# SonyResearch/micro_diffusion

Hardware: AMD Instinct MI355X
Metric: training images/sec (global batch 2048) MicroDiT-XL/2 256-res mask=0.75 (higher is better)
Workload: dtype bf16; 1 GPU; MicroDiT_XL_2 res_256_pretrain.yaml mask=0.75, full step = 2 microbatches x 1024 fwd+bwd + grad exchange + clip 0.25 + AdamW; global_batch=2048, microbatch=1024, parallelism=dp1, grad_exchange=none (single rank)

## Files before the change

include/microdit_hip.h:

```cpp
#ifndef MICRODIT_HIP_H
#define MICRODIT_HIP_H

#include <stdint.h>

#ifdef __cplusplus
extern "C" {
#endif

#ifndef __HIP_PLATFORM_AMD__
typedef struct ihipStream_t* hipStream_t;
#endif

#define MD_ABI_VERSION 6
int md_abi_version(void);

enum md_act { MD_ACT_NONE = 0, MD_ACT_GELU_TANH = 1, MD_ACT_GELU_ERF = 2, MD_ACT_SILU = 3 };

enum md_epilogue {
    MD_EPI_STORE_BF16 = 0,
    MD_EPI_RESIDUAL = 1,
    MD_EPI_STORE_F32 = 2,
    MD_EPI_ACCUM_F32 = 3,
    MD_EPI_ATOMIC_F32 = 4,
    MD_EPI_DACT = 5,
// ... 7 lines not shown
    int64_t M, N;
    int64_t c_off;
} md_gemm_problem;
#define MD_GEMM_MAX_PROBLEMS 8

typedef struct md_gemm_args {
    const void* A;
    const void* B;
    void* C;
    void* C2;
    const void* bias;
    const void* res;
    const void* gate;
    const void* aux;
    int64_t M, N, K;
    int64_t lda, ldb, ldc, ldc2, ldr, ldg, ldaux;
    int64_t sA, sB, sC, sC2, sBias, sAux;
    int64_t sSplit;
    int64_t rows_per_sample;
    int32_t batch;
    int32_t ksplit;
    int32_t a_kcontig, b_kcontig;
    int32_t mode;
    int32_t act;
    float alpha;
    int32_t variant;
    int32_t raster_group_n;
    void* timeline;
    int32_t* chosen_variant;
    const void* const* A_list;
    const void* const* B_list;
    int32_t list_segments;
    const md_gemm_problem* problems;
    int32_t n_problems;
    int32_t cu_limit;
    void* tail_ws;
    int64_t tail_ws_bytes;
    int32_t tail_mode;
    int32_t* tail_used;
    int32_t dact_cached;
} md_gemm_args;

#define MD_NOT_ELIGIBLE (-2)
enum md_gemm_variant {
    MD_GEMM_AUTO = 0,
    MD_GEMM_REG128 = 1,
    MD_GEMM_DMA128 = 2,
    MD_GEMM_PACED256 = 3,
    MD_GEMM_PP256 = 4,
    MD_GEMM_W4 = 5
};

int md_gemm_bf16(const md_gemm_args* args, hipStream_t stream);
int md_splitk_reduce(const float* ws, float* out, int64_t M, int64_t N, int64_t ldo, int64_t sOut, int32_t ksplit,
                     int32_t batch, int32_t accumulate, hipStream_t stream);

int md_splitk_reduce_flat(const float* ws, float* out, int64_t n, int64_t slice_stride, int32_t ksplit, int32_t accumulate,
                          hipStream_t stream);

typedef struct md_ln_args {
    const void* x;
    const void* w;
    const void* shift;
    const void* scale;
    const void* pos;
    void* out;
    void* mean;
    void* rstd;
    int64_t rows, C, ldx, ldo, ldmod, rows_per_sample, pos_rows;
    float eps;
    int32_t act;
} md_ln_args;

typedef struct md_ln_bwd_args {
    const void* dz;
    void* dx;
    void* dscale;
    void* dshift;
    void* dw;
    int64_t lddz, lddx, ldg;
    int64_t rows_per_block;
    int32_t accumulate;
    int32_t dscale_is_output;
} md_ln_bwd_args;

int md_ln_fwd(const md_ln_args* a, hipStream_t stream);
int md_ln_bwd(const md_ln_args* a, const md_ln_bwd_args* b, hipStream_t stream);

int md_qkln_fwd(void* buf, int64_t rows, int64_t ld, int64_t col0, int64_t width, int32_t nseg, int64_t seg_stride,
                float* rstd_out, float eps, hipStream_t stream);
int md_qkln_bwd(void* d, int64_t ldd, int64_t dcol0, const void* y, int64_t ldy, int64_t ycol0, int64_t rows,
                int64_t width, int32_t nseg, int64_t dseg_stride, int64_t yseg_stride, const float* rstd, hipStream_t stream);

int md_qkln_fwd_hm(const void* buf, int64_t rows, int64_t ld, int64_t col0, int64_t width, int32_t nseg, int64_t seg_stride,
                   void* out, int64_t out_seg_stride, int64_t S, int32_t hd, float* rstd_out, float eps, hipStream_t stream);
int md_qkln_bwd_hm(const void* dy, int64_t dy_seg_stride, const void* y, int64_t y_seg_stride, void* d, int64_t ldd, int64_t dcol0,
                   int64_t dseg_stride, int64_t rows, int64_t width, int32_t nseg, int64_t S, int32_t hd, const float* rstd,
                   hipStream_t stream);

enum md_det_kind { MD_DET_GATE_BWD = 0, MD_DET_LN_BWD = 1, MD_DET_COLSUM = 2 };
int md_det_ws_floats(int32_t kind, int64_t rows, int64_t rows_per_sample, int64_t rows_per_block, int64_t C, int64_t* out_floats);
int md_ln_bwd_det(const md_ln_args* a, const md_ln_bwd_args* b, float* ws, int64_t ws_floats, hipStream_t stream);
int md_gate_bwd_det(const void* dx, const void* br, const void* gate, int64_t ldgate, void* dbr, float* dgate, int64_t lddg,
                    int64_t rows, int64_t C, int64_t rows_per_sample, int64_t rows_per_block, float* ws, int64_t ws_floats,
                    hipStream_t stream);
int md_colsum_det(const void* x, int32_t x_is_f32, int64_t ld, float* out, int64_t rows, int64_t C, float* ws, int64_t ws_floats,
                  hipStream_t stream);

typedef struct md_attn_args {
    const void *q, *k, *v;
    void* o;
    void* lse;
    const void* d_o;
    void *dq, *dk, *dv;
    void* delta;
    int64_t B, H, Sq, Skv;
    int64_t ldq, ldk, ldv, ldo, sq, sk, sv, so;
    int64_t lddq, lddk, lddv, lddo, sdq, sdk, sdv, sdo;
    float scale;
    int32_t hd;
    int32_t bwd_split;
    int64_t hsq, hsk, hsv, hso, hsdq, hsdk, hsdv, hsdo;
} md_attn_args;

int md_attn_fwd(const md_attn_args* a, hipStream_t stream);
int md_attn_bwd(const md_attn_args* a, hipStream_t stream);

int md_swiglu_fwd(const void* h12, int64_t ldh, void* a, int64_t lda, int64_t M, int64_t f, hipStream_t stream);
int md_swiglu_bwd(const void* da, int64_t ldda, const void* h12, int64_t ldh, void* dh12, int64_t lddh, int64_t M, int64_t f,
                  hipStream_t stream);
int md_gate_bwd(const void* dx, const void* br, const void* gate, int64_t ldgate, void* dbr, float* dgate, int64_t lddg,
                int64_t rows, int64_t C, int64_t rows_per_sample, int64_t rows_per_block, hipStream_t stream);
int md_act_fwd(const void* x, void* y, int64_t n, int32_t act, hipStream_t stream);
int md_act_bwd(const float* dy, const void* x, void* dx, int64_t n, int32_t act, hipStream_t stream);
int md_colsum(const void* x, int32_t x_is_f32, int64_t ld, float* out, int64_t rows, int64_t C, hipStream_t stream);
int md_cast_f32_bf16(const float* x, void* y, int64_t n, const float* scale_ptr, hipStream_t stream);
int md_cast_f32_bf16_clear(float* x, void* y, int64_t n, hipStream_t stream);
int md_cast_rows_bf16(const void* x, int32_t x_dtype, void* y, int64_t rows, int64_t C, const float* rowscale,
                      int64_t rows_per_sample, hipStream_t stream);
int md_mean_tokens(const void* y, void* out, int64_t B, int64_t L, int64_t C, hipStream_t stream);
int md_mean_tokens_bwd(const void* dpool, float* dy, int64_t B, int64_t L, int64_t C, hipStream_t stream);
int md_add_bf16(const void* a, const void* b, void* y, int64_t n, hipStream_t stream);
int md_fill_zero(void* p, int64_t bytes, hipStream_t stream);

int md_get_mask(const float* noise, int64_t B, int64_t T, int64_t len_keep, int32_t* keep_rows, int32_t* ids_restore,
                float* mask, hipStream_t stream);
int md_gather_rows(const void* src, int64_t ld_src, const int32_t* idx, void* dst, int64_t ld_dst, int64_t n, int64_t C,
                   hipStream_t stream);
int md_scatter_rows(const void* src, int64_t ld_src, const int32_t* idx, void* dst, int64_t ld_dst, int64_t n, int64_t C,
                    hipStream_t stream);
int md_moe_route(const float* logits, float* probs, int64_t ld, int64_t B, int64_t S, int32_t E, int32_t k, int32_t* rowidx,
                 float* gval, int32_t* slot, hipStream_t stream);
int md_moe_combine(const void* h2, const float* gval, const int32_t* slot, const void* res, const void* gate, int64_t ldgate,
                   void* br, void* out, int64_t B, int64_t S, int32_t E, int32_t k, int64_t C, hipStream_t stream);
int md_moe_combine_bwd(const void* dbr, const void* h2, const int32_t* rowidx, const float* gval, void* dh2, float* dgval,
                       int64_t R, int64_t C, hipStream_t stream);
int md_moe_dispatch_bwd(const void* dxin, const int32_t* slot, void* dx, const float* probs, int64_t ldp, const float* dgval,
                        void* dlogits, int64_t ldo, int64_t B, int64_t S, int32_t E, int32_t k, int64_t C, hipStream_t stream);

int md_edm_prepare(const float* x0, const float* eps, const float* rnd, float* xn, float* sigma, float* cin, float* cnoise,
                   int64_t B, int64_t per_sample, float p_mean, float p_std, float sigma_data, hipStream_t stream);
int md_edm_prepare_f16(const void* x0_f16, const float* eps, const float* rnd, float* xn, float* x0_f32, float* sigma, float* cin,
                       float* cnoise, int64_t B, int64_t per_sample, float p_mean, float p_std, float sigma_data,
                       hipStream_t stream);
int md_patchify(const float* x, const float* scale, void* out, int64_t B, int32_t C, int32_t H, int32_t W, int32_t p,
                hipStream_t stream);
int md_timestep_embed(const float* t, void* out, int64_t B, int32_t dim, hipStream_t stream);
int md_unpatchify(const void* tok, const int32_t* ids_restore, int64_t Tk, const float* mask_token, float* img, int64_t B,
                  int32_t C, int32_t H, int32_t W, int32_t p, hipStream_t stream);
int md_edm_loss(const void* tok, const int32_t* keep_rows, const float* xn, const float* x0, const float* sigma,
                float* loss_per_sample, float* loss_mean, float* dtok, int64_t B, int64_t Tk, int32_t C, int32_t H, int32_t W,
                int32_t p, float sigma_data, hipStream_t stream);
int md_edm_loss_train(const void* tok, const int32_t* keep_rows, const float* xn, const float* x0, const float* sigma,
                      float* loss_per_sample, float* loss_mean, void* dtok_bf16, float grad_scale, float* loss_accum,
                      float accum_weight, int64_t B, int64_t Tk, int32_t C, int32_t H, int32_t W, int32_t p, float sigma_data,
                      hipStream_t stream);

int md_logvar_fwd(const float* cnoise, const float* freq, const float* phase, const float* w, float* u, float* inv, int64_t B,
                  int32_t C, hipStream_t stream);
// ... 103 lines not shown
```

micro_diffusion_amd/csrc/attention.hip:

```cpp
#include <stdlib.h>
#include "md_common.h"
#include "../../include/microdit_hip.h"

namespace {

typedef __attribute__((address_space(3))) s16x4 lds_s16x4;
typedef unsigned int u32x4 __attribute__((ext_vector_type(4)));

__device__ __forceinline__ bf16x4 tr4(const unsigned char* p) {
    s16x4 v = __builtin_amdgcn_ds_read_tr16_b64_v4i16((lds_s16x4*)(p));
    U64 t;
    t.s = v;
    return t.h;
}

__device__ __forceinline__ bf16x8 tr_frag(const unsigned char* tile, int pitch, int k_lo, int k_hi, int col0, int lane) {
    const int li = lane & 15;
    const int col = col0 + ((lane >> 4) & 1) * 16 + (li & 3) * 4;
    const bf16x4 lo = tr4(tile + (k_lo + (li >> 2)) * pitch + col * 2);
    const bf16x4 hi = tr4(tile + (k_hi + (li >> 2)) * pitch + col * 2);
    bf16x8 f;
    f[0] = lo[0]; f[1] = lo[1]; f[2] = lo[2]; f[3] = lo[3];
    f[4] = hi[0]; f[5] = hi[1]; f[6] = hi[2]; f[7] = hi[3];
    return f;
}

__device__ __forceinline__ bf16x8 row_frag(const unsigned char* tile, int pitch, int kbase, int lane) {
    U128 t;
    t.u = *reinterpret_cast<const uint4*>(tile + (lane & 31) * pitch + (kbase + (lane >> 5) * 8) * 2);
    return t.h;
}

template <int HD>
__device__ __forceinline__ void stage_tile(unsigned char* tile, int pitch, const bf16* src, int64_t ld, int64_t row0,
                                           int64_t nrows, int nstage, int tid, int nthreads) {
    constexpr int CPR = HD / 8;
    for (int task = tid; task < nstage * CPR; task += nthreads) {
        const int r = task / CPR, c = task % CPR;
        uint4 v = make_uint4(0, 0, 0, 0);
        if (row0 + r < nrows) v = *reinterpret_cast<const uint4*>(src + (row0 + r) * ld + c * 8);
        *reinterpret_cast<uint4*>(tile + r * pitch + c * 16) = v;
    }
}

constexpr int STG = 32;

template <int HD, int MAXIT>
__device__ __forceinline__ void stage_pair(unsigned char* tileA, unsigned char* tileB, int pitch, const bf16* A, int64_t lda, const bf16* B,
                                           int64_t ldb, int64_t row0, int64_t nrows, int nstage, int tid, int nthreads) {
    constexpr int CPR = HD / 8;
    uint4 ra[MAXIT], rb[MAXIT];
#pragma unroll
    for (int it = 0; it < MAXIT; ++it) {
        const int task = tid + it * nthreads, r = task / CPR, c = task % CPR;
        ra[it] = rb[it] = make_uint4(0, 0, 0, 0);
        if (task < nstage * CPR && row0 + r < nrows) {
            ra[it] = *reinterpret_cast<const uint4*>(A + (row0 + r) * lda + c * 8);
            rb[it] = *reinterpret_cast<const uint4*>(B + (row0 + r) * ldb + c * 8);
        }
    }
#pragma unroll
    for (int it = 0; it < MAXIT; ++it) {
        const int task = tid + it * nthreads, r = task / CPR, c = task % CPR;
        if (task < nstage * CPR) {
            *reinterpret_cast<uint4*>(tileA + r * pitch + c * 16) = ra[it];
            *reinterpret_cast<uint4*>(tileB + r * pitch + c * 16) = rb[it];
        }
    }
}

constexpr float LOG2E = 1.4426950408889634f;
__device__ __forceinline__ int tile_slot(int r, int hh) { return (r & 3) + 8 * (r >> 2) + 4 * hh; }

__device__ __forceinline__ void ds_cols(f32x16& s, const f32x16& dp, float c1, float l2, float dlt, int rem, int hh) {
#pragma unroll
    for (int r = 0; r < 16; ++r) {
        const float pr = tile_slot(r, hh) < rem ? __builtin_amdgcn_exp2f(s[r] * c1 - l2) : 0.f;
        s[r] = pr * (dp[r] - dlt);
    }
}
template <bool WANT_P, bool WANT_DS>
__device__ __forceinline__ void p_ds_rows(f32x16& s, f32x16& dp, float c1, const float* tL2, const float* tDlt, int rem, int hh) {
#pragma unroll
    for (int r = 0; r < 16; ++r) {
        const int ql = tile_slot(r, hh);
        const float pr = ql < rem ? __builtin_amdgcn_exp2f(s[r] * c1 - tL2[ql]) : 0.f;
        if (WANT_DS) dp[r] = pr * (dp[r] - tDlt[ql]);
        if (WANT_P) s[r] = pr;
    }
}
constexpr float LSE_MASKED = 1e30f;
template <bool WANT_P, bool WANT_DS, bool VEC = true>
__device__ __forceinline__ void p_ds_rows_nomask(f32x16& s, f32x16& dp, float c1, const float* tL2, const float* tDlt, int hh) {
    if (!VEC) {
#pragma unroll
        for (int r = 0; r < 16; ++r) {
            const int ql = tile_slot(r, hh);
            const float pr = __builtin_amdgcn_exp2f(s[r] * c1 - tL2[ql]);
            if (WANT_DS) dp[r] = pr * (dp[r] - tDlt[ql]);
            if (WANT_P) s[r] = pr;
        }
        return;
    }
#pragma unroll
    for (int j = 0; j < 4; ++j) {
        const f32x4 l4 = *reinterpret_cast<const f32x4*>(tL2 + 8 * j + 4 * hh);
        f32x4 d4 = {0.f, 0.f, 0.f, 0.f};
        if (WANT_DS) d4 = *reinterpret_cast<const f32x4*>(tDlt + 8 * j + 4 * hh);
#pragma unroll
        for (int e = 0; e < 4; ++e) {
            const int r = 4 * j + e;
            const float pr = __builtin_amdgcn_exp2f(s[r] * c1 - l4[e]);
            if (WANT_DS) dp[r] = pr * (dp[r] - d4[e]);
            if (WANT_P) s[r] = pr;
        }
    }
}

__device__ __forceinline__ bf16x8 pack8(const f32x16& a, int base) {
    bf16x8 o;
#pragma unroll
    for (int e = 0; e < 8; ++e) o[e] = f2bf(a[base + e]);
    return o;
}

__device__ __forceinline__ void bh_of(int64_t lin, int64_t H, int64_t B, int64_t& b, int64_t& h) {
    const int64_t n8 = (B >> 3) * 8 * H;
    if (lin < n8) {
        const int64_t s = lin >> 3, x = lin & 7;
        lin = ((s / H) * 8 + x) * H + s % H;
    }
    b = lin / H;
    h = lin - b * H;
}

template <int HD>
__device__ __forceinline__ void store_rows(bf16* dst_row, const f32x16 (&acc)[HD / 32], float mul, int lane) {
    const int hh = lane >> 5;
#pragma unroll
    for (int di = 0; di < HD / 32; ++di)
#pragma unroll
        for (int g = 0; g < 4; ++g) {
            bf16x4 o;
#pragma unroll
            for (int e = 0; e < 4; ++e) o[e] = f2bf(acc[di][4 * g + e] * mul);
            st_bf16x4(dst_row + di * 32 + 8 * g + 4 * hh, o);
        }
}

template <int HD, int MAXIT>
__global__ __launch_bounds__(256) void attn_fwd_kernel(md_attn_args p) {
    constexpr int PK = (HD + 8) * 2;
    __shared__ __attribute__((aligned(16))) unsigned char smem[2 * STG * PK];
    const int tid = threadIdx.x, lane = tid & 63, wave = tid >> 6, nthreads = blockDim.x, nw = nthreads >> 6;
    const int hh = lane >> 5;
    const float c1 = p.scale * LOG2E;
    int64_t b = blockIdx.z, h = blockIdx.y;
    if (gridDim.x == 1) bh_of(blockIdx.y + (int64_t)gridDim.y * blockIdx.z, gridDim.y, gridDim.z, b, h);
    const int64_t q = ((int64_t)blockIdx.x * nw + wave) * 32 + (lane & 31);
    const bool qvalid = q < p.Sq;
    const bf16* Q = reinterpret_cast<const bf16*>(p.q) + b * p.sq + h * p.hsq;
    const bf16* K = reinterpret_cast<const bf16*>(p.k) + b * p.sk + h * p.hsk;
    const bf16* V = reinterpret_cast<const bf16*>(p.v) + b * p.sv + h * p.hsv;

    bf16x8 qf[HD / 16];
#pragma unroll
    for (int s = 0; s < HD / 16; ++s) {
        if (qvalid)
            qf[s] = ld_bf16x8(Q + q * p.ldq + s * 16 + hh * 8);
        else
#pragma unroll
            for (int e = 0; e < 8; ++e) qf[s][e] = f2bf(0.f);
    }
    f32x16 oacc[HD / 32];
#pragma unroll
    for (int di = 0; di < HD / 32; ++di)
#pragma unroll
        for (int r = 0; r < 16; ++r) oacc[di][r] = 0.f;
    float m = -1e30f, l = 0.f;

    for (int64_t kbase = 0; kbase < p.Skv; kbase += STG) {
        __syncthreads();
        const int nst = (int)((p.Skv - kbase >= STG) ? STG : ((p.Skv - kbase + 31) / 32) * 32);
        stage_pair<HD, MAXIT>(smem, smem + STG * PK, PK, K, p.ldk, V, p.ldv, kbase, p.Skv, nst, tid, nthreads);
        __syncthreads();
      for (int sub = 0; sub < STG / 32 && kbase + sub * 32 < p.Skv; ++sub) {
        const int64_t key0 = kbase + sub * 32;
        const unsigned char* sK = smem + sub * 32 * PK;
        const unsigned char* sV = smem + STG * PK + sub * 32 * PK;
        f32x16 sacc;
#pragma unroll
        for (int r = 0; r < 16; ++r) sacc[r] = 0.f;
#pragma unroll
        for (int s = 0; s < HD / 16; ++s)
            sacc = __builtin_amdgcn_mfma_f32_32x32x16_bf16(row_frag(sK, PK, s * 16, lane), qf[s], sacc, 0, 0, 0);
        const int rem = (int)(p.Skv - key0);
        float tmax = -1e30f;
#pragma unroll
        for (int r = 0; r < 16; ++r) {
            sacc[r] = tile_slot(r, hh) < rem ? sacc[r] * c1 : -1e30f;
            tmax = fmaxf(tmax, sacc[r]);
        }
        tmax = fmaxf(tmax, __shfl_xor(tmax, 32, 64));
        const float m_new = fmaxf(m, tmax);
        const float alpha = __builtin_amdgcn_exp2f(m - m_new);
        float psum = 0.f;
#pragma unroll
        for (int r = 0; r < 16; ++r) {
            const float pr = __builtin_amdgcn_exp2f(sacc[r] - m_new);
            sacc[r] = pr;
            psum += pr;
        }
        psum += __shfl_xor(psum, 32, 64);
        l = l * alpha + psum;
        m = m_new;
#pragma unroll
        for (int di = 0; di < HD / 32; ++di)
#pragma unroll
            for (int r = 0; r < 16; ++r) oacc[di][r] *= alpha;
#pragma unroll
        for (int sp = 0; sp < 2; ++sp) {
            const bf16x8 pf = pack8(sacc, 8 * sp);
#pragma unroll
            for (int di = 0; di < HD / 32; ++di)
                oacc[di] = __builtin_amdgcn_mfma_f32_32x32x16_bf16(
                    tr_frag(sV, PK, 16 * sp + 4 * hh, 16 * sp + 8 + 4 * hh, di * 32, lane), pf, oacc[di], 0, 0, 0);
        }
      }
    }
    if (qvalid) {
        bf16* O = reinterpret_cast<bf16*>(p.o) + b * p.so + h * p.hso + q * p.ldo;
        store_rows<HD>(O, oacc, 1.f / l, lane);
        if (lane < 32 && p.lse) reinterpret_cast<float*>(p.lse)[(b * p.H + h) * p.Sq + q] = (m + __log2f(l)) * 0.6931471805599453f;
    }
}


template <int HD, int MAXIT>
struct ChunkRegs {
    u32x4 a[MAXIT], b[MAXIT];
};
template <int HD, int SCH, int MAXIT>
__device__ __forceinline__ void chunk_load(ChunkRegs<HD, MAXIT>& R, const bf16* A, int64_t lda, const bf16* B, int64_t ldb, int64_t row0,
                                           int64_t nrows, int tid, int nthreads) {
    constexpr int CPR = HD / 8;
    const u32x4 z4 = {0u, 0u, 0u, 0u};
#pragma unroll
    for (int it = 0; it < MAXIT; ++it) {
        const int task = tid + it * nthreads, r = task / CPR, c = task % CPR;
        const bool ok = task < SCH * CPR && row0 + r < nrows;
        R.a[it] = ok ? *reinterpret_cast<const u32x4*>(A + (row0 + r) * lda + c * 8) : z4;
        R.b[it] = ok ? *reinterpret_cast<const u32x4*>(B + (row0 + r) * ldb + c * 8) : z4;
    }
}
template <int HD, int SCH, int MAXIT>
__device__ __forceinline__ void chunk_store(const ChunkRegs<HD, MAXIT>& R, unsigned char* tileA, unsigned char* tileB, int pitch, int tid,
                                            int nthreads) {
    constexpr int CPR = HD / 8;
#pragma unroll
    for (int it = 0; it < MAXIT; ++it) {
        const int task = tid + it * nthreads, r = task / CPR, c = task % CPR;
        if (task < SCH * CPR) {
            *reinterpret_cast<u32x4*>(tileA + r * pitch + c * 16) = R.a[it];
            *reinterpret_cast<u32x4*>(tileB + r * pitch + c * 16) = R.b[it];
        }
    }
}

template <int HD, int SCH, int MAXIT>
__global__ __launch_bounds__(512) void attn_fwd_stream_kernel(md_attn_args p) {
    constexpr int PK = (HD + 8) * 2;
    __shared__ __attribute__((aligned(16))) unsigned char smem[2 * SCH * PK];
    unsigned char* sKc = smem;
    unsigned char* sVc = smem + SCH * PK;
    const int tid = threadIdx.x, lane = tid & 63, wave = tid >> 6, nthreads = blockDim.x, nw = nthreads >> 6;
    const int hh = lane >> 5;
    const float c1 = p.scale * LOG2E;
    const int64_t b = blockIdx.z, h = blockIdx.y;
    const int64_t q = ((int64_t)blockIdx.x * nw + wave) * 32 + (lane & 31);
    const bool qvalid = q < p.Sq;
    const bf16* Q = reinterpret_cast<const bf16*>(p.q) + b * p.sq + h * p.hsq;
    const bf16* K = reinterpret_cast<const bf16*>(p.k) + b * p.sk + h * p.hsk;
    const bf16* V = reinterpret_cast<const bf16*>(p.v) + b * p.sv + h * p.hsv;

    ChunkRegs<HD, MAXIT> R;
    chunk_load<HD, SCH, MAXIT>(R, K, p.ldk, V, p.ldv, 0, p.Skv, tid, nthreads);
    bf16x8 qf[HD / 16];
// ... 224 lines not shown
        if (tid < SCH) {
            sLseAll[tid] = rl;
            sDltAll[tid] = rd;
        }
        __syncthreads();
        if (qbase + SCH < p.Sq) {
            chunk_load<HD, SCH, MAXIT>(R, Q, p.ldq, dO, p.lddo, qbase + SCH, p.Sq, tid, nthreads);
            const int64_t rn = qbase + SCH + tid;
            const bool ok = tid < SCH && rn < p.Sq;
            rl = ok ? LSE[rn] * LOG2E : LSE_MASKED;
            rd = ok ? DLT[rn] : 0.f;
        }
        auto tile = [&](int sub, int rem) {
            const unsigned char* tQ = sQ + sub * 32 * PK;
            const unsigned char* tdO = sdO + sub * 32 * PK;
            const float* tLse = sLseAll + sub * 32;
            const float* tDlt = sDltAll + sub * 32;
            f32x16 sacc, dpacc;
#pragma unroll
            for (int r = 0; r < 16; ++r) {
                sacc[r] = 0.f;
                dpacc[r] = 0.f;
            }
#pragma unroll
            for (int s = 0; s < HD / 16; ++s) {
                sacc = __builtin_amdgcn_mfma_f32_32x32x16_bf16(row_frag(tQ, PK, s * 16, lane), kf[s], sacc, 0, 0, 0);
                dpacc = __builtin_amdgcn_mfma_f32_32x32x16_bf16(row_frag(tdO, PK, s * 16, lane), vf[s], dpacc, 0, 0, 0);
            }
            (void)rem;
            p_ds_rows_nomask<true, true>(sacc, dpacc, c1, tLse, tDlt, hh);
#pragma unroll
            for (int sp = 0; sp < 2; ++sp) {
                const bf16x8 pf = pack8(sacc, 8 * sp);
                const bf16x8 dsf = pack8(dpacc, 8 * sp);
#pragma unroll
                for (int di = 0; di < HD / 32; ++di) {
                    dvacc[di] = __builtin_amdgcn_mfma_f32_32x32x16_bf16(
                        tr_frag(tdO, PK, 16 * sp + 4 * hh, 16 * sp + 8 + 4 * hh, di * 32, lane), pf, dvacc[di], 0, 0, 0);
                    dkacc[di] = __builtin_amdgcn_mfma_f32_32x32x16_bf16(
                        tr_frag(tQ, PK, 16 * sp + 4 * hh, 16 * sp + 8 + 4 * hh, di * 32, lane), dsf, dkacc[di], 0, 0, 0);
                }
            }
        };
        for (int sub = 0; sub < SCH / 32 && qbase + sub * 32 < p.Sq; ++sub) tile(sub, (int)(p.Sq - qbase - sub * 32));
    }
    if (kvalid) {
        bf16* dK = reinterpret_cast<bf16*>(p.dk) + b * p.sdk + h * p.hsdk + key * p.lddk;
        bf16* dV = reinterpret_cast<bf16*>(p.dv) + b * p.sdv + h * p.hsdv + key * p.lddv;
        store_rows<HD>(dK, dkacc, p.scale, lane);
        store_rows<HD>(dV, dvacc, 1.f, lane);
    }
}

template <int HD, int SQP, int SKP>
__global__ __launch_bounds__((SQP > SKP ? SQP : SKP) * 2) void attn_bwd_fused_kernel(md_attn_args p) {
    constexpr int PK = (HD + 8) * 2;
    __shared__ __attribute__((aligned(16))) unsigned char smem[(2 * SQP + 2 * SKP) * PK + 2 * SQP * 4];
    unsigned char* sQ = smem;
    unsigned char* sdO = smem + SQP * PK;
    unsigned char* sK = smem + 2 * SQP * PK;
    unsigned char* sV = sK + SKP * PK;
    float* sLse = reinterpret_cast<float*>(sV + SKP * PK);
    float* sDlt = sLse + SQP;
    const int tid = threadIdx.x, lane = tid & 63, wave = tid >> 6, nthreads = blockDim.x;
    const int hh = lane >> 5;
    const float c1 = p.scale * LOG2E;
    int64_t b, h;
    bh_of(blockIdx.x + (int64_t)gridDim.x * blockIdx.y, gridDim.x, gridDim.y, b, h);
    const bf16* Q = reinterpret_cast<const bf16*>(p.q) + b * p.sq + h * p.hsq;
    const bf16* K = reinterpret_cast<const bf16*>(p.k) + b * p.sk + h * p.hsk;
    const bf16* V = reinterpret_cast<const bf16*>(p.v) + b * p.sv + h * p.hsv;
    const bf16* dO = reinterpret_cast<const bf16*>(p.d_o) + b * p.sdo + h * p.hsdo;
    const bf16* O = reinterpret_cast<const bf16*>(p.o) + b * p.so + h * p.hso;
    const int nq32 = (int)((p.Sq + 31) / 32), nk32 = (int)((p.Skv + 31) / 32);

    {
        constexpr int CPR = HD / 8;
        constexpr int NT = (SQP > SKP ? SQP : SKP) * 2;
        constexpr int ITQ = (SQP * CPR + NT - 1) / NT, ITK = (SKP * CPR + NT - 1) / NT;
        const float* LSE = reinterpret_cast<const float*>(p.lse) + (b * p.H + h) * p.Sq;
        u32x4 rq[ITQ], rdo[ITQ], ro[ITQ], rk[ITK], rv[ITK];
        float rl[ITQ];
        const u32x4 z4 = {0u, 0u, 0u, 0u};
#pragma unroll
        for (int it = 0; it < ITQ; ++it) {
            const int task = tid + it * NT, r = task / CPR, c = task % CPR;
            const bool ok = task < SQP * CPR && r < p.Sq;
            rq[it] = ok ? *reinterpret_cast<const u32x4*>(Q + (int64_t)r * p.ldq + c * 8) : z4;
            rdo[it] = ok ? *reinterpret_cast<const u32x4*>(dO + (int64_t)r * p.lddo + c * 8) : z4;
            ro[it] = ok ? *reinterpret_cast<const u32x4*>(O + (int64_t)r * p.ldo + c * 8) : z4;
            rl[it] = (ok && c == 0) ? LSE[r] : 0.f;
        }
#pragma unroll
        for (int it = 0; it < ITK; ++it) {
            const int task = tid + it * NT, r = task / CPR, c = task % CPR;
            const bool ok = task < SKP * CPR && r < p.Skv;
            rk[it] = ok ? *reinterpret_cast<const u32x4*>(K + (int64_t)r * p.ldk + c * 8) : z4;
            rv[it] = ok ? *reinterpret_cast<const u32x4*>(V + (int64_t)r * p.ldv + c * 8) : z4;
        }
#pragma unroll
        for (int it = 0; it < ITQ; ++it) {
            const int task = tid + it * NT, r = task / CPR, c = task % CPR;
            if (task < SQP * CPR) {
                *reinterpret_cast<u32x4*>(sQ + r * PK + c * 16) = rq[it];
                *reinterpret_cast<u32x4*>(sdO + r * PK + c * 16) = rdo[it];
            }
            const bf16x8 g = __builtin_bit_cast(bf16x8, rdo[it]), o = __builtin_bit_cast(bf16x8, ro[it]);
            float d = 0.f;
#pragma unroll
            for (int e = 0; e < 8; ++e) d += bf2f(o[e]) * bf2f(g[e]);
#pragma unroll
            for (int s2 = CPR / 2; s2 > 0; s2 >>= 1) d += __shfl_xor(d, s2, 64);
            if (c == 0 && task < SQP * CPR) {
                sDlt[r] = d;
                sLse[r] = rl[it] * LOG2E;
            }
        }
#pragma unroll
        for (int it = 0; it < ITK; ++it) {
            const int task = tid + it * NT, r = task / CPR, c = task % CPR;
            if (task < SKP * CPR) {
                *reinterpret_cast<u32x4*>(sK + r * PK + c * 16) = rk[it];
                *reinterpret_cast<u32x4*>(sV + r * PK + c * 16) = rv[it];
            }
        }
    }
    __syncthreads();

    if (wave < nq32) {
        const unsigned char* myQ = sQ + wave * 32 * PK;
        const unsigned char* mydO = sdO + wave * 32 * PK;
        const int64_t q = (int64_t)wave * 32 + (lane & 31);
        bf16x8 qf[HD / 16], dof[HD / 16];
#pragma unroll
        for (int s = 0; s < HD / 16; ++s) {
            qf[s] = row_frag(myQ, PK, s * 16, lane);
            dof[s] = row_frag(mydO, PK, s * 16, lane);
        }
        const float lse = sLse[wave * 32 + (lane & 31)], dlt = sDlt[wave * 32 + (lane & 31)];
        f32x16 dqacc[HD / 32];
#pragma unroll
        for (int di = 0; di < HD / 32; ++di)
#pragma unroll
            for (int r = 0; r < 16; ++r) dqacc[di][r] = 0.f;
        for (int j = 0; j < nk32; ++j) {
            const unsigned char* tK = sK + j * 32 * PK;
            const unsigned char* tV = sV + j * 32 * PK;
            f32x16 sacc, dpacc;
#pragma unroll
            for (int r = 0; r < 16; ++r) {
                sacc[r] = 0.f;
                dpacc[r] = 0.f;
            }
#pragma unroll
            for (int s = 0; s < HD / 16; ++s) {
                sacc = __builtin_amdgcn_mfma_f32_32x32x16_bf16(row_frag(tK, PK, s * 16, lane), qf[s], sacc, 0, 0, 0);
                dpacc = __builtin_amdgcn_mfma_f32_32x32x16_bf16(row_frag(tV, PK, s * 16, lane), dof[s], dpacc, 0, 0, 0);
            }
            ds_cols(sacc, dpacc, c1, lse, dlt, (int)p.Skv - j * 32, hh);
#pragma unroll
            for (int sp = 0; sp < 2; ++sp) {
                const bf16x8 dsf = pack8(sacc, 8 * sp);
#pragma unroll
                for (int di = 0; di < HD / 32; ++di)
                    dqacc[di] = __builtin_amdgcn_mfma_f32_32x32x16_bf16(
                        tr_frag(tK, PK, 16 * sp + 4 * hh, 16 * sp + 8 + 4 * hh, di * 32, lane), dsf, dqacc[di], 0, 0, 0);
            }
        }
        if (q < p.Sq) {
            bf16* dQ = reinterpret_cast<bf16*>(p.dq) + b * p.sdq + h * p.hsdq + q * p.lddq;
            store_rows<HD>(dQ, dqacc, p.scale, lane);
        }
    }
// ... 4 lines not shown
        bf16x8 kf[HD / 16], vf[HD / 16];
#pragma unroll
        for (int s = 0; s < HD / 16; ++s) {
            kf[s] = row_frag(myK, PK, s * 16, lane);
            vf[s] = row_frag(myV, PK, s * 16, lane);
        }
        f32x16 dkacc[HD / 32], dvacc[HD / 32];
#pragma unroll
        for (int di = 0; di < HD / 32; ++di)
#pragma unroll
            for (int r = 0; r < 16; ++r) {
                dkacc[di][r] = 0.f;
                dvacc[di][r] = 0.f;
            }
        for (int i = 0; i < nq32; ++i) {
            const unsigned char* tQ = sQ + i * 32 * PK;
            const unsigned char* tdO = sdO + i * 32 * PK;
            const float* tLse = sLse + i * 32;
            const float* tDlt = sDlt + i * 32;
            f32x16 sacc, dpacc;
#pragma unroll
            for (int r = 0; r < 16; ++r) {
                sacc[r] = 0.f;
                dpacc[r] = 0.f;
            }
#pragma unroll
            for (int s = 0; s < HD / 16; ++s) {
                sacc = __builtin_amdgcn_mfma_f32_32x32x16_bf16(row_frag(tQ, PK, s * 16, lane), kf[s], sacc, 0, 0, 0);
                dpacc = __builtin_amdgcn_mfma_f32_32x32x16_bf16(row_frag(tdO, PK, s * 16, lane), vf[s], dpacc, 0, 0, 0);
            }
            p_ds_rows<true, true>(sacc, dpacc, c1, tLse, tDlt, (int)p.Sq - i * 32, hh);
#pragma unroll
            for (int sp = 0; sp < 2; ++sp) {
                const bf16x8 pf = pack8(sacc, 8 * sp);
                const bf16x8 dsf = pack8(dpacc, 8 * sp);
#pragma unroll
                for (int di = 0; di < HD / 32; ++di) {
                    dvacc[di] = __builtin_amdgcn_mfma_f32_32x32x16_bf16(
                        tr_frag(tdO, PK, 16 * sp + 4 * hh, 16 * sp + 8 + 4 * hh, di * 32, lane), pf, dvacc[di], 0, 0, 0);
                    dkacc[di] = __builtin_amdgcn_mfma_f32_32x32x16_bf16(
                        tr_frag(tQ, PK, 16 * sp + 4 * hh, 16 * sp + 8 + 4 * hh, di * 32, lane), dsf, dkacc[di], 0, 0, 0);
                }
            }
        }
        if (key < p.Skv) {
            bf16* dK = reinterpret_cast<bf16*>(p.dk) + b * p.sdk + h * p.hsdk + key * p.lddk;
            bf16* dV = reinterpret_cast<bf16*>(p.dv) + b * p.sdv + h * p.hsdv + key * p.lddv;
            store_rows<HD>(dK, dkacc, p.scale, lane);
            store_rows<HD>(dV, dvacc, 1.f, lane);
        }
    }
}

template <int HD, int SQP, int SKP, bool SPLIT2>
__global__ __launch_bounds__((SQP > SKP ? SQP : SKP) * 2) __attribute__((amdgpu_waves_per_eu(SPLIT2 ? 4 : 3)))
void attn_bwd_fused2_kernel(md_attn_args p) {
    constexpr int PK = (HD + 8) * 2;
    constexpr int RMAX = SQP > SKP ? SQP : SKP;
    constexpr int NT = RMAX * 2;
    __shared__ __attribute__((aligned(16))) unsigned char smem[2 * RMAX * PK + 2 * SQP * 4];
    unsigned char* sA = smem;
    unsigned char* sB = smem + RMAX * PK;
    float* sLse = reinterpret_cast<float*>(smem + 2 * RMAX * PK);
    float* sDlt = sLse + SQP;
    const int tid = threadIdx.x, lane = tid & 63, wave = tid >> 6;
    const int hh = lane >> 5;
    const float c1 = p.scale * LOG2E;
    int64_t b, h;
    bh_of(blockIdx.x + (int64_t)gridDim.x * blockIdx.y, gridDim.x, gridDim.y, b, h);
    const bf16* Q = reinterpret_cast<const bf16*>(p.q) + b * p.sq + h * p.hsq;
    const bf16* K = reinterpret_cast<const bf16*>(p.k) + b * p.sk + h * p.hsk;
    const bf16* V = reinterpret_cast<const bf16*>(p.v) + b * p.sv + h * p.hsv;
    const bf16* dO = reinterpret_cast<const bf16*>(p.d_o) + b * p.sdo + h * p.hsdo;
    const bf16* O = reinterpret_cast<const bf16*>(p.o) + b * p.so + h * p.hso;
    const int nq32 = (int)((p.Sq + 31) / 32), nk32 = (int)((p.Skv + 31) / 32);

    constexpr int CPR = HD / 8;
    constexpr int ITQ = (SQP * CPR + NT - 1) / NT, ITK = (SKP * CPR + NT - 1) / NT;
    u32x4 rk[ITK], rv[ITK];
    {
        const float* LSE = reinterpret_cast<const float*>(p.lse) + (b * p.H + h) * p.Sq;
        u32x4 rq[ITQ], rdo[ITQ], ro[ITQ];
        float rl[ITQ];
        const u32x4 z4 = {0u, 0u, 0u, 0u};
#pragma unroll
        for (int it = 0; it < ITQ; ++it) {
            const int task = tid + it * NT, r = task / CPR, c = task % CPR;
            const bool ok = task < SQP * CPR && r < p.Sq;
            rq[it] = ok ? *reinterpret_cast<const u32x4*>(Q + (int64_t)r * p.ldq + c * 8) : z4;
            rdo[it] = ok ? *reinterpret_cast<const u32x4*>(dO + (int64_t)r * p.lddo + c * 8) : z4;
            ro[it] = ok ? *reinterpret_cast<const u32x4*>(O + (int64_t)r * p.ldo + c * 8) : z4;
            rl[it] = (ok && c == 0) ? LSE[r] : 0.f;
        }
#pragma unroll
        for (int it = 0; it < ITK; ++it) {
            const int task = tid + it * NT, r = task / CPR, c = task % CPR;
            const bool ok = task < SKP * CPR && r < p.Skv;
            rk[it] = ok ? *reinterpret_cast<const u32x4*>(K + (int64_t)r * p.ldk + c * 8) : z4;
            rv[it] = ok ? *reinterpret_cast<const u32x4*>(V + (int64_t)r * p.ldv + c * 8) : z4;
        }
#pragma unroll
        for (int it = 0; it < ITQ; ++it) {
            const int task = tid + it * NT, r = task / CPR, c = task % CPR;
            if (task < SQP * CPR) {
                *reinterpret_cast<u32x4*>(sA + r * PK + c * 16) = rq[it];
                *reinterpret_cast<u32x4*>(sB + r * PK + c * 16) = rdo[it];
            }
            const bf16x8 g = __builtin_bit_cast(bf16x8, rdo[it]), o = __builtin_bit_cast(bf16x8, ro[it]);
            float d = 0.f;
#pragma unroll
            for (int e = 0; e < 8; ++e) d += bf2f(o[e]) * bf2f(g[e]);
#pragma unroll
            for (int s2 = CPR / 2; s2 > 0; s2 >>= 1) d += __shfl_xor(d, s2, 64);
            if (c == 0 && task < SQP * CPR) {
                sDlt[r] = d;
                sLse[r] = rl[it] * LOG2E;
            }
        }
    }
    __syncthreads();
    const bool qrole = wave < nq32, krole = wave < nk32;
    bf16x8 qf[HD / 16], dof[HD / 16];
    float lse = 0.f, dlt = 0.f;
    if (qrole) {
#pragma unroll
        for (int s = 0; s < HD / 16; ++s) {
            qf[s] = row_frag(sA + wave * 32 * PK, PK, s * 16, lane);
            dof[s] = row_frag(sB + wave * 32 * PK, PK, s * 16, lane);
        }
        lse = sLse[wave * 32 + (lane & 31)];
        dlt = sDlt[wave * 32 + (lane & 31)];
    }
    __syncthreads();
#pragma unroll
    for (int it = 0; it < ITK; ++it) {
        const int task = tid + it * NT, r = task / CPR, c = task % CPR;
        if (task < SKP * CPR) {
            *reinterpret_cast<u32x4*>(sA + r * PK + c * 16) = rk[it];
            *reinterpret_cast<u32x4*>(sB + r * PK + c * 16) = rv[it];
        }
    }
    __syncthreads();
    if (qrole) {
        const int64_t q = (int64_t)wave * 32 + (lane & 31);
        f32x16 dqacc[HD / 32];
#pragma unroll
        for (int di = 0; di < HD / 32; ++di)
#pragma unroll
            for (int r = 0; r < 16; ++r) dqacc[di][r] = 0.f;
        for (int j = 0; j < nk32; ++j) {
            const unsigned char* tK = sA + j * 32 * PK;
            const unsigned char* tV = sB + j * 32 * PK;
            f32x16 sacc, dpacc;
#pragma unroll
            for (int r = 0; r < 16; ++r) {
                sacc[r] = 0.f;
                dpacc[r] = 0.f;
            }
#pragma unroll
            for (int s = 0; s < HD / 16; ++s) {
                sacc = __builtin_amdgcn_mfma_f32_32x32x16_bf16(row_frag(tK, PK, s * 16, lane), qf[s], sacc, 0, 0, 0);
                dpacc = __builtin_amdgcn_mfma_f32_32x32x16_bf16(row_frag(tV, PK, s * 16, lane), dof[s], dpacc, 0, 0, 0);
            }
            ds_cols(sacc, dpacc, c1, lse, dlt, (int)p.Skv - j * 32, hh);
#pragma unroll
            for (int sp = 0; sp < 2; ++sp) {
                const bf16x8 dsf = pack8(sacc, 8 * sp);
#pragma unroll
                for (int di = 0; di < HD / 32; ++di)
// ... 86 lines not shown
                            tr_frag(tQ, PK, 16 * sp + 4 * hh, 16 * sp + 8 + 4 * hh, di * 32, lane), dsf, acc[di], 0, 0, 0);
                }
            }
            if (key < p.Skv) {
                store_rows<HD>(dK, acc, p.scale, lane);
            }
        } else {
            f32x16 dkacc[HD / 32], dvacc[HD / 32];
#pragma unroll
            for (int di = 0; di < HD / 32; ++di)
#pragma unroll
                for (int r = 0; r < 16; ++r) {
                    dkacc[di][r] = 0.f;
                    dvacc[di][r] = 0.f;
                }
            for (int i = 0; i < nq32; ++i) {
                const unsigned char* tQ = sA + i * 32 * PK;
                const unsigned char* tdO = sB + i * 32 * PK;
                const float* tLse = sLse + i * 32;
                const float* tDlt = sDlt + i * 32;
                f32x16 sacc, dpacc;
#pragma unroll
                for (int r = 0; r < 16; ++r) {
                    sacc[r] = 0.f;
                    dpacc[r] = 0.f;
                }
#pragma unroll
                for (int s = 0; s < HD / 16; ++s) {
                    sacc = __builtin_amdgcn_mfma_f32_32x32x16_bf16(row_frag(tQ, PK, s * 16, lane), kf[s], sacc, 0, 0, 0);
                    dpacc = __builtin_amdgcn_mfma_f32_32x32x16_bf16(row_frag(tdO, PK, s * 16, lane), vf[s], dpacc, 0, 0, 0);
                }
                p_ds_rows<true, true>(sacc, dpacc, c1, tLse, tDlt, (int)p.Sq - i * 32, hh);
#pragma unroll
                for (int sp = 0; sp < 2; ++sp) {
                    const bf16x8 pf = pack8(sacc, 8 * sp);
                    const bf16x8 dsf = pack8(dpacc, 8 * sp);
#pragma unroll
                    for (int di = 0; di < HD / 32; ++di) {
                        dvacc[di] = __builtin_amdgcn_mfma_f32_32x32x16_bf16(
                            tr_frag(tdO, PK, 16 * sp + 4 * hh, 16 * sp + 8 + 4 * hh, di * 32, lane), pf, dvacc[di], 0, 0, 0);
                        dkacc[di] = __builtin_amdgcn_mfma_f32_32x32x16_bf16(
                            tr_frag(tQ, PK, 16 * sp + 4 * hh, 16 * sp + 8 + 4 * hh, di * 32, lane), dsf, dkacc[di], 0, 0, 0);
                    }
                }
            }
            if (key < p.Skv) {
                store_rows<HD>(dK, dkacc, p.scale, lane);
                store_rows<HD>(dV, dvacc, 1.f, lane);
            }
        }
    }
}

inline int fused_bucket(int64_t S) { return S <= 64 ? 64 : S <= 96 ? 96 : S <= 256 ? 256 : 0; }

template <int HD>
void launch_bwd_fused_one(const md_attn_args* a, int variant, int bq, int bk, hipStream_t stream) {
    const dim3 grid((unsigned)a->H, (unsigned)a->B);
#define FUSED(SQP, SKP) hipLaunchKernelGGL((attn_bwd_fused_kernel<HD, SQP, SKP>), grid, dim3((SQP > SKP ? SQP : SKP) * 2), 0, stream, *a)
#define FUSED2(SQP, SKP, SPL) \
    hipLaunchKernelGGL((attn_bwd_fused2_kernel<HD, SQP, SKP, SPL>), grid, dim3((SQP > SKP ? SQP : SKP) * 2), 0, stream, *a)
#define SMALL(SQP, SKP)                          \
    do {                                         \
        if (variant == 2 || (variant == 0 && SQP == 64 && SKP == 64)) FUSED(SQP, SKP); \
        else if (variant == 4) FUSED2(SQP, SKP, true); \
        else FUSED2(SQP, SKP, false);            \
    } while (0)
#define BIG(SQP, SKP)                            \
    do {                                         \
        if (variant == 2) FUSED(SQP, SKP);       \
        else FUSED2(SQP, SKP, true);             \
    } while (0)
    if (bq == 64 && bk == 64) SMALL(64, 64);
    else if (bq == 64 && bk == 96) SMALL(64, 96);
    else if (bq == 96 && bk == 64) SMALL(96, 64);
    else if (bq == 96 && bk == 96) SMALL(96, 96);
    else if (bq == 256 && bk == 96) BIG(256, 96);
    else if (bq == 256 && bk == 256) BIG(256, 256);
    else if (bq == 64 && bk == 256) BIG(64, 256);
    else if (bq == 256 && bk == 64) BIG(256, 64);
    else BIG(96, 256);
#undef SMALL
#undef BIG
#undef FUSED
#undef FUSED2
}

template <int HD>
bool launch_bwd_fused(const md_attn_args* a, int variant, hipStream_t stream) {
    const int bq = fused_bucket(a->Sq), bk = fused_bucket(a->Skv);
    if (!bq || !bk) return false;
    launch_bwd_fused_one<HD>(a, variant, bq, bk, stream);
    return true;
}

inline int stream_waves(int64_t S) {
    static const int cap = [] {
        const char* e = getenv("MD_ATTN_STREAM_WAVES");
        const int v = e ? atoi(e) : 8;
        return v < 3 ? 3 : (v > 8 ? 8 : v);
    }();
    int w = (int)((S + 31) / 32 > cap ? cap : (S + 31) / 32);
    if (w == 5) w = 6;
    if (w < 3) w = 3;
    return w;
}
template <int HD>
void launch_bwd_stream(const md_attn_args* a, hipStream_t stream) {
    int nwq = stream_waves(a->Sq), nwk = stream_waves(a->Skv);
    if (a->Skv <= 128 && nwq > 4) nwq = 4;
    if (a->Sq <= 128 && nwk > 4) nwk = 4;
    const dim3 gq((unsigned)((a->Sq + 32 * nwq - 1) / (32 * nwq)), (unsigned)a->H, (unsigned)a->B);
    const dim3 gk((unsigned)((a->Skv + 32 * nwk - 1) / (32 * nwk)), (unsigned)a->H, (unsigned)a->B);
#define STREAM(KERN, GRID, NW)                                                                                       \
    do {                                                                                                             \
        const dim3 blk(64 * NW);                                                                                     \
        if (NW == 8) hipLaunchKernelGGL((KERN<HD, 128, 2>), GRID, blk, 0, stream, *a);                               \
        else if (NW >= 6) hipLaunchKernelGGL((KERN<HD, 128, 3>), GRID, blk, 0, stream, *a);                          \
        else if (NW == 4) hipLaunchKernelGGL((KERN<HD, 64, 2>), GRID, blk, 0, stream, *a);                           \
        else hipLaunchKernelGGL((KERN<HD, 64, 3>), GRID, blk, 0, stream, *a);                                        \
    } while (0)
    STREAM(attn_bwd_dq_stream_kernel, gq, nwq);
    STREAM(attn_bwd_dkv_stream_kernel, gk, nwk);
#undef STREAM
}

inline int waves_for(int64_t S) {
    int64_t w = (S + 31) / 32;
    return (int)(w > 4 ? 4 : (w < 1 ? 1 : w));
}

inline bool attn_ok(const md_attn_args* a) {
    return a && a->q && a->k && a->v && a->o && a->B > 0 && a->H > 0 && a->Sq > 0 && a->Skv > 0 &&
           (a->hd == 32 || a->hd == 64) && a->ldq % 8 == 0 && a->ldk % 8 == 0 && a->ldv % 8 == 0 && a->ldo % 4 == 0 &&
           a->sq % 8 == 0 && a->sk % 8 == 0 && a->sv % 8 == 0 && a->so % 4 == 0 && a->hsq % 8 == 0 && a->hsk % 8 == 0 &&
           a->hsv % 8 == 0 && a->hso % 4 == 0 && a->hsdo % 8 == 0 && a->hsdq % 4 == 0 && a->hsdk % 4 == 0 && a->hsdv % 4 == 0;
}

inline md_attn_args with_head_strides(const md_attn_args* a) {
    md_attn_args c = *a;
    int64_t* hs[8] = {&c.hsq, &c.hsk, &c.hsv, &c.hso, &c.hsdq, &c.hsdk, &c.hsdv, &c.hsdo};
    for (int64_t* p : hs)
        if (*p == 0) *p = c.hd;
    return c;
}

}

extern "C" int md_attn_fwd(const md_attn_args* a_in, hipStream_t stream) {
    if (!attn_ok(a_in)) return MD_BAD_ARG;
    const md_attn_args args = with_head_strides(a_in);
    const md_attn_args* a = &args;
    static const bool fwd_stream = [] { const char* e = getenv("MD_ATTN_FWD_STREAM"); return !e || atoi(e) != 0; }();
    static const int fwd_stream_min = [] { const char* e = getenv("MD_ATTN_FWD_STREAM_MIN_SKV"); return e ? atoi(e) : 257; }();
    if (fwd_stream && a->Skv >= fwd_stream_min && a->Sq >= 192) {
        int nw = stream_waves(a->Sq);
        if (nw < 6) nw = 6;
        const dim3 grid((unsigned)((a->Sq + 32 * nw - 1) / (32 * nw)), (unsigned)a->H, (unsigned)a->B), blk(64 * nw);
        if (a->hd == 64) {
            if (nw == 8) hipLaunchKernelGGL((attn_fwd_stream_kernel<64, 128, 2>), grid, blk, 0, stream, *a);
            else hipLaunchKernelGGL((attn_fwd_stream_kernel<64, 128, 3>), grid, blk, 0, stream, *a);
        } else {
            if (nw == 8) hipLaunchKernelGGL((attn_fwd_stream_kernel<32, 128, 2>), grid, blk, 0, stream, *a);
            else hipLaunchKernelGGL((attn_fwd_stream_kernel<32, 128, 3>), grid, blk, 0, stream, *a);
        }
        MD_LAUNCH_CHECK();
        return 0;
    }
    const int nw = waves_for(a->Sq);
    dim3 grid((unsigned)((a->Sq + 32 * nw - 1) / (32 * nw)), (unsigned)a->H, (unsigned)a->B);
#define FWD(HD_)                                                                                                  \
    do {                                                                                                           \
        const int chunks = (32 * (HD_ / 8) + 64 * nw - 1) / (64 * nw);                                             \
        if (chunks <= 1) hipLaunchKernelGGL((attn_fwd_kernel<HD_, 1>), grid, dim3(64 * nw), 0, stream, *a);        \
        else if (chunks == 2) hipLaunchKernelGGL((attn_fwd_kernel<HD_, 2>), grid, dim3(64 * nw), 0, stream, *a);   \
        else hipLaunchKernelGGL((attn_fwd_kernel<HD_, 4>), grid, dim3(64 * nw), 0, stream, *a);                    \
    } while (0)
    if (a->hd == 64) FWD(64);
    else FWD(32);
#undef FWD
    MD_LAUNCH_CHECK();
    return 0;
}

extern "C" int md_attn_bwd(const md_attn_args* a_in, hipStream_t stream) {
    if (!attn_ok(a_in) || !a_in->d_o || !a_in->dq || !a_in->dk || !a_in->dv || !a_in->lse || !a_in->delta) return MD_BAD_ARG;
    const md_attn_args args = with_head_strides(a_in);
    const md_attn_args* a = &args;
    if (a->lddq % 4 || a->lddk % 4 || a->lddv % 4 || a->lddo % 8 || a->sdo % 8) return MD_BAD_ARG;
    if (a->bwd_split < 0 || a->bwd_split > 5 || a->bwd_split == 1) return MD_BAD_ARG;
    const bool long_seq = a->Sq > 256 || a->Skv > 256;
    if (a->bwd_split == 5 || (a->bwd_split == 0 && long_seq)) {
        if (a->hd == 64) launch_bwd_stream<64>(a, stream);
        else launch_bwd_stream<32>(a, stream);
        MD_LAUNCH_CHECK();
        return 0;
    }
    if (a->hd == 64 ? launch_bwd_fused<64>(a, a->bwd_split, stream) : launch_bwd_fused<32>(a, a->bwd_split, stream)) {
        MD_LAUNCH_CHECK();
        return 0;
    }
    return -1;
}
```

micro_diffusion_amd/csrc/gemm_pp_common.h:

```cpp
#pragma once
#include "md_common.h"
#include "gemm_common.h"

namespace {

constexpr int PT = 256;
constexpr int HT = 16384;
constexpr int B_REGION = 65536;
constexpr int NUM_CU = 256;

template <int KC>
struct Frag;
template <>
struct Frag<1> {
    bf16x8 v;
    __device__ __forceinline__ bf16x8 get() const { return v; }
};
template <>
struct Frag<0> {
    bf16x4 lo, hi;
    __device__ __forceinline__ bf16x8 get() const {
        bf16x8 f;
        f[0] = lo[0]; f[1] = lo[1]; f[2] = lo[2]; f[3] = lo[3];
        f[4] = hi[0]; f[5] = hi[1]; f[6] = hi[2]; f[7] = hi[3];
// ... 43 lines not shown
    else frag_read<KC, SLOT + KS * 4096>(f, ad[I]);
}

template <int KC>
__device__ __forceinline__ void stage_offsets(unsigned (&ofs)[2][2], int r0, int rmax, int ld, int wave, int lane) {
    asm volatile("" : "+v"(lane));
#pragma unroll
    for (int h = 0; h < 2; ++h)
#pragma unroll
        for (int j = 0; j < 2; ++j) {
            if constexpr (KC) {
                const int row = (wave * 2 + j) * 8 + (lane >> 3);
                const int c = (lane & 7) ^ ((row >> 1) & 7);
                int gr = r0 + h * 128 + row;
                gr = (gr < rmax ? gr : rmax - 1) - r0;
                ofs[h][j] = (unsigned)(gr * ld + c * 8) * 2u;
            } else {
                const int kk = (wave * 2 + j) * 4 + (lane >> 4);
                const int c = (lane & 15) ^ ((kk & 3) << 2);
                int gc = r0 + h * 128 + c * 8;
                const int last = (rmax - 1) & ~7;
                gc = (gc < last ? gc : last) - r0;
                ofs[h][j] = (unsigned)(kk * ld + gc) * 2u;
            }
        }
}

__device__ __forceinline__ void stage_half(const char* base, const unsigned (&ofs)[2], unsigned char* slot, int wave) {
#pragma unroll
    for (int j = 0; j < 2; ++j)
        __builtin_amdgcn_global_load_lds((glb_void_t*)(base + ofs[j]), (lds_void_t*)(slot + (wave * 2 + j) * 1024), 16, 0, 0);
}

constexpr int PP_MAX_PROB = MD_GEMM_MAX_PROBLEMS;
struct PPProblem {
    const void* A;
    const void* B;
    int64_t c_off;
    int lda, ldb, M, N;
    int ntm, ntn, tile0, group_n;
};

struct PPPlan {
    int ntm, ntn, ntiles, total;
    int nk;
    int kspan;
    int group_n;
    int M, N, ksplit;
    int lda, ldb;
    int rps_shift;
    int nseg, nk_seg;
    int nprob;
    int tail_first, tail_units, tail_split, tail_nk;
    PPProblem prob[PP_MAX_PROB];
};

__device__ __forceinline__ void work_decode(const PPPlan& w, int item, int& m0, int& n0, int& batch, int& split) {
    const unsigned y = (unsigned)item / (unsigned)w.ntiles;
    const unsigned t = (unsigned)item - y * (unsigned)w.ntiles;
    batch = (int)(y / (unsigned)w.ksplit);
    split = (int)(y - (unsigned)batch * (unsigned)w.ksplit);
    const unsigned per_group = (unsigned)(w.group_n * w.ntm);
    const unsigned g = t / per_group, rem = t - g * per_group;
    const int first_n = (int)g * w.group_n;
    const int gn = (w.ntn - first_n) < w.group_n ? (w.ntn - first_n) : w.group_n;
    const unsigned tm = rem / (unsigned)gn;
    m0 = (int)tm * PT;
    n0 = (first_n + (int)(rem - tm * (unsigned)gn)) * PT;
}

__device__ __forceinline__ void work_decode_grouped(const PPPlan& w, int item, int& q, int& m0, int& n0, int& split) {
    const unsigned y = (unsigned)item / (unsigned)w.ntiles;
    const int t = (int)((unsigned)item - y * (unsigned)w.ntiles);
    split = (int)y;
    q = 0;
#pragma unroll 1
    for (int i = 1; i < w.nprob; ++i)
        if (t >= w.prob[i].tile0) q = i;
    const PPProblem& pr = w.prob[q];
    const unsigned tl = (unsigned)(t - pr.tile0);
    const unsigned per_group = (unsigned)(pr.group_n * pr.ntm);
    const unsigned g = tl / per_group, rem = tl - g * per_group;
    const int first_n = (int)g * pr.group_n;
    const int gn = (pr.ntn - first_n) < pr.group_n ? (pr.ntn - first_n) : pr.group_n;
    const unsigned tm = rem / (unsigned)gn;
    m0 = (int)tm * PT;
    n0 = (first_n + (int)(rem - tm * (unsigned)gn)) * PT;
}

enum {
    PP_E_BF16 = 0,
    PP_E_BF16_GELU = 1,
    PP_E_RES = 2,
    PP_E_DACT_GELU = 3,
    PP_E_F32 = 4,
    PP_E_BF16_GELU_D = 5,
    PP_E_DACT_MUL = 6,
    PP_E_DACT_SWIGLU = 7
};

struct EpiTile {
    int m0, n0, batch, split;
    int q, M, N, ldc;
    bool plain;
    char* cbase;
    char* c2base;
// ... 114 lines not shown
inline int md_gemm_pp_epi_kind(const md_gemm_args* a) {
    switch (a->mode) {
        case MD_EPI_STORE_BF16:
            return a->act == MD_ACT_NONE ? PP_E_BF16 : a->act == MD_ACT_GELU_ERF ? ((a->dact_cached && a->C2) ? PP_E_BF16_GELU_D : PP_E_BF16_GELU) : -1;
        case MD_EPI_RESIDUAL: return PP_E_RES;
        case MD_EPI_DACT: return a->act == MD_ACT_GELU_ERF ? (a->dact_cached ? PP_E_DACT_MUL : PP_E_DACT_GELU) : -1;
        case MD_EPI_STORE_F32: return PP_E_F32;
        case MD_EPI_SWIGLU_BWD: return PP_E_DACT_SWIGLU;
        default: return -1;
    }
}


inline bool md_gemm_pp_plan(const md_gemm_args* a, PPPlan* w) {
    w->nprob = 0;
    w->ntm = (int)((a->M + PT - 1) / PT);
    w->ntn = (int)((a->N + PT - 1) / PT);
    w->ntiles = w->ntm * w->ntn;
    if (a->problems && a->n_problems > 0) {
        w->nprob = a->n_problems;
        int t0 = 0;
        const int64_t kspan_ = a->K / a->ksplit;
        for (int i = 0; i < a->n_problems; ++i) {
            const md_gemm_problem& s = a->problems[i];
            PPProblem& d = w->prob[i];
            d.A = s.A; d.B = s.B; d.c_off = s.c_off;
            d.lda = (int)s.lda; d.ldb = (int)s.ldb; d.M = (int)s.M; d.N = (int)s.N;
            d.ntm = (int)((s.M + PT - 1) / PT);
            d.ntn = (int)((s.N + PT - 1) / PT);
            d.tile0 = t0;
            int64_t g = (2 << 20) / (PT * kspan_ * 2);
            if (g < 4) g = 4;
            if (g > d.ntn) g = d.ntn;
            d.group_n = (int)g;
            t0 += d.ntm * d.ntn;
        }
        w->ntiles = t0;
    }
    const int64_t total = (int64_t)w->ntiles * (w->nprob ? 1 : a->batch) * a->ksplit;
    if (total > (1 << 30)) return false;
    w->total = (int)total;
    w->kspan = (int)(a->K / a->ksplit);
    w->nk = w->kspan / BKT;
    w->nseg = (a->A_list && a->list_segments > 1) ? a->list_segments : 1;
    w->nk_seg = w->nk / w->nseg;
    w->group_n = a->raster_group_n > 0 ? a->raster_group_n : 1;
    w->M = (int)a->M;
    w->N = (int)a->N;
    w->ksplit = a->ksplit;
    w->lda = (int)a->lda;
    w->ldb = (int)a->ldb;
    w->tail_first = w->total;
    w->tail_units = w->tail_split = w->tail_nk = 0;
    w->rps_shift = -1;
    if (a->rows_per_sample > 0 && (a->rows_per_sample & (a->rows_per_sample - 1)) == 0) {
        w->rps_shift = 0;
        while (((int64_t)1 << w->rps_shift) < a->rows_per_sample) ++w->rps_shift;
    }
    return true;
}

}
```

micro_diffusion_amd/csrc/gemm_w4.hip:

```cpp
#include "gemm_pp_common.h"

namespace {

struct W4Addr {
    unsigned adA[8];
    unsigned adB[8];
    unsigned aofs[8], bofs[8];
    unsigned ldsw;
};

#ifndef W4_ACC_INC
#define W4_ACC_INC "gemm_w4_acc.inc"
#endif
#include W4_ACC_INC

constexpr int W4_BUF = 32768;
constexpr int W4_BREG = 65536;
constexpr int W4_SLAB = 8192;

constexpr bool w4_is_dact(int epi) { return epi == PP_E_DACT_GELU || epi == PP_E_DACT_MUL || epi == PP_E_DACT_SWIGLU; }



typedef unsigned w4_u32x2 __attribute__((ext_vector_type(2), may_alias));
typedef unsigned w4_u32x4 __attribute__((ext_vector_type(4), may_alias));

struct W4Tile {
    int m0, n0, batch;
    int mlim, nlim;
    char* cbase;
    char* c2base;
    const char* opbase;
    const char* gbase;
};

struct W4EpiLane {
    unsigned wr[8];
    unsigned rd[4];
    unsigned oc, oc2, oo, og;
    int rg, c8;
};
struct W4Ops {
    uint4 v[4];
    uint4 gq;
    uint4 v2[4];
};

template <int EPI>
__device__ __forceinline__ void w4_epi_lane(const md_gemm_args& p, const W4Tile& et, int wcol, int lane_in, W4EpiLane& L) {
    int lane = lane_in;
    asm volatile("" : "+v"(lane));
    const int r = lane & 15, g = lane >> 4;
#pragma unroll
    for (int j = 0; j < 8; ++j) L.wr[j] = (unsigned)(r * 256 + ((32 * j + 8 * g) ^ (r << 4)));
#pragma unroll
    for (int t = 0; t < 4; ++t) L.rd[t] = (unsigned)((4 * t + g) * 256 + ((16 * r) ^ ((4 * t + g) << 4)));
    L.rg = g;
    L.c8 = r * 8;
    const int cc = wcol + r * 8 < et.nlim ? r * 8 : 0;
    L.oc = (unsigned)(g * (int)p.ldc + r * 8) * 2u;
    L.oc2 = (unsigned)(g * (int)p.ldc2 + r * 8) * 2u;
    L.oo = (unsigned)(g * (int)(EPI == PP_E_RES ? p.ldr : p.ldaux) + cc) * 2u;
    L.og = (unsigned)cc * 2u;
}

struct W4Rows {
    char* c;
    char* c2;
    const char* op;
    int64_t sc, sc2, so;
};

template <int EPI, bool INTERIOR>
__device__ __forceinline__ void w4_epi_req(const md_gemm_args& p, const W4Tile& et, const W4EpiLane& L, const char* oprow, int row0, int wcol, uint4& dst) {
    if (INTERIOR) {
        dst = *reinterpret_cast<const uint4*>(oprow + L.oo);
    } else if constexpr (EPI == PP_E_DACT_SWIGLU) {
        dst = make_uint4(0u, 0u, 0u, 0u);
    } else {
        const int64_t ldo = EPI == PP_E_RES ? p.ldr : p.ldaux;
        const int row = row0 + L.rg < et.mlim - 1 ? row0 + L.rg : et.mlim - 1;
        dst = *reinterpret_cast<const uint4*>(et.opbase + ((int64_t)row * ldo + wcol) * 2 + L.og);
    }
}
template <int EPI, int I>
__device__ __forceinline__ void w4_epi_gate(const md_gemm_args& p, const PPPlan& w, const W4Tile& et, const W4EpiLane& L, int wrow, int wcol, uint4& gq) {
    gq = make_uint4(0x3f803f80u, 0x3f803f80u, 0x3f803f80u, 0x3f803f80u);
    if (et.gbase) {
        int r0 = et.m0 + wrow + 16 * I;
        r0 = r0 < w.M - 1 ? r0 : w.M - 1;
        const unsigned srow = w.rps_shift >= 0 ? (unsigned)r0 >> w.rps_shift : (unsigned)r0 / (unsigned)p.rows_per_sample;
        gq = *reinterpret_cast<const uint4*>(et.gbase + ((int64_t)srow * p.ldg + wcol) * 2 + L.og);
    }
}

template <int I>
__device__ __forceinline__ void w4_epi_write(unsigned char* slab, const W4EpiLane& L) {
    unsigned char* half = slab + (I & 1) * 4096;
#pragma unroll
    for (int jh = 0; jh < 2; ++jh) {
        float a[16];
        if (jh == 0) w4_acc_read16<I, 0>(a);
        else w4_acc_read16<I, 1>(a);
#pragma unroll
        for (int q = 0; q < 4; ++q) {
            const w4_u32x2 v = {cvt_pk_bf16(a[4 * q], a[4 * q + 1]), cvt_pk_bf16(a[4 * q + 2], a[4 * q + 3])};
            *reinterpret_cast<w4_u32x2*>(half + L.wr[4 * jh + q]) = v;
        }
    }
}

template <int EPI, int I, bool INTERIOR>
__device__ __forceinline__ void w4_epi_store(const md_gemm_args& p, const PPPlan& w, const W4Tile& et, const W4EpiLane& L, int wrow, int wcol,
                                             const w4_u32x4 (&Tv)[4], W4Ops& ops, W4Rows& R) {
#pragma unroll
    for (int t = 0; t < 4; ++t) {
        const uint4 T = make_uint4(Tv[t].x, Tv[t].y, Tv[t].z, Tv[t].w);
        const int row0 = wrow + 16 * I + 4 * t;
        const bool ok = INTERIOR || (wcol + L.c8 < et.nlim && row0 + L.rg < et.mlim);
        char* const crow = R.c;
        uint4 out = T;
        if constexpr (EPI == PP_E_BF16 || EPI == PP_E_RES || EPI == PP_E_BF16_GELU) {
            if (et.c2base && ok) *reinterpret_cast<uint4*>(R.c2 + L.oc2) = T;
        }
        if constexpr (EPI == PP_E_BF16_GELU) {
            float v[8];
            unpack8(T, v);
#pragma unroll
            for (int e = 0; e < 8; e += 2) {
                const f32x2 g2 = gelu_erf_2(f32x2{v[e], v[e + 1]});
                v[e] = g2.x;
                v[e + 1] = g2.y;
            }
            out = make_uint4(cvt_pk_bf16(v[0], v[1]), cvt_pk_bf16(v[2], v[3]), cvt_pk_bf16(v[4], v[5]), cvt_pk_bf16(v[6], v[7]));
        } else if constexpr (EPI == PP_E_BF16_GELU_D) {
            float v[8], dv[8];
            unpack8(T, v);
#pragma unroll
            for (int e = 0; e < 8; e += 2) {
                f32x2 g2, d2;
                gelu_dgelu_erf_2(f32x2{v[e], v[e + 1]}, g2, d2);
                v[e] = g2.x;
                v[e + 1] = g2.y;
                dv[e] = d2.x;
                dv[e + 1] = d2.y;
            }
            out = make_uint4(cvt_pk_bf16(v[0], v[1]), cvt_pk_bf16(v[2], v[3]), cvt_pk_bf16(v[4], v[5]), cvt_pk_bf16(v[6], v[7]));
            if (et.c2base && ok)
                *reinterpret_cast<uint4*>(R.c2 + L.oc2) =
                    make_uint4(cvt_pk_bf16(dv[0], dv[1]), cvt_pk_bf16(dv[2], dv[3]), cvt_pk_bf16(dv[4], dv[5]), cvt_pk_bf16(dv[6], dv[7]));
        } else if constexpr (EPI == PP_E_RES) {
            const uint4 gq = ops.gq;
            const unsigned lw[4] = {T.x, T.y, T.z, T.w}, rw[4] = {ops.v[t].x, ops.v[t].y, ops.v[t].z, ops.v[t].w}, gw[4] = {gq.x, gq.y, gq.z, gq.w};
            unsigned ow[4];
#pragma unroll
            for (int h = 0; h < 4; ++h) {
                const float y0 = __uint_as_float(lw[h] << 16), y1 = __uint_as_float(lw[h] & 0xffff0000u);
                const float r0 = __uint_as_float(rw[h] << 16), r1 = __uint_as_float(rw[h] & 0xffff0000u);
                const float g0 = __uint_as_float(gw[h] << 16), g1 = __uint_as_float(gw[h] & 0xffff0000u);
                ow[h] = cvt_pk_bf16(r0 + g0 * y0, r1 + g1 * y1);
            }
            out = make_uint4(ow[0], ow[1], ow[2], ow[3]);
        } else if constexpr (EPI == PP_E_DACT_MUL) {
            float v[8], ax[8];
            unpack8(T, v);
            unpack8(ops.v[t], ax);
#pragma unroll
            for (int e = 0; e < 8; ++e) v[e] *= ax[e];
            out = make_uint4(cvt_pk_bf16(v[0], v[1]), cvt_pk_bf16(v[2], v[3]), cvt_pk_bf16(v[4], v[5]), cvt_pk_bf16(v[6], v[7]));
        } else if constexpr (EPI == PP_E_DACT_SWIGLU) {
            float g[8], x1[8], x2[8], o2[8];
            unpack8(T, g);
            unpack8(ops.v[t], x1);
            unpack8(ops.v2[t], x2);
#pragma unroll
            for (int e = 0; e < 8; ++e) {
                const float sg = __builtin_amdgcn_rcpf(1.f + __builtin_amdgcn_exp2f(x1[e] * -1.4426950408889634f));
                const float sl = x1[e] * sg;
                o2[e] = g[e] * sl;
                g[e] = g[e] * x2[e] * (sg + sl * (1.f - sg));
            }
            out = make_uint4(cvt_pk_bf16(g[0], g[1]), cvt_pk_bf16(g[2], g[3]), cvt_pk_bf16(g[4], g[5]), cvt_pk_bf16(g[6], g[7]));
            if (ok) *reinterpret_cast<uint4*>(crow + L.oc + 2 * (int64_t)p.N) =
                make_uint4(cvt_pk_bf16(o2[0], o2[1]), cvt_pk_bf16(o2[2], o2[3]), cvt_pk_bf16(o2[4], o2[5]), cvt_pk_bf16(o2[6], o2[7]));
        } else if constexpr (EPI == PP_E_DACT_GELU) {
            float v[8], ax[8];
            unpack8(T, v);
            unpack8(ops.v[t], ax);
#pragma unroll
            for (int e = 0; e < 8; e += 2) {
                const f32x2 d = dgelu_erf_2(f32x2{ax[e], ax[e + 1]});
                v[e] *= d.x;
                v[e + 1] *= d.y;
            }
            out = make_uint4(cvt_pk_bf16(v[0], v[1]), cvt_pk_bf16(v[2], v[3]), cvt_pk_bf16(v[4], v[5]), cvt_pk_bf16(v[6], v[7]));
        }
#ifdef W4_X_NOSTORE
        asm volatile("" : : "v"(out.x), "v"(out.y), "v"(out.z), "v"(out.w));
#else
        if (ok) *reinterpret_cast<uint4*>(crow + L.oc) = out;
#endif
        if constexpr ((EPI == PP_E_RES || w4_is_dact(EPI)) && I < 7) {
            w4_epi_req<EPI, INTERIOR>(p, et, L, R.op, row0 + 16, wcol, ops.v[t]);
            if constexpr (EPI == PP_E_DACT_SWIGLU) w4_epi_req<EPI, INTERIOR>(p, et, L, R.op + 2 * (int64_t)p.N, row0 + 16, wcol, ops.v2[t]);
        }
        R.c += R.sc;
        R.c2 += R.sc2;
        R.op += R.so;
    }
    if constexpr (EPI == PP_E_RES && I < 7) w4_epi_gate<EPI, I + 1>(p, w, et, L, wrow, wcol, ops.gq);
}

template <int I>
__device__ __forceinline__ void w4_epi_read(unsigned char* slab, const W4EpiLane& L, w4_u32x4 (&Tv)[4]) {
    unsigned char* half = slab + (I & 1) * 4096;
#pragma unroll
    for (int t = 0; t < 4; ++t) Tv[t] = *reinterpret_cast<const w4_u32x4*>(half + L.rd[t]);
}

template <int EPI, bool INTERIOR>
__device__ __forceinline__ void w4_epilogue(const md_gemm_args& p, const PPPlan& w, const W4Tile& et, unsigned char* slab, int wrow, int wcol, int lane) {
    W4EpiLane L;
    w4_epi_lane<EPI>(p, et, wcol, lane, L);
    W4Ops ops;
    W4Rows R;
    const int64_t ldo = EPI == PP_E_RES ? p.ldr : p.ldaux;
    R.sc = 8 * p.ldc;
    R.sc2 = 8 * p.ldc2;
    R.so = 8 * ldo;
    R.c = et.cbase + ((int64_t)wrow * p.ldc + wcol) * 2;
    R.c2 = et.c2base ? et.c2base + ((int64_t)wrow * p.ldc2 + wcol) * 2 : nullptr;
    R.op = nullptr;
    if constexpr (EPI == PP_E_RES || w4_is_dact(EPI)) {
        R.op = et.opbase + ((int64_t)wrow * ldo + wcol) * 2;
#pragma unroll
        for (int t = 0; t < 4; ++t) {
            w4_epi_req<EPI, INTERIOR>(p, et, L, R.op, wrow + 4 * t, wcol, ops.v[t]);
            if constexpr (EPI == PP_E_DACT_SWIGLU) w4_epi_req<EPI, INTERIOR>(p, et, L, R.op + 2 * (int64_t)p.N, wrow + 4 * t, wcol, ops.v2[t]);
            R.op += R.so;
        }
        if constexpr (EPI == PP_E_RES) w4_epi_gate<EPI, 0>(p, w, et, L, wrow, wcol, ops.gq);
    }
    w4_u32x4 Tv[4];
    w4_epi_write<0>(slab, L);
#define W4_EPI_STEP(I)                                                                                                  \
    w4_epi_read<I>(slab, L, Tv);                                                                                        \
    if constexpr ((I) < 7) w4_epi_write<((I) < 7 ? (I) + 1 : 7)>(slab, L);                                               \
    if constexpr ((I) == 0) asm volatile("s_waitcnt vmcnt(0)" ::: "memory");                                             \
    w4_epi_store<EPI, I, INTERIOR>(p, w, et, L, wrow, wcol, Tv, ops, R);
    W4_EPI_STEP(0) W4_EPI_STEP(1) W4_EPI_STEP(2) W4_EPI_STEP(3) W4_EPI_STEP(4) W4_EPI_STEP(5) W4_EPI_STEP(6) W4_EPI_STEP(7)
#undef W4_EPI_STEP
}

__device__ __forceinline__ void w4_epilogue_f32(float* tile, int64_t ldc, int wrow, int wcol, int lane_in) {
    int lane = lane_in;
    asm volatile("" : "+v"(lane));
    float* const p0 = tile + (int64_t)(wrow + (lane & 15)) * ldc + wcol + 4 * (lane >> 4);
    asm volatile("s_waitcnt vmcnt(0)" ::: "memory");
#define W4_F32_STEP(I, JH)                                                                                               \
    {                                                                                                                    \
        float a[16];                                                                                                     \
        w4_acc_read16<I, JH>(a);                                                                                         \
        float* const pr = p0 + (int64_t)(16 * (I)) * ldc + 64 * (JH);                                                    \
        _Pragma("unroll") for (int q = 0; q < 4; ++q)                                                                    \
            *reinterpret_cast<float4*>(pr + 16 * q) = make_float4(a[4 * q], a[4 * q + 1], a[4 * q + 2], a[4 * q + 3]);   \
    }
    W4_F32_STEP(0, 0) W4_F32_STEP(0, 1) W4_F32_STEP(1, 0) W4_F32_STEP(1, 1) W4_F32_STEP(2, 0) W4_F32_STEP(2, 1) W4_F32_STEP(3, 0) W4_F32_STEP(3, 1)
    W4_F32_STEP(4, 0) W4_F32_STEP(4, 1) W4_F32_STEP(5, 0) W4_F32_STEP(5, 1) W4_F32_STEP(6, 0) W4_F32_STEP(6, 1) W4_F32_STEP(7, 0) W4_F32_STEP(7, 1)
#undef W4_F32_STEP
}

template <int AKC, int BKC, int EPI>
__global__ __launch_bounds__(256) __attribute__((amdgpu_num_vgpr(144))) void gemm_bf16_w4_kernel(md_gemm_args p, PPPlan w) {
    __shared__ __attribute__((aligned(1024))) unsigned char smem[2 * W4_BREG + 4 * W4_SLAB];
    const int tid = threadIdx.x, lane = tid & 63;
    const int wave = __builtin_amdgcn_readfirstlane(tid >> 6);
    const int wr = wave >> 1, wc = wave & 1;

    int w_first, w_stride, w_count;
    {
        const int G = gridDim.x, x = blockIdx.x & 7, j = blockIdx.x >> 3;
        const int q = w.total >> 3, r = w.total & 7;
        const int lo = x < r ? x * (q + 1) : r * (q + 1) + (x - r) * q;
        const int cnt = q + (x < r ? 1 : 0);
        w_stride = (G - x + 7) >> 3;
        w_first = lo + j;
        w_count = j < cnt ? (int)((unsigned)(cnt - j + w_stride - 1) / (unsigned)w_stride) : 0;
    }
    if (w_count == 0) return;
    const int pairs = w_count * (w.nk >> 1);

    const unsigned lds0 = (unsigned)(uintptr_t)(lds_void_t*)smem;
    W4Addr ad;
    {
        const int ra = wr * 128 + (lane & 15), rb = wc * 128 + (lane & 15);
#pragma unroll
        for (int ks = 0; ks < 2; ++ks) {
            if (AKC) ad.adA[ks] = lds0 + (unsigned)(ra * 128 + ((((4 * ks + (lane >> 4)) ^ (ra >> 1)) & 7) << 4));
            if (BKC) ad.adB[ks] = lds0 + (unsigned)(W4_BREG + rb * 128 + ((((4 * ks + (lane >> 4)) ^ (rb >> 1)) & 7) << 4));
        }
        if (AKC) {
#pragma unroll
            for (int i = 2; i < 8; ++i) ad.adA[i] = 0;
        } else {
            const int li = lane & 15, g = lane >> 4;
            const int kk = 8 * g + (li >> 2);
            const int swz = ((kk & 3) << 1) | (((kk >> 3) & 1) << 3);
#pragma unroll
            for (int i = 0; i < 8; ++i) {
                const int col = wr * 128 + 16 * i + 4 * (li & 3);
                ad.adA[i] = lds0 + (unsigned)(kk * 512 + ((((col >> 3) ^ swz) & 31) << 4) + ((col >> 2) & 1) * 8);
            }
        }
        if (!BKC) {
            const int li = lane & 15, g = lane >> 4;
            const int kk = 8 * g + (li >> 2);
            const int swz = ((kk & 3) << 1) | (((kk >> 3) & 1) << 3);
#pragma unroll
            for (int j = 0; j < 8; ++j) {
                const int col = wc * 128 + 16 * j + 4 * (li & 3);
                ad.adB[j] = lds0 + (unsigned)(W4_BREG + kk * 512 + ((((col >> 3) ^ swz) & 31) << 4) + ((col >> 2) & 1) * 8);
            }
        } else {
#pragma unroll
            for (int j = 2; j < 8; ++j) ad.adB[j] = 0;
// ... 84 lines not shown
    int c_n = 0, c_kt = 0;
#define W4_KTILE(BUF, FRESH)                                                                                            \
    do {                                                                                                                \
        w4_h0<AKC, BKC, BUF, FRESH>(ad, rA, rB, s_koffA, s_koffB);                                                      \
        w4_h1<AKC, BKC, BUF, FRESH>(ad, rA, rB, s_koffA, s_koffB);                                                      \
        w4_h2<AKC, BKC, BUF, FRESH>(ad, rA, rB, s_koffA, s_koffB);                                                      \
        s_koffA += kstepA;                                                                                              \
        s_koffB += kstepB;                                                                                              \
        w4_h3<AKC, BKC, BUF>(ad);                                                                                       \
    } while (0)

    for (int it = 0; it < pairs; ++it) {
        if (c_kt == 0) W4_KTILE(0, true);
        else W4_KTILE(0, false);
        W4_KTILE(1, false);
        stager_pair_done();
        c_kt += 2;
        if (c_kt == w.nk) {
            if constexpr (EPI == PP_E_F32) {
                int m0, n0, batch = 0, split;
                float* tile;
                int64_t ldc;
                if (GROUPABLE && w.nprob) {
                    int q;
                    work_decode_grouped(w, w_first + c_n * w_stride, q, m0, n0, split);
                    const PPProblem& pr = w.prob[q];
                    ldc = pr.N;
                    tile = reinterpret_cast<float*>(p.C) + (int64_t)split * p.sSplit + pr.c_off + (int64_t)m0 * ldc + n0;
                } else {
                    work_decode(w, w_first + c_n * w_stride, m0, n0, batch, split);
                    ldc = p.ldc;
                    tile = reinterpret_cast<float*>(p.C) + (int64_t)batch * p.sC + (int64_t)split * p.sSplit + (int64_t)m0 * ldc + n0;
                }
                asm volatile("s_nop 15\n\ts_nop 15");
                w4_epilogue_f32(tile, ldc, wr * 128, wc * 128, lane);
                c_kt = 0;
                ++c_n;
                continue;
            }
            W4Tile et;
            int split;
            work_decode(w, w_first + c_n * w_stride, et.m0, et.n0, et.batch, split);
            et.mlim = w.M - et.m0;
            et.nlim = w.N - et.n0;
            et.cbase = reinterpret_cast<char*>(p.C) + ((int64_t)et.batch * p.sC + (int64_t)et.m0 * p.ldc + et.n0) * 2;
            et.c2base = (!w4_is_dact(EPI) && p.C2) ? reinterpret_cast<char*>(p.C2) + ((int64_t)et.batch * p.sC2 + (int64_t)et.m0 * p.ldc2 + et.n0) * 2 : nullptr;
            et.opbase = EPI == PP_E_RES   ? reinterpret_cast<const char*>(p.res) + ((int64_t)et.m0 * p.ldr + et.n0) * 2
                        : w4_is_dact(EPI) ? reinterpret_cast<const char*>(p.aux) + ((int64_t)et.batch * p.sAux + (int64_t)et.m0 * p.ldaux + et.n0) * 2
                                          : nullptr;
            et.gbase = (EPI == PP_E_RES && p.gate) ? reinterpret_cast<const char*>(p.gate) + (size_t)et.n0 * 2 : nullptr;
            asm volatile("s_nop 15\n\ts_nop 15");
#ifndef W4_X_NOEPI
            unsigned char* const slab = smem + 2 * W4_BREG + wave * W4_SLAB;
            if (et.mlim >= PT && et.nlim >= PT) w4_epilogue<EPI, true>(p, w, et, slab, wr * 128, wc * 128, lane);
            else w4_epilogue<EPI, false>(p, w, et, slab, wr * 128, wc * 128, lane);
#else
            asm volatile("s_waitcnt vmcnt(0)" ::: "memory");
#endif
            c_kt = 0;
            ++c_n;
        }
    }
    asm volatile("s_waitcnt vmcnt(0)" ::: "memory");
}

}

static bool w4_instantiated(int akc, int bkc, int epi) {
    if (!akc) return !bkc && epi == PP_E_F32;
    if (bkc) return epi == PP_E_BF16 || epi == PP_E_RES || epi == PP_E_DACT_GELU || epi == PP_E_DACT_MUL;
    return epi == PP_E_BF16 || epi == PP_E_BF16_GELU || epi == PP_E_BF16_GELU_D || epi == PP_E_RES || epi == PP_E_DACT_SWIGLU;
}

bool md_gemm_w4_eligible(const md_gemm_args* a) {
    const int epi = md_gemm_pp_epi_kind(a);
    if (epi < 0 || !w4_instantiated(a->a_kcontig, a->b_kcontig, epi)) return false;
    if (!md_gemm_pp_shape_ok(a, epi)) return false;
    if (epi == PP_E_DACT_SWIGLU && (!a->aux || a->batch != 1 || a->ldaux < 2 * a->N || a->ldc < 2 * a->N)) return false;
    if (a->A_list || a->B_list || a->timeline) return false;
    if (a->bias || a->alpha != 1.f) return false;
    const int64_t kspan = a->K / a->ksplit;
    if (epi == PP_E_F32) {
        if (a->ksplit > 1 && a->sSplit <= 0) return false;
        if (a->problems) {
            for (int i = 0; i < a->n_problems; ++i) {
                const md_gemm_problem& s = a->problems[i];
                if (s.M % PT || s.N % PT || kspan * (s.lda > s.ldb ? s.lda : s.ldb) >= ((int64_t)1 << 30)) return false;
            }
            return true;
        }
        if (a->M % PT || a->N % PT || a->ldc % 4) return false;
        return kspan * (a->lda > a->ldb ? a->lda : a->ldb) < ((int64_t)1 << 30);
    }
    if (a->ksplit != 1 || a->problems) return false;
    if (!a->b_kcontig && (a->K * a->ldb >= (int64_t)1 << 30)) return false;
    return true;
}

int md_gemm_w4_launch(const md_gemm_args* a, hipStream_t stream) {
    PPPlan w;
    if (!md_gemm_pp_plan(a, &w)) return MD_BAD_ARG;
    const int cus = (a->cu_limit > 0 && a->cu_limit < NUM_CU) ? a->cu_limit : NUM_CU;
    const unsigned G = (unsigned)(w.total < cus ? w.total : cus);
    if (a->tail_used) *a->tail_used = 0;
    const int epi = md_gemm_pp_epi_kind(a);
    const dim3 grid(G, 1, 1), block(256);
#define W4_LAUNCH(AK, BK, E) hipLaunchKernelGGL((gemm_bf16_w4_kernel<AK, BK, E>), grid, block, 0, stream, *a, w)
    if (!a->a_kcontig) {
        W4_LAUNCH(0, 0, PP_E_F32);
    } else if (a->b_kcontig) {
        if (epi == PP_E_BF16) W4_LAUNCH(1, 1, PP_E_BF16);
        else if (epi == PP_E_RES) W4_LAUNCH(1, 1, PP_E_RES);
        else if (epi == PP_E_DACT_MUL) W4_LAUNCH(1, 1, PP_E_DACT_MUL);
        else W4_LAUNCH(1, 1, PP_E_DACT_GELU);
    } else {
        if (epi == PP_E_BF16) W4_LAUNCH(1, 0, PP_E_BF16);
        else if (epi == PP_E_BF16_GELU) W4_LAUNCH(1, 0, PP_E_BF16_GELU);
        else if (epi == PP_E_BF16_GELU_D) W4_LAUNCH(1, 0, PP_E_BF16_GELU_D);
        else if (epi == PP_E_DACT_SWIGLU) W4_LAUNCH(1, 0, PP_E_DACT_SWIGLU);
        else W4_LAUNCH(1, 0, PP_E_RES);
    }
#undef W4_LAUNCH
    MD_LAUNCH_CHECK();
    return 0;
}
```

micro_diffusion_amd/csrc/norm.hip:

```cpp
#include "md_common.h"
#include "../../include/microdit_hip.h"

namespace {

constexpr int MAXCH = 4;

__device__ __forceinline__ float act_fwd(float v, int act) {
    if (act == MD_ACT_GELU_TANH) return gelu_tanh_f(v);
    if (act == MD_ACT_GELU_ERF) return gelu_erf_f(v);
    if (act == MD_ACT_SILU) return silu_f(v);
    return v;
}
__device__ __forceinline__ float act_bwd(float v, int act) {
    if (act == MD_ACT_GELU_TANH) return dgelu_tanh_f(v);
    if (act == MD_ACT_GELU_ERF) return dgelu_erf_f(v);
    if (act == MD_ACT_SILU) return dsilu_f(v);
    return 1.f;
}

template <int NCH, bool GENERIC, bool KEEP_RAW>
__device__ __forceinline__ void load_row(const md_ln_args& p, int64_t row, int lane, float (&v)[NCH][8],
                                         float (&raw)[KEEP_RAW ? NCH : 1][8]) {
    const bf16* xr = reinterpret_cast<const bf16*>(p.x) + row * p.ldx;
    const float* pr = (GENERIC && p.pos) ? reinterpret_cast<const float*>(p.pos) + (row % p.pos_rows) * p.C : nullptr;
// ... 301 lines not shown
__global__ __launch_bounds__(256) void ln_det_sum_kernel(const float* ws, int64_t nslices, float* out, int64_t ldo, int64_t C) {
    det_slice_sum(ws, nslices, out, ldo, C);
}

template <int NCH>
__global__ __launch_bounds__(256) void qkln_fwd_kernel(bf16* buf, int64_t rows, int64_t ld, int64_t col0, int C, int nseg,
                                                       int64_t seg_stride, float* rstd_out, float eps) {
    const int lane = threadIdx.x & 63;
    const int64_t wave = (int64_t)blockIdx.x * 4 + (threadIdx.x >> 6);
    const int64_t nwaves = (int64_t)gridDim.x * 4;
    const int64_t items = rows * nseg;
    const float invC = 1.f / (float)C;
    auto at = [&](int64_t vr) { return buf + (vr / nseg) * ld + col0 + (vr % nseg) * seg_stride; };
    bf16x8 nxt[NCH];
    if (wave < items) issue_row<NCH>(at(wave), C, lane, nxt);
    for (int64_t vr = wave; vr < items; vr += nwaves) {
        bf16* r = at(vr);
        float v[NCH][8];
        unpack_row<NCH>(nxt, v);
        if (vr + nwaves < items) issue_row<NCH>(at(vr + nwaves), C, lane, nxt);
        float s = 0.f;
#pragma unroll
        for (int j = 0; j < NCH; ++j)
#pragma unroll
            for (int e = 0; e < 8; ++e) s += v[j][e];
        const float mean = wave_sum(s) * invC;
        float q = 0.f;
#pragma unroll
        for (int j = 0; j < NCH; ++j) {
            const int c = lane * 8 + j * 512;
            if (c < C) {
#pragma unroll
                for (int e = 0; e < 8; ++e) {
                    const float d = v[j][e] - mean;
                    q += d * d;
                }
            }
        }
        const float rstd = rsqrtf(wave_sum(q) * invC + eps);
        if (lane == 0) rstd_out[(vr % nseg) * rows + vr / nseg] = rstd;
#pragma unroll
        for (int j = 0; j < NCH; ++j) {
            const int c = lane * 8 + j * 512;
            if (c < C) {
                bf16x8 o;
#pragma unroll
                for (int e = 0; e < 8; ++e) o[e] = f2bf((v[j][e] - mean) * rstd);
                st_bf16x8(r + c, o);
            }
        }
    }
}

template <int NCH>
__global__ __launch_bounds__(256) void qkln_bwd_kernel(bf16* d, int64_t ldd, int64_t dcol0, const bf16* y, int64_t ldy,
                                                       int64_t ycol0, int64_t rows, int C, int nseg, int64_t dseg_stride,
                                                       int64_t yseg_stride, const float* rstd_in) {
    const int lane = threadIdx.x & 63;
    const int64_t wave = (int64_t)blockIdx.x * 4 + (threadIdx.x >> 6);
    const int64_t nwaves = (int64_t)gridDim.x * 4;
    const int64_t items = rows * nseg;
    const float invC = 1.f / (float)C;
    auto dat = [&](int64_t vr) { return d + (vr / nseg) * ldd + dcol0 + (vr % nseg) * dseg_stride; };
    auto yat = [&](int64_t vr) { return y + (vr / nseg) * ldy + ycol0 + (vr % nseg) * yseg_stride; };
    bf16x8 ng[NCH], ny[NCH];
    float nrstd = 0.f;
    if (wave < items) {
        issue_row<NCH>(dat(wave), C, lane, ng);
        issue_row<NCH>(yat(wave), C, lane, ny);
        nrstd = rstd_in[(wave % nseg) * rows + wave / nseg];
    }
    for (int64_t vr = wave; vr < items; vr += nwaves) {
        bf16* dr = dat(vr);
        float g[NCH][8], xh[NCH][8];
        unpack_row<NCH>(ng, g);
        unpack_row<NCH>(ny, xh);
        const float rstd = nrstd;
        float s1 = 0.f, s2 = 0.f;
#pragma unroll
        for (int j = 0; j < NCH; ++j)
#pragma unroll
            for (int e = 0; e < 8; ++e) {
                s1 += g[j][e];
                s2 += g[j][e] * xh[j][e];
            }
        if (vr + nwaves < items) {
            const int64_t nx = vr + nwaves;
            issue_row<NCH>(dat(nx), C, lane, ng);
            issue_row<NCH>(yat(nx), C, lane, ny);
            nrstd = rstd_in[(nx % nseg) * rows + nx / nseg];
        }
        s1 = wave_sum(s1) * invC;
        s2 = wave_sum(s2) * invC;
#pragma unroll
        for (int j = 0; j < NCH; ++j) {
            const int c = lane * 8 + j * 512;
            if (c < C) {
                bf16x8 o;
#pragma unroll
                for (int e = 0; e < 8; ++e) o[e] = f2bf(rstd * (g[j][e] - s1 - xh[j][e] * s2));
                st_bf16x8(dr + c, o);
            }
        }
    }
}

struct HmMap {
    int64_t S, H;
    int hd_shift;
    __device__ __forceinline__ int64_t row_base(int64_t row) const {
        const int64_t b = row / S, s = row - b * S;
        return (b * H * S + s) << hd_shift;
    }
    __device__ __forceinline__ int64_t col_off(int c) const {
        return ((int64_t)(c >> hd_shift) * S << hd_shift) + (c & ((1 << hd_shift) - 1));
    }
};
template <int NCH>
__device__ __forceinline__ void issue_row_hm(const bf16* base, const HmMap& m, int C, int lane, bf16x8 (&h)[NCH]) {
#pragma unroll
    for (int j = 0; j < NCH; ++j) {
        const int c = lane * 8 + j * 512;
        if (c < C) h[j] = ld_bf16x8(base + m.col_off(c));
        else
#pragma unroll
            for (int e = 0; e < 8; ++e) h[j][e] = (bf16)0.f;
    }
}

template <int NCH>
__global__ __launch_bounds__(256) void qkln_fwd_hm_kernel(const bf16* buf, int64_t rows, int64_t ld, int64_t col0, int C, int nseg,
                                                          int64_t seg_stride, bf16* out, int64_t out_seg_stride, HmMap m,
                                                          float* rstd_out, float eps) {
    const int lane = threadIdx.x & 63;
    const int64_t wave = (int64_t)blockIdx.x * 4 + (threadIdx.x >> 6);
    const int64_t nwaves = (int64_t)gridDim.x * 4;
    const int64_t items = rows * nseg;
    const float invC = 1.f / (float)C;
    auto at = [&](int64_t vr) { return buf + (vr / nseg) * ld + col0 + (vr % nseg) * seg_stride; };
    bf16x8 nxt[NCH];
    if (wave < items) issue_row<NCH>(at(wave), C, lane, nxt);
    for (int64_t vr = wave; vr < items; vr += nwaves) {
        float v[NCH][8];
// ... 160 lines not shown
    md_ln_bwd_args k = *b;
    if (region > 0) {
        k.dscale = wsS;
        k.dshift = wsH;
    }
    dim3 grid((unsigned)chunks, (unsigned)nsmp, 1);
    const bool generic = a->act != MD_ACT_NONE || a->pos != nullptr;
#define LNB(N, G) hipLaunchKernelGGL((ln_bwd_kernel<N, G, true>), grid, dim3(256), 0, stream, *a, k)
    if (generic) {
        if (a->C <= 512) LNB(1, true); else if (a->C <= 1024) LNB(2, true); else LNB(4, true);
    } else {
        if (a->C <= 512) LNB(1, false); else if (a->C <= 1024) LNB(2, false); else LNB(4, false);
    }
#undef LNB
    if ((want_cols && region > 0) || (b->dscale && (b->dw || b->dscale_is_output)))
        hipLaunchKernelGGL(ln_det_finish_kernel, dim3((unsigned)((a->C + 255) / 256), (unsigned)groups), dim3(256), 0, stream, wsS, wsH,
                           chunks, reinterpret_cast<float*>(b->dscale), reinterpret_cast<float*>(b->dshift), b->ldg,
                           reinterpret_cast<const float*>(a->w), reinterpret_cast<const bf16*>(a->scale), a->ldmod,
                           reinterpret_cast<float*>(b->dw), wsW, nsmp, a->C, b->dscale_is_output);
    if (wsW)
        hipLaunchKernelGGL(ln_det_sum_kernel, dim3((unsigned)((a->C + 63) / 64), 1), dim3(256), 0, stream, wsW, groups,
                           reinterpret_cast<float*>(b->dw), (int64_t)0, a->C);
    MD_LAUNCH_CHECK();
    return 0;
}

extern "C" int md_qkln_fwd(void* buf, int64_t rows, int64_t ld, int64_t col0, int64_t width, int32_t nseg, int64_t seg_stride,
                           float* rstd_out, float eps, hipStream_t stream) {
    if (!buf || !rstd_out || rows <= 0 || width <= 0 || width % 8 || width > 64 * 8 * MAXCH || ld % 8 || col0 % 8 || nseg < 1 ||
        nseg > 4 || seg_stride % 8 || (nseg > 1 && seg_stride < width))
        return MD_BAD_ARG;
#define QKF(N) hipLaunchKernelGGL(qkln_fwd_kernel<N>, dim3(ln_grid(rows * nseg)), dim3(256), 0, stream, (bf16*)buf, rows, ld, \
                                  col0, (int)width, (int)nseg, seg_stride, rstd_out, eps)
    if (width <= 512) QKF(1); else if (width <= 1024) QKF(2); else QKF(4);
#undef QKF
    MD_LAUNCH_CHECK();
    return 0;
}

extern "C" int md_qkln_bwd(void* d, int64_t ldd, int64_t dcol0, const void* y, int64_t ldy, int64_t ycol0, int64_t rows,
                           int64_t width, int32_t nseg, int64_t dseg_stride, int64_t yseg_stride, const float* rstd,
                           hipStream_t stream) {
    if (!d || !y || !rstd || rows <= 0 || width <= 0 || width % 8 || width > 64 * 8 * MAXCH || ldd % 8 || ldy % 8 ||
        dcol0 % 8 || ycol0 % 8 || nseg < 1 || nseg > 4 || dseg_stride % 8 || yseg_stride % 8)
        return MD_BAD_ARG;
#define QKB(N) hipLaunchKernelGGL(qkln_bwd_kernel<N>, dim3(ln_grid(rows * nseg)), dim3(256), 0, stream, (bf16*)d, ldd, dcol0, \
                                  (const bf16*)y, ldy, ycol0, rows, (int)width, (int)nseg, dseg_stride, yseg_stride, rstd)
    if (width <= 512) QKB(1); else if (width <= 1024) QKB(2); else QKB(4);
#undef QKB
    MD_LAUNCH_CHECK();
    return 0;
}

namespace {
inline bool hm_ok(int64_t rows, int64_t width, int64_t S, int32_t hd) {
    return S > 0 && rows % S == 0 && (hd == 32 || hd == 64) && width % hd == 0;
}
}

extern "C" int md_qkln_fwd_hm(const void* buf, int64_t rows, int64_t ld, int64_t col0, int64_t width, int32_t nseg, int64_t seg_stride,
                              void* out, int64_t out_seg_stride, int64_t S, int32_t hd, float* rstd_out, float eps, hipStream_t stream) {
    if (!buf || !out || !rstd_out || rows <= 0 || width <= 0 || width % 8 || width > 64 * 8 * MAXCH || ld % 8 || col0 % 8 || nseg < 1 ||
        nseg > 4 || seg_stride % 8 || (nseg > 1 && (seg_stride < width || out_seg_stride < rows * width)) || out_seg_stride % 8 ||
        !hm_ok(rows, width, S, hd))
        return MD_BAD_ARG;
    const HmMap m{S, width / hd, hd == 64 ? 6 : 5};
#define QKF(N) hipLaunchKernelGGL(qkln_fwd_hm_kernel<N>, dim3(ln_grid(rows * nseg)), dim3(256), 0, stream, (const bf16*)buf, rows, ld, \
                                  col0, (int)width, (int)nseg, seg_stride, (bf16*)out, out_seg_stride, m, rstd_out, eps)
    if (width <= 512) QKF(1); else if (width <= 1024) QKF(2); else QKF(4);
#undef QKF
    MD_LAUNCH_CHECK();
    return 0;
}

extern "C" int md_qkln_bwd_hm(const void* dy, int64_t dy_seg_stride, const void* y, int64_t y_seg_stride, void* d, int64_t ldd,
                              int64_t dcol0, int64_t dseg_stride, int64_t rows, int64_t width, int32_t nseg, int64_t S, int32_t hd,
                              const float* rstd, hipStream_t stream) {
    if (!dy || !y || !d || !rstd || rows <= 0 || width <= 0 || width % 8 || width > 64 * 8 * MAXCH || ldd % 8 || dcol0 % 8 ||
        nseg < 1 || nseg > 4 || dseg_stride % 8 || dy_seg_stride % 8 || y_seg_stride % 8 || !hm_ok(rows, width, S, hd))
        return MD_BAD_ARG;
    const HmMap m{S, width / hd, hd == 64 ? 6 : 5};
#define QKB(N) hipLaunchKernelGGL(qkln_bwd_hm_kernel<N>, dim3(ln_grid(rows * nseg)), dim3(256), 0, stream, (const bf16*)dy, dy_seg_stride, \
                                  (const bf16*)y, y_seg_stride, (bf16*)d, ldd, dcol0, dseg_stride, rows, (int)width, (int)nseg, m, rstd)
    if (width <= 512) QKB(1); else if (width <= 1024) QKB(2); else QKB(4);
#undef QKB
    MD_LAUNCH_CHECK();
    return 0;
}
```

micro_diffusion_amd/engine.py:

```python
from __future__ import annotations

import ctypes
import math
import os
from ctypes import byref
from typing import Dict, List, Optional

import torch

from . import hip
from .arch import BlockPlan, DiTConfig, caption_ffn_hidden, plan_blocks

BF16, F32, I32 = torch.bfloat16, torch.float32, torch.int32
TAIL_WS_BYTES = 256 * 256 * 256 * 4


class Tape:
    pass


class _Arena:
    ALIGN = 256

    def __init__(self, dev):
# ... 54 lines not shown
            return self
        kv = {name: (k[:B * self.Lc], None if khm is None else khm[:B * self.Lc]) for name, (k, khm) in self.kv.items()}
        return Conditioning(B, self.Lc, self.head_major, self.version, self.pooled[:B], kv)


def _p(t):
    return None if t is None else t.data_ptr()


class DiTEngine:
    def __init__(self, cfg: DiTConfig, params: Dict[str, torch.Tensor], shadows: Dict[str, torch.Tensor],
                 grads: Dict[str, torch.Tensor], buffers: Dict[str, torch.Tensor]):
        self.cfg = cfg
        self.P, self.S, self.G, self.buf = params, shadows, grads, buffers
        self.mixer, self.backbone = plan_blocks(cfg)
        self.dev = next(iter(params.values())).device
        self.L = hip.lib()
        self.wgrad_target_blocks = 768
        self.gemm_profile = None
        self.kernel_profile = None
        self.gemm_prefer = hip.GEMM_AUTO
        self.attn_bwd_prefer = hip.ATTN_BWD_AUTO
        self.qk_head_major = os.environ.get("MD_QK_HEAD_MAJOR", "0") == "1"
        self.deterministic = os.environ.get("MD_DETERMINISTIC", "0") == "1"
        self._det_ws_floats = {}
        self.gemm_log = None
        self.before_segment = None
        self.keep_last_tape = False
        self.last_tape = None
        self.route_override = None
        self.route_stats = None
        self.ws = torch.empty(128 << 20, device=self.dev, dtype=F32)
        self.use_arena = False
        self._tape_arena, self._scratch_arena = _Arena(self.dev), _Arena(self.dev)
        self._arena = None
        self._record = False
        self._chosen = ctypes.c_int32(-1)
        self._ptr_cache = {}
        self.ksplit_min_items = 192
        self.splitk_force_pp = False
        self.short_k_accum = True
        self.group_wgrad = True
        self._wgroup = None
        self.single_slice_ws = True
        self.group_dycond = True
        self.group_adaln = True
        self._posb = None
        self.moe_cache_dact = True
        self.batch_adaln = True
        self._adaln = self._adaln_region()
        self.gemm_tail_mode = int(os.environ.get("MD_GEMM_TAIL", "0"))
        self.wgrad_bf16 = None
        self.fuse_swiglu_bwd = os.environ.get("MD_FUSE_SWIGLU_BWD", "1") != "0"
        self.weights_version = 0
        self.cu_limit_fn = None

    def _adaln_region(self):
        names = [bp.name for bp in self.mixer] + [bp.name for bp in self.backbone]
        col, n, w0, b0 = {}, 0, None, None
        for nm in names:
            w, b = self.S.get(nm + ".adaLN_modulation.1.weight"), self.P.get(nm + ".adaLN_modulation.1.bias")
            if w is None or b is None or w.dim() != 2 or w.shape[1] != self.cfg.dim:
                return None
            if w0 is None:
                w0, b0 = w, b
            elif w.data_ptr() != w0.data_ptr() + 2 * n * self.cfg.dim or b.data_ptr() != b0.data_ptr() + 4 * n:
                return None
            col[nm] = n
            n += w.shape[0]
        if w0 is None or n % 8:
            return None
        return {"N": n, "w": w0.data_ptr(), "b": b0.data_ptr(), "col": col}

    def _adaln_all(self, gc, B):
        r = self._adaln
        out = self.empty(B, r["N"])
        D = self.cfg.dim
        self._gemm(A=gc.data_ptr(), B=r["w"], C=out.data_ptr(), bias=r["b"], M=B, N=r["N"], K=D, lda=D, ldb=D, ldc=r["N"], batch=1, ksplit=1,
                   a_kcontig=1, b_kcontig=1, mode=hip.EPI_STORE_BF16, act=0, alpha=1.0)
        return out

    def _st(self):
        return torch.cuda.current_stream().cuda_stream

    def empty(self, *shape, dtype=BF16):
        if self._arena is not None:
            return self._arena.alloc(shape, dtype)
        return torch.empty(*shape, device=self.dev, dtype=dtype)

    def zeros(self, *shape, dtype=F32):
        t = self.empty(*shape, dtype=dtype)
        hip.check(self.L.md_fill_zero(t.data_ptr(), t.numel() * t.element_size(), self._st()), "md_fill_zero")
        return t

    def _prof(self, name, nbytes, launch):
        kp = self.kernel_profile
        if kp is None:
            return launch()
        e0, e1 = torch.cuda.Event(enable_timing=True), torch.cuda.Event(enable_timing=True)
        e0.record()
        launch()
        e1.record()
        kp.setdefault(name, []).append((e0, e1, float(nbytes)))

    def _det_ws(self, kind, rows, rps, rpb, C):
        key = (kind, rows, rps, rpb, C)
        n = self._det_ws_floats.get(key)
        if n is None:
            out = ctypes.c_int64(0)
            hip.check(self.L.md_det_ws_floats(kind, rows, rps, rpb, C, byref(out)), "md_det_ws_floats")
            n = self._det_ws_floats[key] = int(out.value)
        if n == 0:
            return None, 0
        return self.empty(n, dtype=F32).data_ptr(), n

    def _colsum(self, src_ptr, is_f32, ld, out_ptr, rows, C):
        nbytes = (4.0 if is_f32 else 2.0) * rows * C
        if not self.deterministic:
            return self._prof("colsum", nbytes, lambda: hip.check(self.L.md_colsum(src_ptr, is_f32, ld, out_ptr, rows, C, self._st()), "colsum"))
        ws, n = self._det_ws(hip.DET_COLSUM, rows, 0, 0, C)
        self._prof("colsum", nbytes,
                   lambda: hip.check(self.L.md_colsum_det(src_ptr, is_f32, ld, out_ptr, rows, C, ws, n, self._st()), "colsum_det"))

    def _gate_bwd(self, dx, br, gate_ptr, ldgate, dbr, dgate_ptr, lddg, M, d, S, rpb):
        if not self.deterministic:
            return self._prof("gate_bwd", 6.0 * M * d, lambda: hip.check(self.L.md_gate_bwd(
                dx.data_ptr(), br.data_ptr(), gate_ptr, ldgate, dbr.data_ptr(), dgate_ptr, lddg, M, d, S, rpb, self._st()), "gate_bwd"))
        ws, n = self._det_ws(hip.DET_GATE_BWD, M, S, rpb, d)
        self._prof("gate_bwd", 6.0 * M * d, lambda: hip.check(self.L.md_gate_bwd_det(
            dx.data_ptr(), br.data_ptr(), gate_ptr, ldgate, dbr.data_ptr(), dgate_ptr, lddg, M, d, S, rpb, ws, n, self._st()), "gate_bwd_det"))

    def _qkln_fwd(self, ptr, rows, ld, off, width, rstd_ptr, nseg=1):
        self._prof("qk_layernorm", 4.0 * rows * width * nseg, lambda: hip.check(
            self.L.md_qkln_fwd(ptr, rows, ld, off, width, nseg, width, rstd_ptr, self.cfg.norm_eps, self._st()), "md_qkln_fwd"))

    def _qkln_bwd(self, dptr, ldd, doff, yptr, ldy, yoff, rows, width, rstd_ptr, nseg=1):
        self._prof("qk_layernorm", 6.0 * rows * width * nseg, lambda: hip.check(
            self.L.md_qkln_bwd(dptr, ldd, doff, yptr, ldy, yoff, rows, width, nseg, width, width, rstd_ptr, self._st()), "md_qkln_bwd"))

    def _qkln_fwd_hm(self, ptr, rows, ld, off, width, out, S, rstd_ptr, nseg=1):
        self._prof("qk_layernorm", 4.0 * rows * width * nseg, lambda: hip.check(
            self.L.md_qkln_fwd_hm(ptr, rows, ld, off, width, nseg, width, out.data_ptr(), rows * width, S, self.cfg.head_dim, rstd_ptr,
                                  self.cfg.norm_eps, self._st()), "md_qkln_fwd_hm"))

    def _qkln_bwd_hm(self, dy, y, dptr, ldd, doff, rows, width, S, rstd_ptr, nseg=1):
        self._prof("qk_layernorm", 6.0 * rows * width * nseg, lambda: hip.check(
            self.L.md_qkln_bwd_hm(dy.data_ptr(), rows * width, y.data_ptr(), rows * width, dptr, ldd, doff, width, rows, width, nseg, S,
                                  self.cfg.head_dim, rstd_ptr, self._st()), "md_qkln_bwd_hm"))

    def _attn_fwd(self, a):
        nb = 2.0 * a.hd * (2 * a.Sq + 2 * a.Skv) * a.B * a.H
        self._prof("attention", nb, lambda: hip.check(self.L.md_attn_fwd(byref(a), self._st()), "md_attn_fwd"))

    def _gemm(self, **kw):
        a = hip.GemmArgs()
        problems = kw.pop("_problems", None)
        may_refuse = kw.pop("_try", False)
        for k, v in kw.items():
            setattr(a, k, v)
        if self.deterministic and a.mode == hip.EPI_ATOMIC_F32 and a.ksplit > 1:
            raise RuntimeError("deterministic mode: a split-K GEMM with the fp32-atomic epilogue sums in an order that changes from run "
                               "to run; use the workspace slices + md_splitk_reduce (gemm_f32_acc)")
        prof = self.gemm_profile
        if prof is not None:
            e0, e1 = torch.cuda.Event(enable_timing=True), torch.cuda.Event(enable_timing=True)
            e0.record()
        chosen = self._chosen
        a.chosen_variant = ctypes.addressof(chosen)
        if self.cu_limit_fn is not None:
            a.cu_limit = self.cu_limit_fn()
        if self.gemm_tail_mode != 1 and a.mode in (hip.EPI_STORE_BF16, hip.EPI_RESIDUAL, hip.EPI_DACT):
            a.tail_ws, a.tail_ws_bytes, a.tail_mode = self.ws.data_ptr(), TAIL_WS_BYTES, self.gemm_tail_mode
        rc = hip.NOT_ELIGIBLE
        want = self.gemm_prefer if self.gemm_prefer != hip.GEMM_AUTO else a.variant
        if want != hip.GEMM_AUTO:
            a.variant = want
            rc = self.L.md_gemm_bf16(byref(a), self._st())
            if rc == hip.NOT_ELIGIBLE:
                a.variant = hip.GEMM_AUTO
        if rc == hip.NOT_ELIGIBLE:
            rc = self.L.md_gemm_bf16(byref(a), self._st())
        if rc == hip.NOT_ELIGIBLE and may_refuse:
            return False
        hip.check(rc, "md_gemm_bf16")
        if self.gemm_log is not None:
            self.gemm_log.append((chosen.value, a.M, a.N, a.K, a.batch))
        if prof is not None:
            e1.record()
            out_b = 4 if a.mode in (hip.EPI_STORE_F32, hip.EPI_ACCUM_F32, hip.EPI_ATOMIC_F32) else 2
            mn = a.M * a.N * a.batch
            byt = 2.0 * (a.M * a.K + a.N * a.K) * a.batch + mn * out_b * a.ksplit
            byt += mn * 2 * ((1 if a.C2 else 0) + (1 if a.res else 0) + (1 if a.aux else 0)) + (mn * 4 if a.mode == hip.EPI_ACCUM_F32 else 0)
            if a.mode == hip.EPI_SWIGLU_BWD:
                byt += mn * 2 * 2
            fl = 2.0 * a.M * a.N * a.K * a.batch
            key = (a.M, a.N, a.K, a.batch, a.a_kcontig, a.b_kcontig, a.ksplit)
            if problems:
                mn = sum(g["M"] * g["N"] for g in problems)
                fl = 2.0 * mn * a.K
                byt = 2.0 * a.K * sum(g["M"] + g["N"] for g in problems) + mn * 4 * a.ksplit
                key = (-len(problems), mn // 1024, a.K, 1, 0, 0, a.ksplit)
            prof.append((e0, e1, fl, key, byt))
        return True

    def lin_fwd(self, x, wname, out, M, N, K, *, ldx=None, ldc=None, mode=hip.EPI_STORE_BF16, act=0, res=None,
                gate=None, ldg=0, rps=0, C2=None, ldc2=0, xoff=0, ooff=0, bias=True):
        b = self.P.get(wname + ".bias") if bias else None
        self._gemm(A=x.data_ptr() + 2 * xoff, B=self.S[wname + ".weight"].data_ptr(),
                   C=out.data_ptr() + (4 if mode in (hip.EPI_STORE_F32, hip.EPI_ACCUM_F32) else 2) * ooff,
                   C2=_p(C2), bias=_p(b), res=_p(res), gate=gate, M=M, N=N, K=K, lda=ldx or K, ldb=K, ldc=ldc or N,
                   ldc2=ldc2 or N, ldr=N, ldg=ldg, rows_per_sample=rps, batch=1, ksplit=1, a_kcontig=1, b_kcontig=1,
                   mode=mode, act=act, alpha=1.0)

    def lin_dgrad(self, dy, wname, dx, M, N, K, *, lddy=None, mode=hip.EPI_STORE_BF16, act=0, aux=None, res=None,
                  dyoff=0):
        self._gemm(A=dy.data_ptr() + 2 * dyoff, B=self.S[wname + ".weight"].data_ptr(), C=dx.data_ptr(), aux=_p(aux),
                   res=_p(res), M=M, N=K, K=N, lda=lddy or N, ldb=K, ldc=K, ldaux=K, ldr=K, batch=1, ksplit=1,
                   a_kcontig=1, b_kcontig=0, mode=mode, act=act, alpha=1.0)

    def _fused12(self, pre):
        w1, w2 = self.S.get(pre + ".w1.weight"), self.S.get(pre + ".w2.weight")
        if w1 is None or w2 is None or (pre + ".w1.bias") in self.P:
            return False
        return (w2.data_ptr() == w1.data_ptr() + w1.numel() * 2 and
                self.G[pre + ".w2.weight"].data_ptr() == self.G[pre + ".w1.weight"].data_ptr() + w1.numel() * 4)

    def _ksplit(self, out_rows, out_cols, contraction, batch=1):
        ws_cap = max(1, self.ws.numel() // (out_rows * out_cols * batch))
        t256 = ((out_rows + 255) // 256) * ((out_cols + 255) // 256) * batch
        if getattr(self, "short_k_accum", True) and contraction <= 512 and t256 >= 64:
            return 1
        if contraction % 128 == 0 and out_cols % 8 == 0:
            units = contraction // 128
# ... 127 lines not shown
                dst = t["gbf"] + (lo - t["g_lo"]) // 2
                self._prof("splitk_reduce", n * (4.0 * ks + 2), lambda lo=lo, n=n, dst=dst: hip.check(
                    self.L.md_splitk_reduce_flat(self.ws.data_ptr() + (lo - base), dst, n, span_el, ks, 2, self._st()), "md_splitk_reduce_flat"))
                continue
            self._prof("splitk_reduce", 4.0 * n * (ks + 2), lambda lo=lo, n=n: hip.check(
                self.L.md_splitk_reduce_flat(self.ws.data_ptr() + (lo - base), lo, n, span_el, ks, 1, self._st()), "md_splitk_reduce_flat"))

    def ln_args(self, x, wname, out, rows, C, *, shift=None, scale=None, ldmod=0, rps=0, mean=None, rstd=None, act=0,
                pos=None, pos_rows=0):
        return hip.LnArgs(x.data_ptr(), _p(self.P[wname + ".weight"]) if wname else None, shift, scale, _p(pos), _p(out),
                          _p(mean), _p(rstd), rows, C, C, C, ldmod, rps, pos_rows, self.cfg.norm_eps, act)

    def ln_fwd(self, a):
        self._prof("layernorm", 4.0 * a.rows * a.C, lambda: hip.check(self.L.md_ln_fwd(byref(a), self._st()), "md_ln_fwd"))

    @staticmethod
    def _rows_per_block(rows, rps, min_blocks=2048):
        rpb = 64
        while rpb > 4 and (rows + rpb - 1) // rpb < min_blocks:
            rpb //= 2
        return int(max(1, min(rpb, rps)))

    def ln_bwd(self, a, dz, dx, *, accumulate, wname=None, dscale=None, dshift=None, ldg=0):
        rps = a.rows_per_sample if a.rows_per_sample > 0 else a.rows
        rpb = self._rows_per_block(a.rows, rps, 1024)
        is_out = 1 if dscale is not None else 0
        if dscale is None and wname is not None:
            scratch = self.zeros(a.rows // rps, a.C)
            dscale, ldg = scratch.data_ptr(), a.C
        b = hip.LnBwdArgs(dz.data_ptr(), _p(dx), dscale, dshift, _p(self.G[wname + ".weight"]) if wname else None,
                          a.C, a.C, ldg, rpb, 1 if accumulate else 0, is_out)
        if self.deterministic:
            ws, n = self._det_ws(hip.DET_LN_BWD, a.rows, rps, rpb, a.C)
            self._prof("layernorm", (8.0 if accumulate else 6.0) * a.rows * a.C,
                       lambda: hip.check(self.L.md_ln_bwd_det(byref(a), byref(b), ws, n, self._st()), "md_ln_bwd_det"))
            return
        self._prof("layernorm", (8.0 if accumulate else 6.0) * a.rows * a.C,
                   lambda: hip.check(self.L.md_ln_bwd(byref(a), byref(b), self._st()), "md_ln_bwd"))

    def attn_args(self, q, k, v, o, lse, B, H, Sq, Skv, ldq, ldk, ldv, hid, *, do=None, dq=None, dk=None, dv=None,
                  delta=None, lddq=0, lddk=0, lddv=0, hm_qk=False):
        hd = self.cfg.head_dim
        a = hip.AttnArgs(q, k, v, _p(o), _p(lse), _p(do), dq, dk, dv, _p(delta), B, H, Sq, Skv, ldq, ldk, ldv, hid,
                         Sq * ldq, Skv * ldk, Skv * ldv, Sq * hid, lddq, lddk, lddv, hid, Sq * lddq, Skv * lddk,
                         Skv * lddv, Sq * hid, 1.0 / math.sqrt(hd), hd, 0)
        if hm_qk:
            a.ldq = a.ldk = a.lddq = a.lddk = hd
            a.sq = a.sdq = H * Sq * hd
            a.sk = a.sdk = H * Skv * hd
            a.hsq = a.hsdq = Sq * hd
            a.hsk = a.hsdk = Skv * hd
        return a

    def _attn_bwd(self, a):
        self._prof("attention", 2.0 * a.hd * (4 * a.Sq + 4 * a.Skv) * a.B * a.H, lambda: self._attn_bwd_launch(a))

    def _attn_bwd_launch(self, a):
        rc = -1
        if self.attn_bwd_prefer != hip.ATTN_BWD_AUTO:
            a.bwd_split = self.attn_bwd_prefer
            rc = self.L.md_attn_bwd(byref(a), self._st())
            a.bwd_split = hip.ATTN_BWD_AUTO
        if rc == -1:
            rc = self.L.md_attn_bwd(byref(a), self._st())
        hip.check(rc, "md_attn_bwd")

    def _self_attn_fwd(self, pre, xin, B, S, dim, hid, heads, t):
        M, L, st = B * S, self.L, self._st()
        qkv = self.empty(M, 3 * hid)
        self.lin_fwd(xin, pre + ".qkv", qkv, M, 3 * hid, dim)
        rq = self.empty(2, M, dtype=F32)
        o = self.empty(M, hid)
        lse = self.empty(B, heads, S, dtype=F32)
        if self.qk_head_major:
            t.qk = self.empty(2, M, hid)
            self._qkln_fwd_hm(qkv.data_ptr(), M, 3 * hid, 0, hid, t.qk, S, rq.data_ptr(), nseg=2)
            a = self.attn_args(t.qk.data_ptr(), t.qk.data_ptr() + 2 * M * hid, qkv.data_ptr() + 4 * hid, o, lse, B, heads, S, S,
                               0, 0, 3 * hid, hid, hm_qk=True)
        else:
            t.qk = None
            self._qkln_fwd(qkv.data_ptr(), M, 3 * hid, 0, hid, rq.data_ptr(), nseg=2)
            a = self.attn_args(qkv.data_ptr(), qkv.data_ptr() + 2 * hid, qkv.data_ptr() + 4 * hid, o, lse, B, heads, S, S,
                               3 * hid, 3 * hid, 3 * hid, hid)
        self._attn_fwd(a)
        t.qkv, t.rq, t.o, t.lse = qkv, rq, o, lse
        return o

    def _self_attn_bwd(self, pre, xin, do, B, S, dim, hid, heads, t, defer=False):
        M, L, st = B * S, self.L, self._st()
        dqkv = self.empty(M, 3 * hid)
        delta = self.empty(B, heads, S, dtype=F32)
        qkv = t.qkv
        if t.qk is not None:
            dqk = self.empty(2, M, hid)
            a = self.attn_args(t.qk.data_ptr(), t.qk.data_ptr() + 2 * M * hid, qkv.data_ptr() + 4 * hid, t.o, t.lse, B, heads, S, S,
                               0, 0, 3 * hid, hid, do=do, dq=dqk.data_ptr(), dk=dqk.data_ptr() + 2 * M * hid,
                               dv=dqkv.data_ptr() + 4 * hid, delta=delta, lddv=3 * hid, hm_qk=True)
            self._attn_bwd(a)
            self._qkln_bwd_hm(dqk, t.qk, dqkv.data_ptr(), 3 * hid, 0, M, hid, S, t.rq.data_ptr(), nseg=2)
        else:
            a = self.attn_args(qkv.data_ptr(), qkv.data_ptr() + 2 * hid, qkv.data_ptr() + 4 * hid, t.o, t.lse, B, heads, S, S,
                               3 * hid, 3 * hid, 3 * hid, hid, do=do, dq=dqkv.data_ptr(), dk=dqkv.data_ptr() + 2 * hid,
                               dv=dqkv.data_ptr() + 4 * hid, delta=delta, lddq=3 * hid, lddk=3 * hid, lddv=3 * hid)
            self._attn_bwd(a)
            self._qkln_bwd(dqkv.data_ptr(), 3 * hid, 0, qkv.data_ptr(), 3 * hid, 0, M, hid, t.rq.data_ptr(), nseg=2)
        self.lin_wgrad(dqkv, xin, pre + ".qkv", M, 3 * hid, dim, defer=defer)
        dxin = self.empty(M, dim)
        self.lin_dgrad(dqkv, pre + ".qkv", dxin, M, 3 * hid, dim)
        return dxin

    def _kv_linear_fwd(self, n, ycond, Mc, hx, d):
        kv = self.empty(Mc, 2 * hx)
        self.lin_fwd(ycond, n + ".cross_attn.kv_linear", kv, Mc, 2 * hx, d)
        return kv

    def _k_norm_fwd(self, kv, Mc, hx, Lc):
        rk = self.empty(Mc, dtype=F32)
        if self.qk_head_major:
            kn = self.empty(Mc, hx)
            self._qkln_fwd_hm(kv.data_ptr(), Mc, 2 * hx, 0, hx, kn, Lc, rk.data_ptr())
            return rk, kn
        self._qkln_fwd(kv.data_ptr(), Mc, 2 * hx, 0, hx, rk.data_ptr())
        return rk, None

    def _block_fwd(self, bp: BlockPlan, x, ycond, B, S, Lc, gc, mod_all=None, kv=None):
        L, st, cfg = self.L, self._st(), self.cfg
        d, h, hx, f = bp.dim, bp.attn_hidden, bp.xattn_hidden, bp.ffn_hidden
        M, Mc, D = B * S, B * Lc, cfg.dim
        n = bp.name
        t = Tape()
        t.x = x
        if mod_all is not None:
            mod, ldm = mod_all, mod_all.shape[1]
            mp = mod_all.data_ptr() + 2 * self._adaln["col"][n]
        else:
            mod, ldm = self.empty(B, 6 * d), 6 * d
            self.lin_fwd(gc, n + ".adaLN_modulation.1", mod, B, 6 * d, D)
            mp = mod.data_ptr()
        t.mod, t.mp, t.ldm = mod, mp, ldm
        t.xm1 = self.empty(M, d)
        t.st1 = self.empty(2, M, dtype=F32)
        a1 = self.ln_args(x, n + ".norm1", t.xm1, M, d, shift=mp, scale=mp + 2 * d, ldmod=ldm, rps=S, mean=t.st1[0], rstd=t.st1[1])
        self.ln_fwd(a1)
        t.sa = Tape()
        o = self._self_attn_fwd(n + ".attn", t.xm1, B, S, d, h, bp.heads, t.sa)
        t.br1 = self.empty(M, d)
        x1 = self.empty(M, d)
        self.lin_fwd(o, n + ".attn.proj", x1, M, d, h, mode=hip.EPI_RESIDUAL, res=x, gate=mp + 2 * 2 * d, ldg=ldm, rps=S,
                     C2=t.br1)
        t.x1 = x1
        t.xn2 = self.empty(M, d)
        t.st2 = self.empty(2, M, dtype=F32)
        self.ln_fwd(self.ln_args(x1, n + ".norm2", t.xn2, M, d, mean=t.st2[0], rstd=t.st2[1]))
        t.o2 = self.empty(M, hx)
        t.q2 = t.o2 if self.qk_head_major else self.empty(M, hx)
        self.lin_fwd(t.xn2, n + ".cross_attn.q_linear", t.q2, M, hx, d)
        if kv is None:
            t.kv = self._kv_linear_fwd(n, ycond, Mc, hx, d)
        else:
            t.kv, t.k2n = kv
            t.rk2 = None
        t.rq2 = self.empty(M, dtype=F32)
        t.lse2 = self.empty(B, bp.xheads, S, dtype=F32)
        if self.qk_head_major:
            t.q2n = self.empty(M, hx)
            self._qkln_fwd_hm(t.q2.data_ptr(), M, hx, 0, hx, t.q2n, S, t.rq2.data_ptr())
            if kv is None:
                t.rk2, t.k2n = self._k_norm_fwd(t.kv, Mc, hx, Lc)
            ax = self.attn_args(t.q2n.data_ptr(), t.k2n.data_ptr(), t.kv.data_ptr() + 2 * hx, t.o2, t.lse2, B, bp.xheads, S, Lc,
                                0, 0, 2 * hx, hx, hm_qk=True)
        else:
            t.q2n = None
            self._qkln_fwd(t.q2.data_ptr(), M, hx, 0, hx, t.rq2.data_ptr())
            if kv is None:
                t.rk2, t.k2n = self._k_norm_fwd(t.kv, Mc, hx, Lc)
            ax = self.attn_args(t.q2.data_ptr(), t.kv.data_ptr(), t.kv.data_ptr() + 2 * hx, t.o2, t.lse2, B, bp.xheads, S, Lc,
                                hx, 2 * hx, 2 * hx, hx)
        self._attn_fwd(ax)
        x2 = self.empty(M, d)
        self.lin_fwd(t.o2, n + ".cross_attn.proj", x2, M, d, hx, mode=hip.EPI_RESIDUAL, res=x1)
        t.x2 = x2
        t.xm3 = self.empty(M, d)
        t.st3 = self.empty(2, M, dtype=F32)
        self.ln_fwd(self.ln_args(x2, n + ".norm3", t.xm3, M, d, shift=mp + 2 * 3 * d, scale=mp + 2 * 4 * d, ldmod=ldm,
                                 rps=S, mean=t.st3[0], rstd=t.st3[1]))
        x3 = self.empty(M, d)
        t.br3 = self.empty(M, d)
        gate_mlp = mp + 2 * 5 * d
        if not bp.moe:
            t.h12 = self.empty(M, 2 * f)
            if self._fused12(n + ".mlp"):
                self.lin_fwd(t.xm3, n + ".mlp.w1", t.h12, M, 2 * f, d)
            else:
                self.lin_fwd(t.xm3, n + ".mlp.w1", t.h12, M, f, d, ldc=2 * f)
                self.lin_fwd(t.xm3, n + ".mlp.w2", t.h12, M, f, d, ldc=2 * f, ooff=f)
            t.a = self.empty(M, f)
            self._prof("swiglu", 6.0 * M * f, lambda: hip.check(L.md_swiglu_fwd(t.h12.data_ptr(), 2 * f, t.a.data_ptr(), f, M, f, st), "swiglu"))
            self.lin_fwd(t.a, n + ".mlp.w3", x3, M, d, f, mode=hip.EPI_RESIDUAL, res=x2, gate=gate_mlp, ldg=ldm, rps=S,
                         C2=t.br3)
        else:
            E = cfg.num_experts
            k = int(cfg.expert_capacity * S / E)
            ldl = 8 if E <= 8 else 16
            Bk = B * k
            t.k, t.ldl = k, ldl
            logits = self.empty(M, ldl, dtype=F32)
            self.lin_fwd(t.xm3, n + ".mlp.gate", logits, M, E, d, ldc=ldl, mode=hip.EPI_STORE_F32)
            t.probs = self.empty(M, ldl, dtype=F32)
            t.rowidx = self.empty(E, Bk, dtype=I32)
            t.gval = self.empty(E, Bk, dtype=F32)
            t.slot = self.empty(M, E, dtype=I32)
            hip.check(L.md_moe_route(logits.data_ptr(), t.probs.data_ptr(), ldl, B, S, E, k, t.rowidx.data_ptr(),
                                     t.gval.data_ptr(), t.slot.data_ptr(), st), "moe_route")
            if self.route_override is not None and n in self.route_override:
                self._override_routing(t, self.route_override[n], B, S, E, k)
            if self.route_stats is not None:
                self.route_stats.record(n, t.slot, t.probs, ldl, t.gval, B, S, k)
            t.xin = self.empty(E, Bk, d)
            hip.check(L.md_gather_rows(t.xm3.data_ptr(), d, t.rowidx.data_ptr(), t.xin.data_ptr(), d, E * Bk, d, st), "gather")
            t.hpre = self.empty(E, Bk, f)
            t.hact = self.empty(E, Bk, f)
            t.hpre_is_dact = 1 if self.moe_cache_dact else 0
            w1, w2 = self.S[n + ".mlp.w1"], self.S[n + ".mlp.w2"]
            self._gemm(A=t.xin.data_ptr(), B=w1.data_ptr(), C=t.hact.data_ptr(), C2=t.hpre.data_ptr(), M=Bk, N=f, K=d, lda=d,
                       ldb=f, ldc=f, ldc2=f, sA=Bk * d, sB=d * f, sC=Bk * f, sC2=Bk * f, batch=E, ksplit=1, a_kcontig=1,
                       b_kcontig=0, mode=hip.EPI_STORE_BF16, act=hip.ACT_GELU_ERF, alpha=1.0, dact_cached=t.hpre_is_dact)
            t.h2 = self.empty(E, Bk, d)
            self._gemm(A=t.hact.data_ptr(), B=w2.data_ptr(), C=t.h2.data_ptr(), M=Bk, N=d, K=f, lda=f, ldb=d, ldc=d,
                       sA=Bk * f, sB=f * d, sC=Bk * d, batch=E, ksplit=1, a_kcontig=1, b_kcontig=0, mode=hip.EPI_STORE_BF16,
                       act=0, alpha=1.0)
            hip.check(L.md_moe_combine(t.h2.data_ptr(), t.gval.data_ptr(), t.slot.data_ptr(), x2.data_ptr(), gate_mlp, ldm,
# ... 37 lines not shown
            if self._fused12(n + ".mlp"):
                self.lin_wgrad(dh12, t.xm3, n + ".mlp.w1", M, 2 * f, d, defer=True)
                self.lin_dgrad(dh12, n + ".mlp.w1", dxm3, M, 2 * f, d)
            else:
                self.lin_wgrad(dh12, t.xm3, n + ".mlp.w1", M, f, d, lddy=2 * f, defer=True)
                self.lin_wgrad(dh12, t.xm3, n + ".mlp.w2", M, f, d, lddy=2 * f, dyoff=f, defer=True)
                self.lin_dgrad(dh12, n + ".mlp.w1", dxm3, M, f, d, lddy=2 * f)
                self.lin_dgrad(dh12, n + ".mlp.w2", dxm3, M, f, d, lddy=2 * f, dyoff=f, mode=hip.EPI_RESIDUAL, res=dxm3)
        else:
            E, k, ldl = cfg.num_experts, t.k, t.ldl
            Bk = B * k
            w1, w2 = self.S[n + ".mlp.w1"], self.S[n + ".mlp.w2"]
            g1, g2 = self.G[n + ".mlp.w1"], self.G[n + ".mlp.w2"]
            dh2 = self.empty(E, Bk, d)
            dgval = self.empty(E, Bk, dtype=F32)
            hip.check(L.md_moe_combine_bwd(dbr3.data_ptr(), t.h2.data_ptr(), t.rowidx.data_ptr(), t.gval.data_ptr(),
                                           dh2.data_ptr(), dgval.data_ptr(), E * Bk, d, st), "combine_bwd")
            self.gemm_f32_acc(out_ptr=g2.data_ptr(), M=f, N=d, K=Bk, ldo=d, batch=E, sOut=f * d, A=t.hact.data_ptr(),
                              B=dh2.data_ptr(), lda=f, ldb=d, sA=Bk * f, sB=Bk * d, a_kcontig=0, b_kcontig=0)
            dhpre = self.empty(E, Bk, f)
            self._gemm(A=dh2.data_ptr(), B=w2.data_ptr(), C=dhpre.data_ptr(), aux=t.hpre.data_ptr(), M=Bk, N=f, K=d, lda=d,
                       ldb=d, ldc=f, ldaux=f, sA=Bk * d, sB=f * d, sC=Bk * f, sAux=Bk * f, batch=E, ksplit=1, a_kcontig=1,
                       b_kcontig=1, mode=hip.EPI_DACT, act=hip.ACT_GELU_ERF, alpha=1.0, dact_cached=t.hpre_is_dact)
            self.gemm_f32_acc(out_ptr=g1.data_ptr(), M=d, N=f, K=Bk, ldo=f, batch=E, sOut=d * f, A=t.xin.data_ptr(),
                              B=dhpre.data_ptr(), lda=d, ldb=f, sA=Bk * d, sB=Bk * f, a_kcontig=0, b_kcontig=0)
            dxin = self.empty(E, Bk, d)
            self._gemm(A=dhpre.data_ptr(), B=w1.data_ptr(), C=dxin.data_ptr(), M=Bk, N=d, K=f, lda=f, ldb=f, ldc=d, sA=Bk * f,
                       sB=d * f, sC=Bk * d, batch=E, ksplit=1, a_kcontig=1, b_kcontig=1, mode=hip.EPI_STORE_BF16, act=0, alpha=1.0)
            dlog = self.empty(M, ldl)
            hip.check(L.md_moe_dispatch_bwd(dxin.data_ptr(), t.slot.data_ptr(), dxm3.data_ptr(), t.probs.data_ptr(), ldl,
                                            dgval.data_ptr(), dlog.data_ptr(), ldl, B, S, E, k, d, st), "dispatch_bwd")
            self.lin_wgrad(dlog, t.xm3, n + ".mlp.gate", M, E, d, lddy=ldl)
            self.lin_dgrad(dlog, n + ".mlp.gate", dxm3, M, E, d, lddy=ldl, mode=hip.EPI_RESIDUAL, res=dxm3)
        a3 = self.ln_args(t.x2, n + ".norm3", None, M, d, scale=mp + 2 * 4 * d, ldmod=ldm, rps=S, mean=t.st3[0], rstd=t.st3[1])
        self.ln_bwd(a3, dxm3, dx, accumulate=True, wname=n + ".norm3", dscale=dmp + 4 * 4 * d, dshift=dmp + 4 * 3 * d, ldg=6 * d)
        self.lin_wgrad(dx, t.o2, n + ".cross_attn.proj", M, d, hx, defer=True)
        do2 = self.empty(M, hx)
        self.lin_dgrad(dx, n + ".cross_attn.proj", do2, M, d, hx)
        dq2 = self.empty(M, hx)
        dkv = self.empty(Mc, 2 * hx) if kvgroup is None else kvgroup["buf"][len(kvgroup["w"])]
        delta = self.empty(B, bp.xheads, S, dtype=F32)
        if t.q2n is not None:
            dq2n, dk2n = self.empty(M, hx), self.empty(Mc, hx)
            ax = self.attn_args(t.q2n.data_ptr(), t.k2n.data_ptr(), t.kv.data_ptr() + 2 * hx, t.o2, t.lse2, B, bp.xheads, S, Lc, 0,
                                0, 2 * hx, hx, do=do2, dq=dq2n.data_ptr(), dk=dk2n.data_ptr(), dv=dkv.data_ptr() + 2 * hx,
                                delta=delta, lddv=2 * hx, hm_qk=True)
            self._attn_bwd(ax)
            self._qkln_bwd_hm(dq2n, t.q2n, dq2.data_ptr(), hx, 0, M, hx, S, t.rq2.data_ptr())
            self._qkln_bwd_hm(dk2n, t.k2n, dkv.data_ptr(), 2 * hx, 0, Mc, hx, Lc, t.rk2.data_ptr())
        else:
            ax = self.attn_args(t.q2.data_ptr(), t.kv.data_ptr(), t.kv.data_ptr() + 2 * hx, t.o2, t.lse2, B, bp.xheads, S, Lc, hx,
                                2 * hx, 2 * hx, hx, do=do2, dq=dq2.data_ptr(), dk=dkv.data_ptr(), dv=dkv.data_ptr() + 2 * hx,
                                delta=delta, lddq=hx, lddk=2 * hx, lddv=2 * hx)
            self._attn_bwd(ax)
            self._qkln_bwd(dq2.data_ptr(), hx, 0, t.q2.data_ptr(), hx, 0, M, hx, t.rq2.data_ptr())
            self._qkln_bwd(dkv.data_ptr(), 2 * hx, 0, t.kv.data_ptr(), 2 * hx, 0, Mc, hx, t.rk2.data_ptr())
        self.lin_wgrad(dq2, t.xn2, n + ".cross_attn.q_linear", M, hx, d, defer=True)
        self.lin_wgrad(dkv, ycond, n + ".cross_attn.kv_linear", Mc, 2 * hx, d)
        if kvgroup is None:
            self.gemm_f32_acc(out_ptr=dycond_f32.data_ptr(), M=Mc, N=d, K=2 * hx, ldo=d, A=dkv.data_ptr(),
                              B=self.S[n + ".cross_attn.kv_linear.weight"].data_ptr(), lda=2 * hx, ldb=d, a_kcontig=1, b_kcontig=0)
        else:
            kvgroup["w"].append(self.S[n + ".cross_attn.kv_linear.weight"].data_ptr())
        dxn2 = self.empty(M, d)
        self.lin_dgrad(dq2, n + ".cross_attn.q_linear", dxn2, M, hx, d)
        self._wgrad_flush()
        a2 = self.ln_args(t.x1, n + ".norm2", None, M, d, mean=t.st2[0], rstd=t.st2[1], rps=S)
        self.ln_bwd(a2, dxn2, dx, accumulate=True, wname=n + ".norm2")
        dbr1 = self.empty(M, d)
        self._gate_bwd(dx, t.br1, mp + 2 * 2 * d, ldm, dbr1, dmp + 4 * 2 * d, 6 * d, M, d, S, rpb)
        self.lin_wgrad(dbr1, t.sa.o, n + ".attn.proj", M, d, h, defer=True)
        do = self.empty(M, h)
        self.lin_dgrad(dbr1, n + ".attn.proj", do, M, d, h)
        dxm1 = self._self_attn_bwd(n + ".attn", t.xm1, do, B, S, d, h, bp.heads, t.sa, defer=True)
        self._wgrad_flush()
        a1 = self.ln_args(t.x, n + ".norm1", None, M, d, scale=mp + 2 * d, ldmod=ldm, rps=S, mean=t.st1[0], rstd=t.st1[1])
        self.ln_bwd(a1, dxm1, dx, accumulate=True, wname=n + ".norm1", dscale=dmp + 4 * d, dshift=dmp, ldg=6 * d)
        self._wgroup = None
        self._adaln_bwd(n + ".adaLN_modulation.1", dmod, B, 6 * d, gc, dgc_f32, group)

    def _adaln_bwd(self, wname, dmod_f32, B, N, gc, dgc_f32, group=None):
        D = self.cfg.dim
        if group is not None:
            i = len(group["w"])
            dmod = group["buf"][i]
        else:
            dmod = self.empty(B, N)
        hip.check(self.L.md_cast_f32_bf16(dmod_f32.data_ptr(), dmod.data_ptr(), B * N, None, self._st()), "cast")
        self.lin_wgrad(dmod, gc, wname, B, N, D, bias_from=dmod_f32)
        if group is not None:
            group["w"].append(self.S[wname + ".weight"].data_ptr())
            return
        self.gemm_f32_acc(out_ptr=dgc_f32.data_ptr(), M=B, N=D, K=N, ldo=D, A=dmod.data_ptr(),
                          B=self.S[wname + ".weight"].data_ptr(), lda=N, ldb=D, a_kcontig=1, b_kcontig=0)

    def _dycond_grouped(self, group, Mc, d, K, out_f32):
        G = len(group["w"])
        if G == 0:
            return
        t256 = ((Mc + 255) // 256) * ((d + 255) // 256)
        if K % 128 or d % 8 or Mc * d > self.ws.numel():
            for i in range(G):
                self.gemm_f32_acc(out_ptr=out_f32.data_ptr(), M=Mc, N=d, K=K, ldo=d, A=group["buf"][i].data_ptr(), B=group["w"][i],
                                  lda=K, ldb=d, a_kcontig=1, b_kcontig=0)
            return
        out_us = Mc * d * 4 / 4e6
        best, best_cost = 1, None
        for ks in range(1, G + 1):
            if G % ks or ks * Mc * d > self.ws.numel():
# ... 465 lines not shown
```

micro_diffusion_amd/hip.py:

```python
from __future__ import annotations

import ctypes
import os
from ctypes import c_float, c_int, c_int32, c_int64, c_void_p, POINTER, Structure, byref

from . import native

_CSRC = native.CSRC
_HEADER = os.path.join(native.INCLUDE, "microdit_hip.h")
LIB_PATH = os.path.join(os.path.dirname(_CSRC), "libmicrodit_hip.so")

HIPCC_FLAGS = ["--offload-arch=gfx950", "-O3", "-std=c++17", "-fPIC", "-munsafe-fp-atomics",
               "-Wno-unused-result", "-Wno-inline-asm"]

ACT_NONE, ACT_GELU_TANH, ACT_GELU_ERF, ACT_SILU = 0, 1, 2, 3
EPI_STORE_BF16, EPI_RESIDUAL, EPI_STORE_F32, EPI_ACCUM_F32, EPI_ATOMIC_F32, EPI_DACT, EPI_SWIGLU_BWD = 0, 1, 2, 3, 4, 5, 6
DET_GATE_BWD, DET_LN_BWD, DET_COLSUM = 0, 1, 2
GEMM_AUTO, GEMM_REG128, GEMM_DMA128, GEMM_PACED256, GEMM_PP256, GEMM_W4 = 0, 1, 2, 3, 4, 5
GEMM_VARIANT_NAMES = {"auto": 0, "reg128": 1, "dma128": 2, "paced256": 3, "pp256": 4, "w4": 5}
ATTN_BWD_AUTO, ATTN_BWD_FUSED_1PHASE, ATTN_BWD_FUSED_2PHASE, ATTN_BWD_FUSED_2PHASE_SPLIT, ATTN_BWD_STREAM_PAIR = 0, 2, 3, 4, 5


def _hashed_files():
    return [os.path.join(_CSRC, f) for f in sorted(os.listdir(_CSRC)) if os.path.isfile(os.path.join(_CSRC, f))] + [_HEADER]
# ... 65 lines not shown
                raise RuntimeError(
                    f"{LIB_PATH} is missing: the MicroDiT HIP extension has not been built. "
                    "Run `python -c 'import __graft_entry__ as g; g.build()'` (needs hipcc). "
                    "There is no CPU / PyTorch fallback for the training path.")
            path = LIB_PATH
        _lib = native.load(path, _SIGS, "md_abi_version", ABI_VERSION)
    return _lib


NOT_ELIGIBLE = -2


def check(code: int, what: str) -> None:
    if code != 0:
        why = {-1: "bad argument", NOT_ELIGIBLE: "forced kernel variant not eligible for this problem"}.get(code, "hipError_t")
        raise RuntimeError(f"{what} failed with code {code} ({why})")


_SIGS = {"md_abi_version": (c_int, [])}


def _sig(name, *argtypes):
    _SIGS[name] = (c_int, list(argtypes))


P, I64, I32, F32 = c_void_p, c_int64, c_int32, c_float

class LnArgs(Structure):
    _fields_ = [("x", c_void_p), ("w", c_void_p), ("shift", c_void_p), ("scale", c_void_p), ("pos", c_void_p),
                ("out", c_void_p), ("mean", c_void_p), ("rstd", c_void_p),
                ("rows", c_int64), ("C", c_int64), ("ldx", c_int64), ("ldo", c_int64), ("ldmod", c_int64),
                ("rows_per_sample", c_int64), ("pos_rows", c_int64), ("eps", c_float), ("act", c_int32)]


class LnBwdArgs(Structure):
    _fields_ = [("dz", c_void_p), ("dx", c_void_p), ("dscale", c_void_p), ("dshift", c_void_p), ("dw", c_void_p),
                ("lddz", c_int64), ("lddx", c_int64), ("ldg", c_int64), ("rows_per_block", c_int64),
                ("accumulate", c_int32), ("dscale_is_output", c_int32)]


class AttnArgs(Structure):
    _fields_ = [("q", c_void_p), ("k", c_void_p), ("v", c_void_p), ("o", c_void_p), ("lse", c_void_p),
                ("d_o", c_void_p), ("dq", c_void_p), ("dk", c_void_p), ("dv", c_void_p), ("delta", c_void_p),
                ("B", c_int64), ("H", c_int64), ("Sq", c_int64), ("Skv", c_int64),
                ("ldq", c_int64), ("ldk", c_int64), ("ldv", c_int64), ("ldo", c_int64),
                ("sq", c_int64), ("sk", c_int64), ("sv", c_int64), ("so", c_int64),
                ("lddq", c_int64), ("lddk", c_int64), ("lddv", c_int64), ("lddo", c_int64),
                ("sdq", c_int64), ("sdk", c_int64), ("sdv", c_int64), ("sdo", c_int64),
                ("scale", c_float), ("hd", c_int32), ("bwd_split", c_int32),
                ("hsq", c_int64), ("hsk", c_int64), ("hsv", c_int64), ("hso", c_int64),
                ("hsdq", c_int64), ("hsdk", c_int64), ("hsdv", c_int64), ("hsdo", c_int64)]


class AdamWArgs(Structure):
    _fields_ = [("p", c_void_p), ("g", c_void_p), ("m", c_void_p), ("v", c_void_p), ("shadow", c_void_p),
                ("sumsq", c_void_p), ("g_bf16", c_void_p), ("ema", c_void_p), ("n", c_int64),
                ("lr", c_float), ("beta1", c_float), ("beta2", c_float), ("eps", c_float), ("weight_decay", c_float),
                ("bias_corr1", c_float), ("bias_corr2", c_float), ("max_norm", c_float), ("grad_scale", c_float),
                ("ema_smoothing", c_float), ("zero_grad", c_int32), ("ema_mode", c_int32)]


SUMSQ_PARTIALS = 1024
STATS_ITEM_MAX = 65536


class StatsItem(Structure):
    _fields_ = [("src_off", c_int64), ("count", c_int32), ("tensor", c_int32)]


class LoraItem(Structure):
    _fields_ = [("w_off", c_int64), ("a_off", c_int64), ("b_off", c_int64), ("ws_off", c_int64), ("rows", c_int32), ("cols", c_int32)]


_sig("md_gemm_bf16", POINTER(GemmArgs), P)
_sig("md_splitk_reduce_flat", P, P, I64, I64, I32, I32, P)
_sig("md_splitk_reduce", P, P, I64, I64, I64, I64, I32, I32, I32, P)
_sig("md_ln_fwd", POINTER(LnArgs), P)
_sig("md_ln_bwd", POINTER(LnArgs), POINTER(LnBwdArgs), P)
_sig("md_qkln_fwd", P, I64, I64, I64, I64, I32, I64, P, F32, P)
_sig("md_qkln_bwd", P, I64, I64, P, I64, I64, I64, I64, I32, I64, I64, P, P)
_sig("md_qkln_fwd_hm", P, I64, I64, I64, I64, I32, I64, P, I64, I64, I32, P, F32, P)
_sig("md_qkln_bwd_hm", P, I64, P, I64, P, I64, I64, I64, I64, I64, I32, I64, I32, P, P)
_sig("md_attn_fwd", POINTER(AttnArgs), P)
_sig("md_attn_bwd", POINTER(AttnArgs), P)
_sig("md_swiglu_fwd", P, I64, P, I64, I64, I64, P)
_sig("md_swiglu_bwd", P, I64, P, I64, P, I64, I64, I64, P)
_sig("md_gate_bwd", P, P, P, I64, P, P, I64, I64, I64, I64, I64, P)
_sig("md_act_fwd", P, P, I64, I32, P)
_sig("md_act_bwd", P, P, P, I64, I32, P)
_sig("md_colsum", P, I32, I64, P, I64, I64, P)
_sig("md_cast_f32_bf16", P, P, I64, P, P)
_sig("md_cast_f32_bf16_clear", P, P, I64, P)
_sig("md_cast_rows_bf16", P, I32, P, I64, I64, P, I64, P)
_sig("md_mean_tokens", P, P, I64, I64, I64, P)
_sig("md_mean_tokens_bwd", P, P, I64, I64, I64, P)
_sig("md_add_bf16", P, P, P, I64, P)
_sig("md_fill_zero", P, I64, P)
_sig("md_get_mask", P, I64, I64, I64, P, P, P, P)
_sig("md_gather_rows", P, I64, P, P, I64, I64, I64, P)
_sig("md_scatter_rows", P, I64, P, P, I64, I64, I64, P)
_sig("md_moe_route", P, P, I64, I64, I64, I32, I32, P, P, P, P)
_sig("md_moe_combine", P, P, P, P, P, I64, P, P, I64, I64, I32, I32, I64, P)
_sig("md_moe_combine_bwd", P, P, P, P, P, P, I64, I64, P)
_sig("md_moe_dispatch_bwd", P, P, P, P, I64, P, P, I64, I64, I64, I32, I32, I64, P)
_sig("md_edm_prepare", P, P, P, P, P, P, P, I64, I64, F32, F32, F32, P)
_sig("md_edm_prepare_f16", P, P, P, P, P, P, P, P, I64, I64, F32, F32, F32, P)
_sig("md_patchify", P, P, P, I64, I32, I32, I32, I32, P)
_sig("md_timestep_embed", P, P, I64, I32, P)
_sig("md_unpatchify", P, P, I64, P, P, I64, I32, I32, I32, I32, P)
_sig("md_edm_loss", P, P, P, P, P, P, P, P, I64, I64, I32, I32, I32, I32, F32, P)
_sig("md_edm_loss_train", P, P, P, P, P, P, P, P, F32, P, F32, I64, I64, I32, I32, I32, I32, F32, P)
_sig("md_logvar_fwd", P, P, P, P, P, P, I64, I32, P)
_sig("md_edm_loss_train_weighted", P, P, P, P, P, P, P, P, F32, P, F32, I64, I64, I32, I32, I32, I32, F32, P, P)
_sig("md_logvar_bwd", P, P, P, P, P, F32, P, P, P, F32, I64, I32, P)
_sig("md_edm_sampler_input", P, P, I64, F32, F32, I32, P)
_sig("md_edm_heun_update", P, P, P, P, P, I64, F32, I32, ctypes.c_double, ctypes.c_double, ctypes.c_double, F32, I32, P)
_sig("md_edm_sampler_patchify", P, P, I64, I32, I32, I32, I32, F32, F32, I32, P)
_sig("md_edm_heun_update_tok", P, P, P, P, P, I64, I32, I32, I32, I32, F32, I32, ctypes.c_double, ctypes.c_double, ctypes.c_double, F32, I32, P)
_sig("md_edm_solver_update", P, P, P, P, I64, F32, I32, ctypes.c_double, F32, ctypes.c_double, ctypes.c_double, ctypes.c_double, ctypes.c_double, P)
_sig("md_edm_solver_update_tok", P, P, P, P, I64, I32, I32, I32, I32, F32, I32, ctypes.c_double, F32, ctypes.c_double, ctypes.c_double,
     ctypes.c_double, ctypes.c_double, P)
_sig("md_edm_churn", P, P, P, I64, ctypes.c_double, P)
_sig("md_edm_blend_known", P, P, P, P, I64, I32, I64, I32, ctypes.c_double, P)
_sig("md_edm_heun_update_guide", P, P, P, P, P, P, I64, F32, ctypes.c_double, ctypes.c_double, ctypes.c_double, F32, I32, P)
_sig("md_edm_solver_update_guide", P, P, P, P, P, I64, F32, ctypes.c_double, F32, ctypes.c_double, ctypes.c_double, ctypes.c_double,
     ctypes.c_double, P)
_sig("md_edm_heun_update_guide_tok", P, P, P, P, P, P, I64, I32, I32, I32, I32, F32, ctypes.c_double, ctypes.c_double, ctypes.c_double, F32,
     I32, P)
_sig("md_edm_solver_update_guide_tok", P, P, P, P, P, I64, I32, I32, I32, I32, F32, ctypes.c_double, F32, ctypes.c_double, ctypes.c_double,
     ctypes.c_double, ctypes.c_double, P)
_sig("md_sumsq", P, I32, I64, P, P)
_sig("md_sumsq_finish", P, I64, P, P)
_sig("md_checksum_u16", P, I64, P, P)
_sig("md_adamw_step", POINTER(AdamWArgs), P)
_sig("md_adamw_step_ranges", POINTER(AdamWArgs), P, P, I32, P)
_sig("md_tensor_stats_partial", P, I32, P, I64, P, P, P, P)
_sig("md_tensor_stats_finish", P, P, P, P, I32, P, P, P, P)
# ... 75 lines not shown
```

Baseline: 2812 images/sec.

## Fuse QK-LayerNorm stats into QKV GEMM epilogue and normalize inside attention

```diff
diff --git a/include/microdit_hip.h b/include/microdit_hip.h
--- a/include/microdit_hip.h
+++ b/include/microdit_hip.h
@@ -83,6 +83,16 @@
 };
 
 int md_gemm_bf16(const md_gemm_args* args, hipStream_t stream);
+
+typedef struct md_gemm_rowstats {
+    float* stats;
+    int64_t col0[2];
+    int64_t width[2];
+    int32_t nseg;
+} md_gemm_rowstats;
+int md_gemm_bf16_rowstats(const md_gemm_args* args, const md_gemm_rowstats* rs, hipStream_t stream);
+int md_qk_stats_finish(const float* partial, int64_t rows, int64_t nslab, int64_t col0, int64_t width, int32_t nseg, int64_t seg_stride,
+                       float* out, float eps, hipStream_t stream);
 int md_splitk_reduce(const float* ws, float* out, int64_t M, int64_t N, int64_t ldo, int64_t sOut, int32_t ksplit,
                      int32_t batch, int32_t accumulate, hipStream_t stream);
 
@@ -122,6 +132,8 @@
                 float* rstd_out, float eps, hipStream_t stream);
 int md_qkln_bwd(void* d, int64_t ldd, int64_t dcol0, const void* y, int64_t ldy, int64_t ycol0, int64_t rows,
                 int64_t width, int32_t nseg, int64_t dseg_stride, int64_t yseg_stride, const float* rstd, hipStream_t stream);
+int md_qkln_bwd_raw(void* d, int64_t ldd, int64_t dcol0, const void* y, int64_t ldy, int64_t ycol0, int64_t rows,
+                    int64_t width, int32_t nseg, int64_t dseg_stride, int64_t yseg_stride, const float* stats, hipStream_t stream);
 
 int md_qkln_fwd_hm(const void* buf, int64_t rows, int64_t ld, int64_t col0, int64_t width, int32_t nseg, int64_t seg_stride,
                    void* out, int64_t out_seg_stride, int64_t S, int32_t hd, float* rstd_out, float eps, hipStream_t stream);
@@ -156,6 +168,13 @@
 
 int md_attn_fwd(const md_attn_args* a, hipStream_t stream);
 int md_attn_bwd(const md_attn_args* a, hipStream_t stream);
+typedef struct md_attn_ln {
+    const float* q_stats;
+    const float* k_stats;
+    int64_t q_stride, k_stride;
+} md_attn_ln;
+int md_attn_fwd_ln(const md_attn_args* a, const md_attn_ln* n, hipStream_t stream);
+int md_attn_bwd_ln(const md_attn_args* a, const md_attn_ln* n, hipStream_t stream);
 
 int md_swiglu_fwd(const void* h12, int64_t ldh, void* a, int64_t lda, int64_t M, int64_t f, hipStream_t stream);
 int md_swiglu_bwd(const void* da, int64_t ldda, const void* h12, int64_t ldh, void* dh12, int64_t lddh, int64_t M, int64_t f,
diff --git a/micro_diffusion_amd/csrc/attention.hip b/micro_diffusion_amd/csrc/attention.hip
--- a/micro_diffusion_amd/csrc/attention.hip
+++ b/micro_diffusion_amd/csrc/attention.hip
@@ -43,26 +43,45 @@
     }
 }
 
+__device__ __forceinline__ u32x4 ln8(u32x4 raw, float2 ms) {
+    const bf16x8 x = __builtin_bit_cast(bf16x8, raw);
+    bf16x8 o;
+#pragma unroll
+    for (int e = 0; e < 8; ++e) o[e] = f2bf((bf2f(x[e]) - ms.x) * ms.y);
+    return __builtin_bit_cast(u32x4, o);
+}
+__device__ __forceinline__ float2 ln_stat(const float* stats, int64_t stride, int64_t row, bool ok) {
+    return (stats && ok) ? *reinterpret_cast<const float2*>(stats + row * stride) : make_float2(0.f, 1.f);
+}
+
 constexpr int STG = 32;
 
-template <int HD, int MAXIT>
+template <int HD, int MAXIT, bool NORM = false>
 __device__ __forceinline__ void stage_pair(unsigned char* tileA, unsigned char* tileB, int pitch, const bf16* A, int64_t lda, const bf16* B,
-                                           int64_t ldb, int64_t row0, int64_t nrows, int nstage, int tid, int nthreads) {
+                                           int64_t ldb, int64_t row0, int64_t nrows, int nstage, int tid, int nthreads,
+                                           const float* statsA = nullptr, int64_t strideA = 0) {
     constexpr int CPR = HD / 8;
     uint4 ra[MAXIT], rb[MAXIT];
+    float2 sa[MAXIT];
 #pragma unroll
     for (int it = 0; it < MAXIT; ++it) {
         const int task = tid + it * nthreads, r = task / CPR, c = task % CPR;
         ra[it] = rb[it] = make_uint4(0, 0, 0, 0);
-        if (task < nstage * CPR && row0 + r < nrows) {
+        const bool ok = task < nstage * CPR && row0 + r < nrows;
+        if (ok) {
             ra[it] = *reinterpret_cast<const uint4*>(A + (row0 + r) * lda + c * 8);
             rb[it] = *reinterpret_cast<const uint4*>(B + (row0 + r) * ldb + c * 8);
         }
+        if (NORM) sa[it] = ln_stat(statsA, strideA, row0 + r, ok);
     }
 #pragma unroll
     for (int it = 0; it < MAXIT; ++it) {
         const int task = tid + it * nthreads, r = task / CPR, c = task % CPR;
         if (task < nstage * CPR) {
+            if (NORM) {
+                const u32x4 nv = ln8(u32x4{ra[it].x, ra[it].y, ra[it].z, ra[it].w}, sa[it]);
+                ra[it] = make_uint4(nv.x, nv.y, nv.z, nv.w);
+            }
             *reinterpret_cast<uint4*>(tileA + r * pitch + c * 16) = ra[it];
             *reinterpret_cast<uint4*>(tileB + r * pitch + c * 16) = rb[it];
         }
@@ -148,8 +167,8 @@
         }
 }
 
-template <int HD, int MAXIT>
-__global__ __launch_bounds__(256) void attn_fwd_kernel(md_attn_args p) {
+template <int HD, int MAXIT, bool NORM>
+__device__ __forceinline__ void attn_fwd_body(const md_attn_args p, const md_attn_ln nl) {
     constexpr int PK = (HD + 8) * 2;
     __shared__ __attribute__((aligned(16))) unsigned char smem[2 * STG * PK];
     const int tid = threadIdx.x, lane = tid & 63, wave = tid >> 6, nthreads = blockDim.x, nw = nthreads >> 6;
@@ -162,8 +181,11 @@
     const bf16* Q = reinterpret_cast<const bf16*>(p.q) + b * p.sq + h * p.hsq;
     const bf16* K = reinterpret_cast<const bf16*>(p.k) + b * p.sk + h * p.hsk;
     const bf16* V = reinterpret_cast<const bf16*>(p.v) + b * p.sv + h * p.hsv;
+    const float* KS = (NORM && nl.k_stats) ? nl.k_stats + b * p.Skv * nl.k_stride : nullptr;
 
     bf16x8 qf[HD / 16];
+    float2 qms = make_float2(0.f, 1.f);
+    if (NORM) qms = ln_stat(nl.q_stats, nl.q_stride, b * p.Sq + q, qvalid);
 #pragma unroll
     for (int s = 0; s < HD / 16; ++s) {
         if (qvalid)
@@ -171,6 +193,7 @@
         else
 #pragma unroll
             for (int e = 0; e < 8; ++e) qf[s][e] = f2bf(0.f);
+        if (NORM) qf[s] = __builtin_bit_cast(bf16x8, ln8(__builtin_bit_cast(u32x4, qf[s]), qms));
     }
     f32x16 oacc[HD / 32];
 #pragma unroll
@@ -182,7 +205,7 @@
     for (int64_t kbase = 0; kbase < p.Skv; kbase += STG) {
         __syncthreads();
         const int nst = (int)((p.Skv - kbase >= STG) ? STG : ((p.Skv - kbase + 31) / 32) * 32);
-        stage_pair<HD, MAXIT>(smem, smem + STG * PK, PK, K, p.ldk, V, p.ldv, kbase, p.Skv, nst, tid, nthreads);
+        stage_pair<HD, MAXIT, NORM>(smem, smem + STG * PK, PK, K, p.ldk, V, p.ldv, kbase, p.Skv, nst, tid, nthreads, KS, nl.k_stride);
         __syncthreads();
       for (int sub = 0; sub < STG / 32 && kbase + sub * 32 < p.Skv; ++sub) {
         const int64_t key0 = kbase + sub * 32;
@@ -233,6 +256,15 @@
         store_rows<HD>(O, oacc, 1.f / l, lane);
         if (lane < 32 && p.lse) reinterpret_cast<float*>(p.lse)[(b * p.H + h) * p.Sq + q] = (m + __log2f(l)) * 0.6931471805599453f;
     }
+}
+
+template <int HD, int MAXIT>
+__global__ __launch_bounds__(256) void attn_fwd_kernel(md_attn_args p) {
+    attn_fwd_body<HD, MAXIT, false>(p, md_attn_ln{nullptr, nullptr, 0, 0});
+}
+template <int HD, int MAXIT>
+__global__ __launch_bounds__(256) void attn_fwd_ln_kernel(md_attn_args p, md_attn_ln nl) {
+    attn_fwd_body<HD, MAXIT, true>(p, nl);
 }
 
 
@@ -563,8 +595,8 @@
     }
 }
 
-template <int HD, int SQP, int SKP>
-__global__ __launch_bounds__((SQP > SKP ? SQP : SKP) * 2) void attn_bwd_fused_kernel(md_attn_args p) {
+template <int HD, int SQP, int SKP, bool NORM>
+__device__ __forceinline__ void attn_bwd_fused_body(const md_attn_args p, const md_attn_ln nl) {
     constexpr int PK = (HD + 8) * 2;
     __shared__ __attribute__((aligned(16))) unsigned char smem[(2 * SQP + 2 * SKP) * PK + 2 * SQP * 4];
     unsigned char* sQ = smem;
@@ -592,6 +624,7 @@
         const float* LSE = reinterpret_cast<const float*>(p.lse) + (b * p.H + h) * p.Sq;
         u32x4 rq[ITQ], rdo[ITQ], ro[ITQ], rk[ITK], rv[ITK];
         float rl[ITQ];
+        float2 mq[ITQ], mk[ITK];
         const u32x4 z4 = {0u, 0u, 0u, 0u};
 #pragma unroll
         for (int it = 0; it < ITQ; ++it) {
@@ -601,6 +634,7 @@
             rdo[it] = ok ? *reinterpret_cast<const u32x4*>(dO + (int64_t)r * p.lddo + c * 8) : z4;
             ro[it] = ok ? *reinterpret_cast<const u32x4*>(O + (int64_t)r * p.ldo + c * 8) : z4;
             rl[it] = (ok && c == 0) ? LSE[r] : 0.f;
+            if (NORM) mq[it] = ln_stat(nl.q_stats, nl.q_stride, b * p.Sq + r, ok);
         }
 #pragma unroll
         for (int it = 0; it < ITK; ++it) {
@@ -608,10 +642,12 @@
             const bool ok = task < SKP * CPR && r < p.Skv;
             rk[it] = ok ? *reinterpret_cast<const u32x4*>(K + (int64_t)r * p.ldk + c * 8) : z4;
             rv[it] = ok ? *reinterpret_cast<const u32x4*>(V + (int64_t)r * p.ldv + c * 8) : z4;
+            if (NORM) mk[it] = ln_stat(nl.k_stats, nl.k_stride, b * p.Skv + r, ok);
         }
 #pragma unroll
         for (int it = 0; it < ITQ; ++it) {
             const int task = tid + it * NT, r = task / CPR, c = task % CPR;
+            if (NORM) rq[it] = ln8(rq[it], mq[it]);
             if (task < SQP * CPR) {
                 *reinterpret_cast<u32x4*>(sQ + r * PK + c * 16) = rq[it];
                 *reinterpret_cast<u32x4*>(sdO + r * PK + c * 16) = rdo[it];
@@ -630,6 +666,7 @@
 #pragma unroll
         for (int it = 0; it < ITK; ++it) {
             const int task = tid + it * NT, r = task / CPR, c = task % CPR;
+            if (NORM) rk[it] = ln8(rk[it], mk[it]);
             if (task < SKP * CPR) {
                 *reinterpret_cast<u32x4*>(sK + r * PK + c * 16) = rk[it];
                 *reinterpret_cast<u32x4*>(sV + r * PK + c * 16) = rv[it];
@@ -740,9 +777,17 @@
     }
 }
 
-template <int HD, int SQP, int SKP, bool SPLIT2>
-__global__ __launch_bounds__((SQP > SKP ? SQP : SKP) * 2) __attribute__((amdgpu_waves_per_eu(SPLIT2 ? 4 : 3)))
-void attn_bwd_fused2_kernel(md_attn_args p) {
+template <int HD, int SQP, int SKP>
+__global__ __launch_bounds__((SQP > SKP ? SQP : SKP) * 2) void attn_bwd_fused_kernel(md_attn_args p) {
+    attn_bwd_fused_body<HD, SQP, SKP, false>(p, md_attn_ln{nullptr, nullptr, 0, 0});
+}
+template <int HD, int SQP, int SKP>
+__global__ __launch_bounds__((SQP > SKP ? SQP : SKP) * 2) void attn_bwd_fused_ln_kernel(md_attn_args p, md_attn_ln nl) {
+    attn_bwd_fused_body<HD, SQP, SKP, true>(p, nl);
+}
+
+template <int HD, int SQP, int SKP, bool SPLIT2, bool NORM>
+__device__ __forceinline__ void attn_bwd_fused2_body(const md_attn_args p, const md_attn_ln nl) {
     constexpr int PK = (HD + 8) * 2;
     constexpr int RMAX = SQP > SKP ? SQP : SKP;
     constexpr int NT = RMAX * 2;
@@ -770,6 +815,7 @@
         const float* LSE = reinterpret_cast<const float*>(p.lse) + (b * p.H + h) * p.Sq;
         u32x4 rq[ITQ], rdo[ITQ], ro[ITQ];
         float rl[ITQ];
+        float2 mq[ITQ], mk[ITK];
         const u32x4 z4 = {0u, 0u, 0u, 0u};
 #pragma unroll
         for (int it = 0; it < ITQ; ++it) {
@@ -779,6 +825,7 @@
             rdo[it] = ok ? *reinterpret_cast<const u32x4*>(dO + (int64_t)r * p.lddo + c * 8) : z4;
             ro[it] = ok ? *reinterpret_cast<const u32x4*>(O + (int64_t)r * p.ldo + c * 8) : z4;
             rl[it] = (ok && c == 0) ? LSE[r] : 0.f;
+            if (NORM) mq[it] = ln_stat(nl.q_stats, nl.q_stride, b * p.Sq + r, ok);
         }
 #pragma unroll
         for (int it = 0; it < ITK; ++it) {
@@ -786,10 +833,12 @@
             const bool ok = task < SKP * CPR && r < p.Skv;
             rk[it] = ok ? *reinterpret_cast<const u32x4*>(K + (int64_t)r * p.ldk + c * 8) : z4;
             rv[it] = ok ? *reinterpret_cast<const u32x4*>(V + (int64_t)r * p.ldv + c * 8) : z4;
+            if (NORM) mk[it] = ln_stat(nl.k_stats, nl.k_stride, b * p.Skv + r, ok);
         }
 #pragma unroll
         for (int it = 0; it < ITQ; ++it) {
             const int task = tid + it * NT, r = task / CPR, c = task % CPR;
+            if (NORM) rq[it] = ln8(rq[it], mq[it]);
             if (task < SQP * CPR) {
                 *reinterpret_cast<u32x4*>(sA + r * PK + c * 16) = rq[it];
                 *reinterpret_cast<u32x4*>(sB + r * PK + c * 16) = rdo[it];
@@ -803,6 +852,13 @@
             if (c == 0 && task < SQP * CPR) {
                 sDlt[r] = d;
                 sLse[r] = rl[it] * LOG2E;
+            }
+        }
+        if (NORM) {
+#pragma unroll
+            for (int it = 0; it < ITK; ++it) {
+                rk[it] = ln8(rk[it], mk[it]);
+                asm volatile("" : "+v"(rk[it]));
             }
         }
     }
@@ -995,14 +1051,35 @@
     }
 }
 
+template <int HD, int SQP, int SKP, bool SPLIT2>
+__global__ __launch_bounds__((SQP > SKP ? SQP : SKP) * 2) __attribute__((amdgpu_waves_per_eu(SPLIT2 ? 4 : 3)))
+void attn_bwd_fused2_kernel(md_attn_args p) {
+    attn_bwd_fused2_body<HD, SQP, SKP, SPLIT2, false>(p, md_attn_ln{nullptr, nullptr, 0, 0});
+}
+template <int HD, int SQP, int SKP, bool SPLIT2>
+__global__ __launch_bounds__((SQP > SKP ? SQP : SKP) * 2) __attribute__((amdgpu_waves_per_eu(SPLIT2 ? 4 : 3)))
+void attn_bwd_fused2_ln_kernel(md_attn_args p, md_attn_ln nl) {
+    attn_bwd_fused2_body<HD, SQP, SKP, SPLIT2, true>(p, nl);
+}
+
 inline int fused_bucket(int64_t S) { return S <= 64 ? 64 : S <= 96 ? 96 : S <= 256 ? 256 : 0; }
 
-template <int HD>
-void launch_bwd_fused_one(const md_attn_args* a, int variant, int bq, int bk, hipStream_t stream) {
+template <int HD, bool NORM>
+void launch_bwd_fused_one(const md_attn_args* a, const md_attn_ln& nl, int variant, int bq, int bk, hipStream_t stream) {
     const dim3 grid((unsigned)a->H, (unsigned)a->B);
-#define FUSED(SQP, SKP) hipLaunchKernelGGL((attn_bwd_fused_kernel<HD, SQP, SKP>), grid, dim3((SQP > SKP ? SQP : SKP) * 2), 0, stream, *a)
-#define FUSED2(SQP, SKP, SPL) \
-    hipLaunchKernelGGL((attn_bwd_fused2_kernel<HD, SQP, SKP, SPL>), grid, dim3((SQP > SKP ? SQP : SKP) * 2), 0, stream, *a)
+#define FUSED(SQP, SKP)                                                                                                              \
+    do {                                                                                                                             \
+        const dim3 blk((SQP > SKP ? SQP : SKP) * 2);                                                                                 \
+        if constexpr (NORM) hipLaunchKernelGGL((attn_bwd_fused_ln_kernel<HD, SQP, SKP>), grid, blk, 0, stream, *a, nl);              \
+        else hipLaunchKernelGGL((attn_bwd_fused_kernel<HD, SQP, SKP>), grid, blk, 0, stream, *a);                                    \
+    } while (0)
+#define FUSED2(SQP, SKP, SPL)                                                                                                        \
+    do {                                                                                                                             \
+        const dim3 blk((SQP > SKP ? SQP : SKP) * 2);                                                                                 \
+        if constexpr (!NORM) hipLaunchKernelGGL((attn_bwd_fused2_kernel<HD, SQP, SKP, SPL>), grid, blk, 0, stream, *a);              \
+        else if constexpr (HD == 64 && !(SPL)) hipLaunchKernelGGL((attn_bwd_fused_ln_kernel<HD, SQP, SKP>), grid, blk, 0, stream, *a, nl); \
+        else hipLaunchKernelGGL((attn_bwd_fused2_ln_kernel<HD, SQP, SKP, SPL>), grid, blk, 0, stream, *a, nl);                       \
+    } while (0)
 #define SMALL(SQP, SKP)                          \
     do {                                         \
         if (variant == 2 || (variant == 0 && SQP == 64 && SKP == 64)) FUSED(SQP, SKP); \
@@ -1030,10 +1107,11 @@
 }
 
 template <int HD>
-bool launch_bwd_fused(const md_attn_args* a, int variant, hipStream_t stream) {
+bool launch_bwd_fused(const md_attn_args* a, const md_attn_ln* nl, int variant, hipStream_t stream) {
     const int bq = fused_bucket(a->Sq), bk = fused_bucket(a->Skv);
     if (!bq || !bk) return false;
-    launch_bwd_fused_one<HD>(a, variant, bq, bk, stream);
+    if (nl) launch_bwd_fused_one<HD, true>(a, *nl, variant, bq, bk, stream);
+    else launch_bwd_fused_one<HD, false>(a, md_attn_ln{nullptr, nullptr, 0, 0}, variant, bq, bk, stream);
     return true;
 }
 
@@ -1088,15 +1166,18 @@
     return c;
 }
 
-}
-
-extern "C" int md_attn_fwd(const md_attn_args* a_in, hipStream_t stream) {
+inline bool ln_ok(const md_attn_ln* n) {
+    return n && (n->q_stats || n->k_stats) && (!n->q_stats || (n->q_stride >= 2 && n->q_stride % 2 == 0 && (uintptr_t)n->q_stats % 8 == 0)) &&
+           (!n->k_stats || (n->k_stride >= 2 && n->k_stride % 2 == 0 && (uintptr_t)n->k_stats % 8 == 0));
+}
+
+int attn_fwd_impl(const md_attn_args* a_in, const md_attn_ln* nl, hipStream_t stream) {
     if (!attn_ok(a_in)) return MD_BAD_ARG;
     const md_attn_args args = with_head_strides(a_in);
     const md_attn_args* a = &args;
     static const bool fwd_stream = [] { const char* e = getenv("MD_ATTN_FWD_STREAM"); return !e || atoi(e) != 0; }();
     static const int fwd_stream_min = [] { const char* e = getenv("MD_ATTN_FWD_STREAM_MIN_SKV"); return e ? atoi(e) : 257; }();
-    if (fwd_stream && a->Skv >= fwd_stream_min && a->Sq >= 192) {
+    if (!nl && fwd_stream && a->Skv >= fwd_stream_min && a->Sq >= 192) {
         int nw = stream_waves(a->Sq);
         if (nw < 6) nw = 6;
         const dim3 grid((unsigned)((a->Sq + 32 * nw - 1) / (32 * nw)), (unsigned)a->H, (unsigned)a->B), blk(64 * nw);
@@ -1119,14 +1200,48 @@
         else if (chunks == 2) hipLaunchKernelGGL((attn_fwd_kernel<HD_, 2>), grid, dim3(64 * nw), 0, stream, *a);   \
         else hipLaunchKernelGGL((attn_fwd_kernel<HD_, 4>), grid, dim3(64 * nw), 0, stream, *a);                    \
     } while (0)
-    if (a->hd == 64) FWD(64);
-    else FWD(32);
+#define FWD_LN(HD_)                                                                                                        \
+    do {                                                                                                                    \
+        const int chunks = (32 * (HD_ / 8) + 64 * nw - 1) / (64 * nw);                                                      \
+        if (chunks <= 1) hipLaunchKernelGGL((attn_fwd_ln_kernel<HD_, 1>), grid, dim3(64 * nw), 0, stream, *a, *nl);         \
+        else if (chunks == 2) hipLaunchKernelGGL((attn_fwd_ln_kernel<HD_, 2>), grid, dim3(64 * nw), 0, stream, *a, *nl);    \
+        else hipLaunchKernelGGL((attn_fwd_ln_kernel<HD_, 4>), grid, dim3(64 * nw), 0, stream, *a, *nl);                     \
+    } while (0)
+    if (nl) {
+        if (a->hd == 64) FWD_LN(64);
+        else FWD_LN(32);
+    } else {
+        if (a->hd == 64) FWD(64);
+        else FWD(32);
+    }
 #undef FWD
+#undef FWD_LN
     MD_LAUNCH_CHECK();
     return 0;
 }
 
-extern "C" int md_attn_bwd(const md_attn_args* a_in, hipStream_t stream) {
+int attn_bwd_impl(const md_attn_args* a_in, const md_attn_ln* nl, hipStream_t stream);
+
+}
+
+extern "C" int md_attn_fwd(const md_attn_args* a_in, hipStream_t stream) { return attn_fwd_impl(a_in, nullptr, stream); }
+
+extern "C" int md_attn_fwd_ln(const md_attn_args* a_in, const md_attn_ln* nl, hipStream_t stream) {
+    if (!attn_ok(a_in) || !ln_ok(nl)) return MD_BAD_ARG;
+    if (a_in->Sq > 256 || a_in->Skv > 256) return MD_NOT_ELIGIBLE;
+    return attn_fwd_impl(a_in, nl, stream);
+}
+
+extern "C" int md_attn_bwd(const md_attn_args* a_in, hipStream_t stream) { return attn_bwd_impl(a_in, nullptr, stream); }
+
+extern "C" int md_attn_bwd_ln(const md_attn_args* a_in, const md_attn_ln* nl, hipStream_t stream) {
+    if (!attn_ok(a_in) || !ln_ok(nl)) return MD_BAD_ARG;
+    if (a_in->Sq > 256 || a_in->Skv > 256 || a_in->bwd_split == 5) return MD_NOT_ELIGIBLE;
+    return attn_bwd_impl(a_in, nl, stream);
+}
+
+namespace {
+int attn_bwd_impl(const md_attn_args* a_in, const md_attn_ln* nl, hipStream_t stream) {
     if (!attn_ok(a_in) || !a_in->d_o || !a_in->dq || !a_in->dk || !a_in->dv || !a_in->lse || !a_in->delta) return MD_BAD_ARG;
     const md_attn_args args = with_head_strides(a_in);
     const md_attn_args* a = &args;
@@ -1139,9 +1254,10 @@
         MD_LAUNCH_CHECK();
         return 0;
     }
-    if (a->hd == 64 ? launch_bwd_fused<64>(a, a->bwd_split, stream) : launch_bwd_fused<32>(a, a->bwd_split, stream)) {
+    if (a->hd == 64 ? launch_bwd_fused<64>(a, nl, a->bwd_split, stream) : launch_bwd_fused<32>(a, nl, a->bwd_split, stream)) {
         MD_LAUNCH_CHECK();
         return 0;
     }
     return -1;
 }
+}
diff --git a/micro_diffusion_amd/csrc/gemm_pp_common.h b/micro_diffusion_amd/csrc/gemm_pp_common.h
--- a/micro_diffusion_amd/csrc/gemm_pp_common.h
+++ b/micro_diffusion_amd/csrc/gemm_pp_common.h
@@ -119,6 +119,8 @@
     int nseg, nk_seg;
     int nprob;
     int tail_first, tail_units, tail_split, tail_nk;
+    float* rs_stats;
+    int rs_lo[2], rs_hi[2];
     PPProblem prob[PP_MAX_PROB];
 };
 
@@ -339,6 +341,8 @@
     w->ldb = (int)a->ldb;
     w->tail_first = w->total;
     w->tail_units = w->tail_split = w->tail_nk = 0;
+    w->rs_stats = nullptr;
+    w->rs_lo[0] = w->rs_lo[1] = w->rs_hi[0] = w->rs_hi[1] = 0;
     w->rps_shift = -1;
     if (a->rows_per_sample > 0 && (a->rows_per_sample & (a->rows_per_sample - 1)) == 0) {
         w->rps_shift = 0;
diff --git a/micro_diffusion_amd/csrc/gemm_w4.hip b/micro_diffusion_amd/csrc/gemm_w4.hip
--- a/micro_diffusion_amd/csrc/gemm_w4.hip
+++ b/micro_diffusion_amd/csrc/gemm_w4.hip
@@ -69,6 +69,10 @@
     char* c2;
     const char* op;
     int64_t sc, sc2, so;
+    char* st;
+    int64_t sst;
+    unsigned sl;
+    bool son;
 };
 
 template <int EPI, bool INTERIOR>
@@ -110,7 +114,7 @@
     }
 }
 
-template <int EPI, int I, bool INTERIOR>
+template <int EPI, int I, bool INTERIOR, bool RS = false>
 __device__ __forceinline__ void w4_epi_store(const md_gemm_args& p, const PPPlan& w, const W4Tile& et, const W4EpiLane& L, int wrow, int wcol,
                                              const w4_u32x4 (&Tv)[4], W4Ops& ops, W4Rows& R) {
 #pragma unroll
@@ -120,6 +124,24 @@
         const bool ok = INTERIOR || (wcol + L.c8 < et.nlim && row0 + L.rg < et.mlim);
         char* const crow = R.c;
         uint4 out = T;
+        if constexpr (RS) {
+            float xv[8];
+            unpack8(T, xv);
+            float s1 = ((xv[0] + xv[1]) + (xv[2] + xv[3])) + ((xv[4] + xv[5]) + (xv[6] + xv[7]));
+            float s2 = xv[0] * xv[0];
+#pragma unroll
+            for (int e = 1; e < 8; ++e) s2 = fmaf(xv[e], xv[e], s2);
+            s1 += dpp_f<0x111, 0xf>(s1);
+            s2 += dpp_f<0x111, 0xf>(s2);
+            s1 += dpp_f<0x112, 0xf>(s1);
+            s2 += dpp_f<0x112, 0xf>(s2);
+            s1 += dpp_f<0x114, 0xf>(s1);
+            s2 += dpp_f<0x114, 0xf>(s2);
+            s1 += dpp_f<0x118, 0xf>(s1);
+            s2 += dpp_f<0x118, 0xf>(s2);
+            if (R.son && L.c8 == 120 && (INTERIOR || row0 + L.rg < et.mlim)) *reinterpret_cast<float2*>(R.st + R.sl) = make_float2(s1, s2);
+            R.st += R.sst;
+        }
         if constexpr (EPI == PP_E_BF16 || EPI == PP_E_RES || EPI == PP_E_BF16_GELU) {
             if (et.c2base && ok) *reinterpret_cast<uint4*>(R.c2 + L.oc2) = T;
         }
@@ -218,7 +240,7 @@
     for (int t = 0; t < 4; ++t) Tv[t] = *reinterpret_cast<const w4_u32x4*>(half + L.rd[t]);
 }
 
-template <int EPI, bool INTERIOR>
+template <int EPI, bool INTERIOR, bool RS = false>
 __device__ __forceinline__ void w4_epilogue(const md_gemm_args& p, const PPPlan& w, const W4Tile& et, unsigned char* slab, int wrow, int wcol, int lane) {
     W4EpiLane L;
     w4_epi_lane<EPI>(p, et, wcol, lane, L);
@@ -231,6 +253,13 @@
     R.c = et.cbase + ((int64_t)wrow * p.ldc + wcol) * 2;
     R.c2 = et.c2base ? et.c2base + ((int64_t)wrow * p.ldc2 + wcol) * 2 : nullptr;
     R.op = nullptr;
+    if constexpr (RS) {
+        const int col = et.n0 + wcol, nslab = w.N >> 7;
+        R.son = w.rs_stats && ((col >= w.rs_lo[0] && col < w.rs_hi[0]) || (col >= w.rs_lo[1] && col < w.rs_hi[1]));
+        R.st = reinterpret_cast<char*>(w.rs_stats) + ((int64_t)(et.m0 + wrow) * nslab + (col >> 7)) * 8;
+        R.sst = (int64_t)32 * nslab;
+        R.sl = (unsigned)(L.rg * nslab) * 8u;
+    }
     if constexpr (EPI == PP_E_RES || w4_is_dact(EPI)) {
         R.op = et.opbase + ((int64_t)wrow * ldo + wcol) * 2;
 #pragma unroll
@@ -247,7 +276,7 @@
     w4_epi_read<I>(slab, L, Tv);                                                                                        \
     if constexpr ((I) < 7) w4_epi_write<((I) < 7 ? (I) + 1 : 7)>(slab, L);                                               \
     if constexpr ((I) == 0) asm volatile("s_waitcnt vmcnt(0)" ::: "memory");                                             \
-    w4_epi_store<EPI, I, INTERIOR>(p, w, et, L, wrow, wcol, Tv, ops, R);
+    w4_epi_store<EPI, I, INTERIOR, RS>(p, w, et, L, wrow, wcol, Tv, ops, R);
     W4_EPI_STEP(0) W4_EPI_STEP(1) W4_EPI_STEP(2) W4_EPI_STEP(3) W4_EPI_STEP(4) W4_EPI_STEP(5) W4_EPI_STEP(6) W4_EPI_STEP(7)
 #undef W4_EPI_STEP
 }
@@ -270,7 +299,7 @@
 #undef W4_F32_STEP
 }
 
-template <int AKC, int BKC, int EPI>
+template <int AKC, int BKC, int EPI, bool RS = false>
 __global__ __launch_bounds__(256) __attribute__((amdgpu_num_vgpr(144))) void gemm_bf16_w4_kernel(md_gemm_args p, PPPlan w) {
     __shared__ __attribute__((aligned(1024))) unsigned char smem[2 * W4_BREG + 4 * W4_SLAB];
     const int tid = threadIdx.x, lane = tid & 63;
@@ -461,8 +490,8 @@
             asm volatile("s_nop 15\n\ts_nop 15");
 #ifndef W4_X_NOEPI
             unsigned char* const slab = smem + 2 * W4_BREG + wave * W4_SLAB;
-            if (et.mlim >= PT && et.nlim >= PT) w4_epilogue<EPI, true>(p, w, et, slab, wr * 128, wc * 128, lane);
-            else w4_epilogue<EPI, false>(p, w, et, slab, wr * 128, wc * 128, lane);
+            if (et.mlim >= PT && et.nlim >= PT) w4_epilogue<EPI, true, RS>(p, w, et, slab, wr * 128, wc * 128, lane);
+            else w4_epilogue<EPI, false, RS>(p, w, et, slab, wr * 128, wc * 128, lane);
 #else
             asm volatile("s_waitcnt vmcnt(0)" ::: "memory");
 #endif
@@ -475,6 +504,7 @@
 
 }
 
+#ifndef W4_ROWSTATS_TU
 static bool w4_instantiated(int akc, int bkc, int epi) {
     if (!akc) return !bkc && epi == PP_E_F32;
     if (bkc) return epi == PP_E_BF16 || epi == PP_E_RES || epi == PP_E_DACT_GELU || epi == PP_E_DACT_MUL;
@@ -533,3 +563,4 @@
     MD_LAUNCH_CHECK();
     return 0;
 }
+#endif
diff --git a/micro_diffusion_amd/csrc/gemm_w4_rowstats.hip b/micro_diffusion_amd/csrc/gemm_w4_rowstats.hip
--- /dev/null
+++ b/micro_diffusion_amd/csrc/gemm_w4_rowstats.hip
@@ -0,0 +1,45 @@
+#define W4_ROWSTATS_TU
+#include "gemm_w4.hip"
+
+#include <stdlib.h>
+
+extern "C" int md_gemm_bf16_rowstats(const md_gemm_args* a_in, const md_gemm_rowstats* rs, hipStream_t stream) {
+    if (!a_in || !rs || !rs->stats || !a_in->A || !a_in->B || !a_in->C) return MD_BAD_ARG;
+    if (a_in->M <= 0 || a_in->N <= 0 || a_in->K <= 0 || a_in->lda % 8 || a_in->ldb % 8 || a_in->ldc % 8) return MD_BAD_ARG;
+    if (rs->nseg < 1 || rs->nseg > 2) return MD_BAD_ARG;
+    for (int i = 0; i < rs->nseg; ++i)
+        if (rs->col0[i] < 0 || rs->width[i] <= 0 || rs->col0[i] + rs->width[i] > a_in->N) return MD_BAD_ARG;
+    md_gemm_args a = *a_in;
+    if (a.mode != MD_EPI_STORE_BF16 || a.act != MD_ACT_NONE || a.C2 || a.bias || a.alpha != 1.f || a.dact_cached) return MD_NOT_ELIGIBLE;
+    if (!a.a_kcontig || !a.b_kcontig || a.batch != 1 || a.ksplit != 1 || a.problems || a.A_list || a.B_list || a.timeline) return MD_NOT_ELIGIBLE;
+    if (a.M % PT || a.N % 128) return MD_NOT_ELIGIBLE;
+    for (int i = 0; i < rs->nseg; ++i)
+        if (rs->col0[i] % 128 || rs->width[i] % 128) return MD_NOT_ELIGIBLE;
+    if (a.variant != MD_GEMM_AUTO && a.variant != MD_GEMM_W4) return MD_NOT_ELIGIBLE;
+    if (!md_gemm_w4_eligible(&a) || (a.cu_limit > 0 && a.cu_limit < NUM_CU) || getenv("MD_GEMM_NO_W4")) return MD_NOT_ELIGIBLE;
+    const int64_t ntn = (a.N + PT - 1) / PT, tiles256 = (a.M / PT) * ntn;
+    if (a.variant == MD_GEMM_AUTO) {
+        const char* w4min = getenv("MD_GEMM_W4_MIN_TILES");
+        if (tiles256 < (w4min ? atoi(w4min) : 192)) return MD_NOT_ELIGIBLE;
+    }
+    a.variant = MD_GEMM_W4;
+    if (a.raster_group_n <= 0) {
+        int64_t g = (2 << 20) / (PT * a.K * 2);
+        if (g < 4) g = 4;
+        if (g > ntn) g = ntn;
+        a.raster_group_n = (int)g;
+    }
+    PPPlan w;
+    if (!md_gemm_pp_plan(&a, &w)) return MD_BAD_ARG;
+    w.rs_stats = rs->stats;
+    for (int i = 0; i < rs->nseg; ++i) {
+        w.rs_lo[i] = (int)rs->col0[i];
+        w.rs_hi[i] = (int)(rs->col0[i] + rs->width[i]);
+    }
+    if (a.chosen_variant) *a.chosen_variant = MD_GEMM_W4;
+    if (a.tail_used) *a.tail_used = 0;
+    const unsigned G = (unsigned)(w.total < NUM_CU ? w.total : NUM_CU);
+    hipLaunchKernelGGL((gemm_bf16_w4_kernel<1, 1, PP_E_BF16, true>), dim3(G, 1, 1), dim3(256), 0, stream, a, w);
+    MD_LAUNCH_CHECK();
+    return 0;
+}
diff --git a/micro_diffusion_amd/csrc/norm.hip b/micro_diffusion_amd/csrc/norm.hip
--- a/micro_diffusion_amd/csrc/norm.hip
+++ b/micro_diffusion_amd/csrc/norm.hip
@@ -377,7 +377,24 @@
     }
 }
 
-template <int NCH>
+__global__ __launch_bounds__(256) void qkln_stats_finish_kernel(const float* partial, int64_t rows, int64_t nslab, int64_t slab0, int nsl,
+                                                              int nseg, int64_t seg_slabs, float* out, float invC, float eps) {
+    const int64_t i = (int64_t)blockIdx.x * 256 + threadIdx.x;
+    if (i >= rows * nseg) return;
+    const int64_t seg = i / rows, row = i - seg * rows;
+    const float2* src = reinterpret_cast<const float2*>(partial) + row * nslab + slab0 + seg * seg_slabs;
+    float s1 = 0.f, s2 = 0.f;
+    for (int k = 0; k < nsl; ++k) {
+        const float2 v = src[k];
+        s1 += v.x;
+        s2 += v.y;
+    }
+    const float mean = s1 * invC;
+    const float var = fmaxf(s2 * invC - mean * mean, 0.f);
+    reinterpret_cast<float2*>(out)[i] = make_float2(mean, rsqrtf(var + eps));
+}
+
+template <int NCH, bool RAW = false>
 __global__ __launch_bounds__(256) void qkln_bwd_kernel(bf16* d, int64_t ldd, int64_t dcol0, const bf16* y, int64_t ldy,
                                                        int64_t ycol0, int64_t rows, int C, int nseg, int64_t dseg_stride,
                                                        int64_t yseg_stride, const float* rstd_in) {
@@ -389,11 +406,21 @@
     auto dat = [&](int64_t vr) { return d + (vr / nseg) * ldd + dcol0 + (vr % nseg) * dseg_stride; };
     auto yat = [&](int64_t vr) { return y + (vr / nseg) * ldy + ycol0 + (vr % nseg) * yseg_stride; };
     bf16x8 ng[NCH], ny[NCH];
-    float nrstd = 0.f;
+    float nrstd = 0.f, nmean = 0.f;
+    auto stat = [&](int64_t vr) {
+        const int64_t at = (vr % nseg) * rows + vr / nseg;
+        if (RAW) {
+            const float2 ms = reinterpret_cast<const float2*>(rstd_in)[at];
+            nmean = ms.x;
+            nrstd = ms.y;
+        } else {
+            nrstd = rstd_in[at];
+        }
+    };
     if (wave < items) {
         issue_row<NCH>(dat(wave), C, lane, ng);
         issue_row<NCH>(yat(wave), C, lane, ny);
-        nrstd = rstd_in[(wave % nseg) * rows + wave / nseg];
+        stat(wave);
     }
     for (int64_t vr = wave; vr < items; vr += nwaves) {
         bf16* dr = dat(vr);
@@ -401,6 +428,14 @@
         unpack_row<NCH>(ng, g);
         unpack_row<NCH>(ny, xh);
         const float rstd = nrstd;
+        if (RAW) {
+            const float mean = nmean;
+#pragma unroll
+            for (int j = 0; j < NCH; ++j)
+#pragma unroll
+                for (int e = 0; e < 8; ++e)
+                    xh[j][e] = lane * 8 + j * 512 < C ? bf2f(f2bf((xh[j][e] - mean) * rstd)) : 0.f;
+        }
         float s1 = 0.f, s2 = 0.f;
 #pragma unroll
         for (int j = 0; j < NCH; ++j)
@@ -413,7 +448,7 @@
             const int64_t nx = vr + nwaves;
             issue_row<NCH>(dat(nx), C, lane, ng);
             issue_row<NCH>(yat(nx), C, lane, ny);
-            nrstd = rstd_in[(nx % nseg) * rows + nx / nseg];
+            stat(nx);
         }
         s1 = wave_sum(s1) * invC;
         s2 = wave_sum(s2) * invC;
@@ -680,6 +715,31 @@
     return 0;
 }
 
+extern "C" int md_qkln_bwd_raw(void* d, int64_t ldd, int64_t dcol0, const void* y, int64_t ldy, int64_t ycol0, int64_t rows,
+                               int64_t width, int32_t nseg, int64_t dseg_stride, int64_t yseg_stride, const float* stats,
+                               hipStream_t stream) {
+    if (!d || !y || !stats || rows <= 0 || width <= 0 || width % 8 || width > 64 * 8 * MAXCH || ldd % 8 || ldy % 8 ||
+        dcol0 % 8 || ycol0 % 8 || nseg < 1 || nseg > 4 || dseg_stride % 8 || yseg_stride % 8)
+        return MD_BAD_ARG;
+#define QKB(N) hipLaunchKernelGGL((qkln_bwd_kernel<N, true>), dim3(ln_grid(rows * nseg)), dim3(256), 0, stream, (bf16*)d, ldd, dcol0, \
+                                  (const bf16*)y, ldy, ycol0, rows, (int)width, (int)nseg, dseg_stride, yseg_stride, stats)
+    if (width <= 512) QKB(1); else if (width <= 1024) QKB(2); else QKB(4);
+#undef QKB
+    MD_LAUNCH_CHECK();
+    return 0;
+}
+
+extern "C" int md_qk_stats_finish(const float* partial, int64_t rows, int64_t nslab, int64_t col0, int64_t width, int32_t nseg,
+                                  int64_t seg_stride, float* out, float eps, hipStream_t stream) {
+    if (!partial || !out || rows <= 0 || nslab <= 0 || col0 < 0 || width <= 0 || col0 % 128 || width % 128 || nseg < 1 || nseg > 2 ||
+        seg_stride % 128 || (nseg > 1 && seg_stride < width) || col0 + (nseg - 1) * seg_stride + width > nslab * 128)
+        return MD_BAD_ARG;
+    hipLaunchKernelGGL(qkln_stats_finish_kernel, dim3((unsigned)((rows * nseg + 255) / 256)), dim3(256), 0, stream, partial, rows, nslab,
+                       col0 / 128, (int)(width / 128), (int)nseg, seg_stride / 128, out, 1.f / (float)width, eps);
+    MD_LAUNCH_CHECK();
+    return 0;
+}
+
 namespace {
 inline bool hm_ok(int64_t rows, int64_t width, int64_t S, int32_t hd) {
     return S > 0 && rows % S == 0 && (hd == 32 || hd == 64) && width % hd == 0;
diff --git a/micro_diffusion_amd/engine.py b/micro_diffusion_amd/engine.py
--- a/micro_diffusion_amd/engine.py
+++ b/micro_diffusion_amd/engine.py
@@ -130,6 +130,7 @@
         self.gemm_tail_mode = int(os.environ.get("MD_GEMM_TAIL", "0"))
         self.wgrad_bf16 = None
         self.fuse_swiglu_bwd = os.environ.get("MD_FUSE_SWIGLU_BWD", "1") != "0"
+        self.fuse_qkln_fwd = os.environ.get("MD_FUSE_QKLN_FWD", "0") != "0"
         self.weights_version = 0
         self.cu_limit_fn = None
 
@@ -226,14 +227,41 @@
             self.L.md_qkln_bwd_hm(dy.data_ptr(), rows * width, y.data_ptr(), rows * width, dptr, ldd, doff, width, rows, width, nseg, S,
                                   self.cfg.head_dim, rstd_ptr, self._st()), "md_qkln_bwd_hm"))
 
-    def _attn_fwd(self, a):
+    def _qkln_bwd_raw(self, dptr, ldd, doff, yptr, ldy, yoff, rows, width, stats_ptr, nseg=1):
+        self._prof("qk_layernorm", 6.0 * rows * width * nseg, lambda: hip.check(
+            self.L.md_qkln_bwd_raw(dptr, ldd, doff, yptr, ldy, yoff, rows, width, nseg, width, width, stats_ptr, self._st()), "md_qkln_bwd_raw"))
+
+    def _lin_fwd_rowstats(self, x, wname, out, M, N, K, width, nseg):
+        if not self.fuse_qkln_fwd or self.qk_head_major or M % 256 or N % 128 or width % 128 or (wname + ".bias") in self.P:
+            return None
+        part = self.empty(M, N // 128, 2, dtype=F32)
+        rs = hip.GemmRowStats(part.data_ptr(), (ctypes.c_int64 * 2)(0, width), (ctypes.c_int64 * 2)(width, width), nseg)
+        if not self._gemm(A=x.data_ptr(), B=self.S[wname + ".weight"].data_ptr(), C=out.data_ptr(), M=M, N=N, K=K, lda=K, ldb=K, ldc=N,
+                          ldc2=N, ldr=N, batch=1, ksplit=1, a_kcontig=1, b_kcontig=1, mode=hip.EPI_STORE_BF16, act=0, alpha=1.0,
+                          _rowstats=rs):
+            return None
+        st = self.empty(nseg, M, 2, dtype=F32)
+        self._prof("qk_stats_finish", 8.0 * M * nseg * (width // 128 + 1), lambda: hip.check(
+            self.L.md_qk_stats_finish(part.data_ptr(), M, N // 128, 0, width, nseg, width, st.data_ptr(), self.cfg.norm_eps, self._st()),
+            "md_qk_stats_finish"))
+        return st
+
+    def _attn_fwd(self, a, ln=None):
         nb = 2.0 * a.hd * (2 * a.Sq + 2 * a.Skv) * a.B * a.H
+        if ln is not None:
+            return self._prof("attention", nb, lambda: hip.check(self.L.md_attn_fwd_ln(byref(a), byref(ln), self._st()), "md_attn_fwd_ln"))
         self._prof("attention", nb, lambda: hip.check(self.L.md_attn_fwd(byref(a), self._st()), "md_attn_fwd"))
+
+    def _attn_ln(self, q_stats, k_stats, Sq, Skv):
+        if (q_stats is None and k_stats is None) or Sq > 256 or Skv > 256:
+            return None
+        return hip.AttnLn(q_stats, k_stats, 2, 2)
 
     def _gemm(self, **kw):
         a = hip.GemmArgs()
         problems = kw.pop("_problems", None)
         may_refuse = kw.pop("_try", False)
+        rowstats = kw.pop("_rowstats", None)
         for k, v in kw.items():
             setattr(a, k, v)
         if self.deterministic and a.mode == hip.EPI_ATOMIC_F32 and a.ksplit > 1:
@@ -251,12 +279,17 @@
             a.tail_ws, a.tail_ws_bytes, a.tail_mode = self.ws.data_ptr(), TAIL_WS_BYTES, self.gemm_tail_mode
         rc = hip.NOT_ELIGIBLE
         want = self.gemm_prefer if self.gemm_prefer != hip.GEMM_AUTO else a.variant
-        if want != hip.GEMM_AUTO:
+        if rowstats is not None:
+            a.variant = want if want == hip.GEMM_W4 else hip.GEMM_AUTO
+            rc = self.L.md_gemm_bf16_rowstats(byref(a), byref(rowstats), self._st())
+            if rc == hip.NOT_ELIGIBLE:
+                return False
+        elif want != hip.GEMM_AUTO:
             a.variant = want
             rc = self.L.md_gemm_bf16(byref(a), self._st())
             if rc == hip.NOT_ELIGIBLE:
                 a.variant = hip.GEMM_AUTO
-        if rc == hip.NOT_ELIGIBLE:
+        if rc == hip.NOT_ELIGIBLE and rowstats is None:
             rc = self.L.md_gemm_bf16(byref(a), self._st())
         if rc == hip.NOT_ELIGIBLE and may_refuse:
             return False
@@ -490,26 +523,38 @@
             a.hsk = a.hsdk = Skv * hd
         return a
 
-    def _attn_bwd(self, a):
-        self._prof("attention", 2.0 * a.hd * (4 * a.Sq + 4 * a.Skv) * a.B * a.H, lambda: self._attn_bwd_launch(a))
-
-    def _attn_bwd_launch(self, a):
+    def _attn_bwd(self, a, ln=None):
+        self._prof("attention", 2.0 * a.hd * (4 * a.Sq + 4 * a.Skv) * a.B * a.H, lambda: self._attn_bwd_launch(a, ln))
+
+    def _attn_bwd_launch(self, a, ln=None):
+        if ln is not None:
+            launch = lambda: self.L.md_attn_bwd_ln(byref(a), byref(ln), self._st())
+        else:
+            launch = lambda: self.L.md_attn_bwd(byref(a), self._st())
         rc = -1
-        if self.attn_bwd_prefer != hip.ATTN_BWD_AUTO:
+        if self.attn_bwd_prefer != hip.ATTN_BWD_AUTO and not (ln is not None and self.attn_bwd_prefer == hip.ATTN_BWD_STREAM_PAIR):
             a.bwd_split = self.attn_bwd_prefer
-            rc = self.L.md_attn_bwd(byref(a), self._st())
+            rc = launch()
             a.bwd_split = hip.ATTN_BWD_AUTO
         if rc == -1:
-            rc = self.L.md_attn_bwd(byref(a), self._st())
+            rc = launch()
         hip.check(rc, "md_attn_bwd")
 
     def _self_attn_fwd(self, pre, xin, B, S, dim, hid, heads, t):
         M, L, st = B * S, self.L, self._st()
         qkv = self.empty(M, 3 * hid)
+        o = self.empty(M, hid)
+        lse = self.empty(B, heads, S, dtype=F32)
+        t.sqk = self._lin_fwd_rowstats(xin, pre + ".qkv", qkv, M, 3 * hid, dim, hid, 2) if S <= 256 else None
+        if t.sqk is not None:
+            t.qk = None
+            a = self.attn_args(qkv.data_ptr(), qkv.data_ptr() + 2 * hid, qkv.data_ptr() + 4 * hid, o, lse, B, heads, S, S,
+                               3 * hid, 3 * hid, 3 * hid, hid)
+            self._attn_fwd(a, self._attn_ln(t.sqk.data_ptr(), t.sqk.data_ptr() + 8 * M, S, S))
+            t.qkv, t.rq, t.o, t.lse = qkv, None, o, lse
+            return o
         self.lin_fwd(xin, pre + ".qkv", qkv, M, 3 * hid, dim)
         rq = self.empty(2, M, dtype=F32)
-        o = self.empty(M, hid)
-        lse = self.empty(B, heads, S, dtype=F32)
         if self.qk_head_major:
             t.qk = self.empty(2, M, hid)
             self._qkln_fwd_hm(qkv.data_ptr(), M, 3 * hid, 0, hid, t.qk, S, rq.data_ptr(), nseg=2)
@@ -540,15 +585,23 @@
             a = self.attn_args(qkv.data_ptr(), qkv.data_ptr() + 2 * hid, qkv.data_ptr() + 4 * hid, t.o, t.lse, B, heads, S, S,
                                3 * hid, 3 * hid, 3 * hid, hid, do=do, dq=dqkv.data_ptr(), dk=dqkv.data_ptr() + 2 * hid,
                                dv=dqkv.data_ptr() + 4 * hid, delta=delta, lddq=3 * hid, lddk=3 * hid, lddv=3 * hid)
-            self._attn_bwd(a)
-            self._qkln_bwd(dqkv.data_ptr(), 3 * hid, 0, qkv.data_ptr(), 3 * hid, 0, M, hid, t.rq.data_ptr(), nseg=2)
+            if t.sqk is not None:
+                self._attn_bwd(a, self._attn_ln(t.sqk.data_ptr(), t.sqk.data_ptr() + 8 * M, S, S))
+                self._qkln_bwd_raw(dqkv.data_ptr(), 3 * hid, 0, qkv.data_ptr(), 3 * hid, 0, M, hid, t.sqk.data_ptr(), nseg=2)
+            else:
+                self._attn_bwd(a)
+                self._qkln_bwd(dqkv.data_ptr(), 3 * hid, 0, qkv.data_ptr(), 3 * hid, 0, M, hid, t.rq.data_ptr(), nseg=2)
         self.lin_wgrad(dqkv, xin, pre + ".qkv", M, 3 * hid, dim, defer=defer)
         dxin = self.empty(M, dim)
         self.lin_dgrad(dqkv, pre + ".qkv", dxin, M, 3 * hid, dim)
         return dxin
 
-    def _kv_linear_fwd(self, n, ycond, Mc, hx, d):
+    def _kv_linear_fwd(self, n, ycond, Mc, hx, d, stats=None):
         kv = self.empty(Mc, 2 * hx)
+        if stats is not None:
+            stats.append(self._lin_fwd_rowstats(ycond, n + ".cross_attn.kv_linear", kv, Mc, 2 * hx, d, hx, 1))
+            if stats[0] is not None:
+                return kv
         self.lin_fwd(ycond, n + ".cross_attn.kv_linear", kv, Mc, 2 * hx, d)
         return kv
 
@@ -592,15 +645,30 @@
         self.ln_fwd(self.ln_args(x1, n + ".norm2", t.xn2, M, d, mean=t.st2[0], rstd=t.st2[1]))
         t.o2 = self.empty(M, hx)
         t.q2 = t.o2 if self.qk_head_major else self.empty(M, hx)
-        self.lin_fwd(t.xn2, n + ".cross_attn.q_linear", t.q2, M, hx, d)
+        lnx = S <= 256 and Lc <= 256
+        t.sq2 = self._lin_fwd_rowstats(t.xn2, n + ".cross_attn.q_linear", t.q2, M, hx, d, hx, 1) if lnx else None
+        if t.sq2 is None:
+            self.lin_fwd(t.xn2, n + ".cross_attn.q_linear", t.q2, M, hx, d)
+        t.sk2 = None
         if kv is None:
-            t.kv = self._kv_linear_fwd(n, ycond, Mc, hx, d)
+            ks = [] if lnx else None
+            t.kv = self._kv_linear_fwd(n, ycond, Mc, hx, d, stats=ks)
+            t.sk2 = ks[0] if ks else None
         else:
             t.kv, t.k2n = kv
             t.rk2 = None
-        t.rq2 = self.empty(M, dtype=F32)
+        t.rq2 = self.empty(M, dtype=F32) if t.sq2 is None else None
         t.lse2 = self.empty(B, bp.xheads, S, dtype=F32)
-        if self.qk_head_major:
+        if t.sq2 is not None or t.sk2 is not None:
+            t.q2n = None
+            if t.sq2 is None:
+                self._qkln_fwd(t.q2.data_ptr(), M, hx, 0, hx, t.rq2.data_ptr())
+            if kv is None and t.sk2 is None:
+                t.rk2, t.k2n = self._k_norm_fwd(t.kv, Mc, hx, Lc)
+            ax = self.attn_args(t.q2.data_ptr(), t.kv.data_ptr(), t.kv.data_ptr() + 2 * hx, t.o2, t.lse2, B, bp.xheads, S, Lc,
+                                hx, 2 * hx, 2 * hx, hx)
+            self._attn_fwd(ax, self._attn_ln(_p(t.sq2), _p(t.sk2), S, Lc))
+        elif self.qk_head_major:
             t.q2n = self.empty(M, hx)
             self._qkln_fwd_hm(t.q2.data_ptr(), M, hx, 0, hx, t.q2n, S, t.rq2.data_ptr())
             if kv is None:
@@ -614,7 +682,8 @@
                 t.rk2, t.k2n = self._k_norm_fwd(t.kv, Mc, hx, Lc)
             ax = self.attn_args(t.q2.data_ptr(), t.kv.data_ptr(), t.kv.data_ptr() + 2 * hx, t.o2, t.lse2, B, bp.xheads, S, Lc,
                                 hx, 2 * hx, 2 * hx, hx)
-        self._attn_fwd(ax)
+        if t.sq2 is None and t.sk2 is None:
+            self._attn_fwd(ax)
         x2 = self.empty(M, d)
         self.lin_fwd(t.o2, n + ".cross_attn.proj", x2, M, d, hx, mode=hip.EPI_RESIDUAL, res=x1)
         t.x2 = x2
@@ -758,9 +827,15 @@
             ax = self.attn_args(t.q2.data_ptr(), t.kv.data_ptr(), t.kv.data_ptr() + 2 * hx, t.o2, t.lse2, B, bp.xheads, S, Lc, hx,
                                 2 * hx, 2 * hx, hx, do=do2, dq=dq2.data_ptr(), dk=dkv.data_ptr(), dv=dkv.data_ptr() + 2 * hx,
                                 delta=delta, lddq=hx, lddk=2 * hx, lddv=2 * hx)
-            self._attn_bwd(ax)
-            self._qkln_bwd(dq2.data_ptr(), hx, 0, t.q2.data_ptr(), hx, 0, M, hx, t.rq2.data_ptr())
-            self._qkln_bwd(dkv.data_ptr(), 2 * hx, 0, t.kv.data_ptr(), 2 * hx, 0, Mc, hx, t.rk2.data_ptr())
+            self._attn_bwd(ax, self._attn_ln(_p(t.sq2), _p(t.sk2), S, Lc))
+            if t.sq2 is not None:
+                self._qkln_bwd_raw(dq2.data_ptr(), hx, 0, t.q2.data_ptr(), hx, 0, M, hx, t.sq2.data_ptr())
+            else:
+                self._qkln_bwd(dq2.data_ptr(), hx, 0, t.q2.data_ptr(), hx, 0, M, hx, t.rq2.data_ptr())
+            if t.sk2 is not None:
+                self._qkln_bwd_raw(dkv.data_ptr(), 2 * hx, 0, t.kv.data_ptr(), 2 * hx, 0, Mc, hx, t.sk2.data_ptr())
+            else:
+                self._qkln_bwd(dkv.data_ptr(), 2 * hx, 0, t.kv.data_ptr(), 2 * hx, 0, Mc, hx, t.rk2.data_ptr())
         self.lin_wgrad(dq2, t.xn2, n + ".cross_attn.q_linear", M, hx, d, defer=True)
         self.lin_wgrad(dkv, ycond, n + ".cross_attn.kv_linear", Mc, 2 * hx, d)
         if kvgroup is None:
diff --git a/micro_diffusion_amd/hip.py b/micro_diffusion_amd/hip.py
--- a/micro_diffusion_amd/hip.py
+++ b/micro_diffusion_amd/hip.py
@@ -141,6 +141,14 @@
                 ("hsdq", c_int64), ("hsdk", c_int64), ("hsdv", c_int64), ("hsdo", c_int64)]
 
 
+class GemmRowStats(Structure):
+    _fields_ = [("stats", c_void_p), ("col0", c_int64 * 2), ("width", c_int64 * 2), ("nseg", c_int32)]
+
+
+class AttnLn(Structure):
+    _fields_ = [("q_stats", c_void_p), ("k_stats", c_void_p), ("q_stride", c_int64), ("k_stride", c_int64)]
+
+
 class AdamWArgs(Structure):
     _fields_ = [("p", c_void_p), ("g", c_void_p), ("m", c_void_p), ("v", c_void_p), ("shadow", c_void_p),
                 ("sumsq", c_void_p), ("g_bf16", c_void_p), ("ema", c_void_p), ("n", c_int64),
@@ -172,6 +180,11 @@
 _sig("md_qkln_bwd_hm", P, I64, P, I64, P, I64, I64, I64, I64, I64, I32, I64, I32, P, P)
 _sig("md_attn_fwd", POINTER(AttnArgs), P)
 _sig("md_attn_bwd", POINTER(AttnArgs), P)
+_sig("md_gemm_bf16_rowstats", POINTER(GemmArgs), POINTER(GemmRowStats), P)
+_sig("md_qk_stats_finish", P, I64, I64, I64, I64, I32, I64, P, F32, P)
+_sig("md_qkln_bwd_raw", P, I64, I64, P, I64, I64, I64, I64, I32, I64, I64, P, P)
+_sig("md_attn_fwd_ln", POINTER(AttnArgs), POINTER(AttnLn), P)
+_sig("md_attn_bwd_ln", POINTER(AttnArgs), POINTER(AttnLn), P)
 _sig("md_swiglu_fwd", P, I64, P, I64, I64, I64, P)
 _sig("md_swiglu_bwd", P, I64, P, I64, P, I64, I64, I64, P)
 _sig("md_gate_bwd", P, P, P, I64, P, P, I64, I64, I64, I64, I64, P)
```

Result: no change. 2809 images/sec (-0.1%).
